# zhaoweicai/mscnn

Measured on AMD Instinct MI355X. Metric: images/sec mscnn-7s-576 KITTI-car inference, higher is better.
Workload: dtype f32

## Files before the change

include/mscnn_hip.h:

```cpp
#ifndef MSCNN_HIP_H_
#define MSCNN_HIP_H_

#include <stddef.h>
#include <stdint.h>

#if defined(__GNUC__)
#define MSCNN_API __attribute__((visibility("default")))
#else
#define MSCNN_API
#endif

#ifdef __cplusplus
extern "C" {
#endif

typedef enum {
  MSCNN_OK = 0,
  MSCNN_ERR_BAD_ARG = 1,
  MSCNN_ERR_HIP = 2,
  MSCNN_ERR_WORKSPACE = 3,
  MSCNN_ERR_UNSUPPORTED = 4
} mscnn_status;

MSCNN_API const char* mscnn_last_error(void);
MSCNN_API const char* mscnn_version(void);

typedef struct mscnn_conv_plan mscnn_conv_plan;

typedef enum {
  MSCNN_CONV_ALGO_AUTO = 0,
  MSCNN_CONV_ALGO_DIRECT = 1,
  MSCNN_CONV_ALGO_WINO_F2 = 2,
  MSCNN_CONV_ALGO_WINO_F3 = 3,
  MSCNN_CONV_ALGO_F16 = 4,
  MSCNN_CONV_ALGO_WINO_F3_X3 = 5,
  MSCNN_CONV_ALGO_WINO_F4 = 6
} mscnn_conv_algo;

typedef struct {
  int N, Cin, H, W;
  int Cout, Kh, Kw;
  int pad_h, pad_w, stride_h, stride_w, group;
  int relu;
  int algo;
  int tune_variant, tune_grid, tune_flags;
} mscnn_conv_desc;

MSCNN_API int mscnn_conv2d_plan_create(const mscnn_conv_desc* desc, mscnn_conv_plan** plan_out);
MSCNN_API void mscnn_conv2d_plan_destroy(mscnn_conv_plan* plan);
MSCNN_API size_t mscnn_conv2d_packed_weight_bytes(const mscnn_conv_plan* plan);
MSCNN_API size_t mscnn_conv2d_workspace_bytes(const mscnn_conv_plan* plan);
MSCNN_API const char* mscnn_conv2d_plan_kernel(const mscnn_conv_plan* plan);
MSCNN_API double mscnn_conv2d_plan_flops(const mscnn_conv_plan* plan);
MSCNN_API const char* mscnn_conv2d_plan_dtype(const mscnn_conv_plan* plan);
MSCNN_API double mscnn_conv2d_plan_executed_flops(const mscnn_conv_plan* plan);
MSCNN_API int mscnn_conv2d_plan_plane_columns(const mscnn_conv_plan* plan, int* cols, int n);
MSCNN_API int mscnn_conv2d_plan_set_profiling(mscnn_conv_plan* plan, int on);
MSCNN_API int mscnn_conv2d_plan_stage_ms(const mscnn_conv_plan* plan, float ms_out[3]);
#define MSCNN_AMAX_SLOTS 1024
MSCNN_API int mscnn_conv2d_plan_publishes_amax(const mscnn_conv_plan* plan);
MSCNN_API int mscnn_conv2d_plan_set_amax_io(mscnn_conv_plan* plan, const uint32_t* in_bound, uint32_t* out_amax);
MSCNN_API int mscnn_conv2d_plan_set_batch(mscnn_conv_plan* plan, int N);
MSCNN_API unsigned long long mscnn_conv2d_plan_weight_layout(const mscnn_conv_plan* plan);
MSCNN_API int mscnn_conv2d_pack_weights(const mscnn_conv_plan* plan, const float* w, float* packed, void* stream);
MSCNN_API int mscnn_conv2d_fwd_f32(const mscnn_conv_plan* plan, const float* x, const float* w, const float* packed,
                         const float* bias, float* y, void* workspace, size_t workspace_bytes, void* stream);
MSCNN_API int mscnn_conv2d_plan_can_pool(const mscnn_conv_plan* plan);
MSCNN_API int mscnn_conv2d_fwd_pool_f32(const mscnn_conv_plan* plan, const float* x, const float* w, const float* packed,
                              const float* bias, float* y, float* y_pool, void* workspace, size_t workspace_bytes,
                              void* stream);

MSCNN_API int mscnn_relu_fwd_f32(const float* x, float* y, size_t count, float negative_slope, void* stream);

MSCNN_API int mscnn_pool_out_dim(int in, int kernel, int pad, int stride);
MSCNN_API int mscnn_pool2d_fwd_f32(const float* x, float* y, int N, int C, int H, int W, int kernel_h, int kernel_w,
                         int pad_h, int pad_w, int stride_h, int stride_w, int method, void* stream);

MSCNN_API int mscnn_inner_product_fwd_f32(const float* x, const float* w, const float* bias, float* y,
                                int M, int N, int K, int relu, void* stream);
MSCNN_API void mscnn_debug_inner_product_rows(int rows);

MSCNN_API int mscnn_inner_product_wg_supported(int M, int N, int K);
MSCNN_API size_t mscnn_inner_product_wg_packed_bytes(int N, int K);
MSCNN_API size_t mscnn_inner_product_wg_workspace_bytes(int M, int N, int K);
MSCNN_API int mscnn_inner_product_wg_pack(const float* w, float* wt, int N, int K, void* stream);
MSCNN_API int mscnn_inner_product_wg_fwd(const float* x, const float* wt, const float* bias, float* y, int M, int N, int K, int relu,
                                         void* workspace, size_t workspace_bytes, void* stream);
MSCNN_API unsigned long long mscnn_wgemm_handoff_event(void);
MSCNN_API void mscnn_wgemm_force_whole_tiles(int on);
MSCNN_API int mscnn_wgemm_whole_tiles_forced(void);
MSCNN_API void mscnn_debug_wgemm_handoff_fault(int drop_publish, unsigned spin_limit);
MSCNN_API long mscnn_debug_wgemm_schedule(const mscnn_conv_plan* plan, int whole_tiles, int* rows, long max_rows, int info[8]);
MSCNN_API int mscnn_inner_product_x3_supported(int N, int K);
MSCNN_API size_t mscnn_inner_product_x3_packed_bytes(int N, int K);
MSCNN_API size_t mscnn_inner_product_x3_workspace_bytes(int M, int N, int K);
MSCNN_API int mscnn_inner_product_x3_pack(const float* w, void* packed, int N, int K, void* stream);
MSCNN_API int mscnn_inner_product_x3_fwd(const float* x, const void* packed, const float* bias, float* y, int M, int N, int K, int relu,
                               const uint32_t* in_bound, void* workspace, size_t workspace_bytes, void* stream);
MSCNN_API int mscnn_inner_product_f16_supported(int N, int K);
MSCNN_API int mscnn_inner_product_pack_f16(const float* w, void* w16, int N, int K, void* stream);
MSCNN_API int mscnn_inner_product_fwd_f16(const float* x, const void* w16, const float* bias, float* y, int M, int N, int K, int relu,
                                          void* stream);

MSCNN_API int mscnn_concat_channels_f32(const float* x, float* y, int N, int C, int inner, int C_total, int c_offset, void* stream);

MSCNN_API int mscnn_deconv_depthwise_fwd_f32(const float* x, const float* w, const float* bias, float* y,
                                   int N, int C, int H, int W, int Kh, int Kw, int pad_h, int pad_w,
                                   int stride_h, int stride_w, void* stream);

MSCNN_API int mscnn_deconv2d_fwd_f32(const float* x, const float* w, const float* bias, float* y, int N, int Cin, int H, int W,
                                     int Cout, int Kh, int Kw, int pad_h, int pad_w, int stride_h, int stride_w, int group,
                                     void* stream);

MSCNN_API int mscnn_max_rel_diff_f32(const float* a, const float* ref, size_t count, float floor, float* out_dev, void* stream);
MSCNN_API int mscnn_max_rel_diff_strided_f32(const float* a, size_t a_stride, const float* ref, size_t ref_stride, size_t planes, size_t run,
                                             const double* sumsq_dev, double sumsq_count, float* out_dev, void* stream);
MSCNN_API int mscnn_store_words_i32(int* dst_dev, const int* values_host, int n, void* stream);
MSCNN_API int mscnn_sum_squares_f32(const float* x, size_t count, double* out_dev, void* stream);

MSCNN_API int mscnn_softmax_fwd_f32(const float* x, float* y, int outer, int C, int inner, void* stream);

MSCNN_API int mscnn_roipool_fwd_f32(const float* feat, const float* rois, float* out, int R, int N, int C, int H, int W,
                          int pooled_h, int pooled_w, float spatial_scale, float pad_ratio,
                          int C_total, int c_offset, void* stream);
MSCNN_API int mscnn_roipool_pair_fwd_f32(const float* feat, const float* rois, float* out, int R, int N, int C, int H, int W,
                                         int pooled_h, int pooled_w, float spatial_scale, float pad_ratio_a, int c_offset_a,
                                         float pad_ratio_b, int c_offset_b, int C_total, void* stream);

MSCNN_API int mscnn_conv2d_plan_can_chain(const mscnn_conv_plan* plan, const mscnn_conv_plan* next);
MSCNN_API int mscnn_conv2d_plan_can_pool_only(const mscnn_conv_plan* plan);
MSCNN_API int mscnn_conv2d_fwd_chain_f32(const mscnn_conv_plan* plan, const mscnn_conv_plan* next, const float* x, const float* packed,
                               const float* bias, float* y, float* y_pool, void* workspace, size_t workspace_bytes,
                               void* next_workspace, size_t next_workspace_bytes, void* stream);

MSCNN_API int mscnn_conv2d_plan_can_fuse_roipool(const mscnn_conv_plan* plan, int C, int pooled_h, int pooled_w);
MSCNN_API size_t mscnn_conv2d_roipool_workspace_bytes(const mscnn_conv_plan* plan, int N, int C, int H, int W);
MSCNN_API size_t mscnn_roipool_maps_bytes(int N, int C, int H, int W);
MSCNN_API int mscnn_roipool_maps_build_f32(const float* feat, float* maps, int N, int C, int H, int W, void* stream);
MSCNN_API int mscnn_conv2d_fwd_roipool_pair_f32(const mscnn_conv_plan* plan, const float* feat, const float* prepared_maps, int N, int C,
                                                int H, int W, const float* rois, float spatial_scale, float pad_ratio_a,
                                                float pad_ratio_b, const float* packed_w, const float* bias, float* y, void* workspace,
                                                size_t workspace_bytes, void* stream);

MSCNN_API int mscnn_roialign_fwd_f32(const float* feat, const float* rois, float* out, int R, int N, int C, int H, int W,
                                     int pooled_h, int pooled_w, float spatial_scale, float pad_ratio, void* stream);
MSCNN_API int mscnn_roialign_ave_fwd_f32(const float* feat, const float* rois, float* out, int R, int N, int C, int H, int W,
                                         int pooled_h, int pooled_w, float spatial_scale, float pad_ratio,
                                         int C_total, int c_offset, void* stream);
MSCNN_API int mscnn_roialign_ave_pair_fwd_f32(const float* feat, const float* rois, float* out, int R, int N, int C, int H, int W,
                                              int pooled_h, int pooled_w, float spatial_scale, float pad_ratio_a, int c_offset_a,
                                              float pad_ratio_b, int c_offset_b, int C_total, void* stream);

MSCNN_API int mscnn_eltwise_fwd_f32(const float* const* bottoms_host, int num_bottoms, const float* coeffs_host, float* y,
                                    size_t count, int op, void* stream);

#define MSCNN_BOXOUT_MAX_HEADS 16
typedef struct {
  int num_heads;
  int num;
  int channels;
  int head_h[MSCNN_BOXOUT_MAX_HEADS], head_w[MSCNN_BOXOUT_MAX_HEADS];
  float field_w[MSCNN_BOXOUT_MAX_HEADS], field_h[MSCNN_BOXOUT_MAX_HEADS], downsample_rate[MSCNN_BOXOUT_MAX_HEADS];
  float fg_thr, iou_thr;
  int nms_mode;
  float field_whr, field_xyr;
  int max_nms_num, max_post_nms_num;
  float min_size;
  int do_bbox_norm;
  float bbox_mean[4], bbox_std[4];
} mscnn_boxoutput_desc;

MSCNN_API size_t mscnn_boxoutput_workspace_bytes(const mscnn_boxoutput_desc* desc);
MSCNN_API int mscnn_boxoutput_max_rows(const mscnn_boxoutput_desc* desc);
MSCNN_API int mscnn_boxoutput_fwd_f32(const mscnn_boxoutput_desc* desc, const float* const* heads_host,
                            float* rois_out, float* props_out, int* anchor_ids_out, int cap,
                            int* count_out_dev, void* workspace, size_t workspace_bytes, void* stream);
MSCNN_API size_t mscnn_boxoutput_batch_workspace_bytes(const mscnn_boxoutput_desc* desc);
MSCNN_API int mscnn_boxoutput_batch_fwd_f32(const mscnn_boxoutput_desc* desc, const float* const* heads_host,
                            float* rois_out, float* props_out, int* anchor_ids_out, int cap,
                            int* count_out_dev, void* workspace, size_t workspace_bytes, void* stream);

MSCNN_API size_t mscnn_nms_workspace_bytes(int n);
MSCNN_API int mscnn_nms_greedy_f32(const float* boxes_xywh, int n, float iou_thr, int nms_mode, unsigned char* keep_out,
                         void* workspace, size_t workspace_bytes, void* stream);

MSCNN_API int mscnn_decodebbox_fwd_f32(const float* bbox, const float* prior, float* out, int R, int bbox_dim,
                             const float* mean_host, const float* std_host, void* stream);

typedef struct {
  int ncls, cls_id;
  float bbox_mean[4], bbox_std[4];
  float proposal_thr;
  double ratio_h, ratio_w, org_h, org_w, nms_overlap;
} mscnn_detections_desc;
MSCNN_API size_t mscnn_detections_workspace_bytes(int R);

enum { MSCNN_NMS_TYPE_MAXG = 0, MSCNN_NMS_TYPE_MAX = 1, MSCNN_NMS_TYPE_MS = 2, MSCNN_NMS_TYPE_COVER = 3, MSCNN_NMS_TYPE_NONE = 4 };
enum { MSCNN_NMS_OVR_UNION = 0, MSCNN_NMS_OVR_MIN = 1 };
#ifndef MSCNN_NMS_PARAMS_DEFINED
#define MSCNN_NMS_PARAMS_DEFINED
typedef struct {
  int type;
  int ovr_dnm;
  double thr;
  float det_thr;
} mscnn_nms_params;
#endif
MSCNN_API int mscnn_nms_params_resolve(const mscnn_nms_params* nms, mscnn_nms_params* out);
MSCNN_API int mscnn_nms_params_from_names(const char* type, const char* ovr_dnm, double thr, double maxn, float det_thr,
                                          mscnn_nms_params* out);
MSCNN_API int mscnn_detections_fwd(const mscnn_detections_desc* desc, const float* bbox_pred, const float* cls_pred,
                         const float* props, int R, double* dets_out, int* ids_out, int* count_out_dev,
                         void* workspace, size_t workspace_bytes, void* stream);

MSCNN_API int mscnn_detections_nms_fwd(const mscnn_detections_desc* desc, const mscnn_nms_params* nms, const float* bbox_pred,
                                       const float* cls_pred, const float* props, int R, double* dets_out, int* ids_out,
                                       int* count_out_dev, void* workspace, size_t workspace_bytes, void* stream);

MSCNN_API int mscnn_detections_cascade_fwd(const mscnn_detections_desc* desc, float det_thr, const float* boxes,
                                 const float* cls_prob, const float* props, int R, double* dets_out, int* ids_out,
                                 int* count_out_dev, void* workspace, size_t workspace_bytes, void* stream);
MSCNN_API int mscnn_detections_cascade_nms_fwd(const mscnn_detections_desc* desc, float det_thr, const mscnn_nms_params* nms,
                                               const float* boxes, const float* cls_prob, const float* props, int R, double* dets_out,
                                               int* ids_out, int* count_out_dev, void* workspace, size_t workspace_bytes, void* stream);

enum { MSCNN_MULTI_PACK_WORDS = 4 };
typedef struct { size_t dets, ids, total; } mscnn_multi_pack_layout;
static inline mscnn_multi_pack_layout mscnn_multi_pack_layout_of(int num_segments, int cap) {
  const size_t S = (size_t)(num_segments > 0 ? num_segments : 0), rows = (size_t)(cap > 0 ? cap : 1);
  mscnn_multi_pack_layout L;
  L.dets = sizeof(int32_t) * MSCNN_MULTI_PACK_WORDS * (1 + S);
  L.ids = L.dets + rows * 5 * sizeof(double);
  L.total = (L.ids + rows * sizeof(int32_t) + 15) / 16 * 16;
  return L;
}
#ifdef __HIPCC__
__host__ __device__
#endif
static inline size_t mscnn_multi_pack_slot(int K, int row0, int k, int rows) {
  return (size_t)K * row0 + (size_t)k * rows;
// ... 88 lines not shown
```

mscnn_amd/csrc/gemm.hip:

```cpp
#include "common.h"
#include "wgemm.h"

namespace {

typedef float f32x16 __attribute__((ext_vector_type(16)));

constexpr int BK = 32, LDK = BK + 4;

struct GemmArgs {
  const float* x; const float* w; const float* bias; float* y; float* ws;
  int M, N, K, MT, NT, KI, G, relu;
  long total_iters;
};

__device__ __forceinline__ void wg_range(long total, int G, int g, long& b, long& e) {
  b = total * g / G;
  e = total * (g + 1) / G;
}

template <int BM, int BN>
__global__ __launch_bounds__(256) void gemm_tn_kernel(GemmArgs a) {
  static_assert(BM * BN == 128 * 128 && BM % 64 == 0 && BN % 64 == 0, "4 waves of 64 x 64");
  __shared__ __attribute__((aligned(16))) float ldsX[BM * LDK];
  __shared__ __attribute__((aligned(16))) float ldsW[BN * LDK];
// ... 378 lines not shown

static int inner_product_gemm(const float* x, const void* w, bool w_is_f16, const float* bias, float* y, int M, int N, int K, int relu,
                              hipStream_t st);

extern "C" int mscnn_inner_product_fwd_f16(const float* x, const void* w16, const float* bias, float* y, int M, int N, int K, int relu,
                                           void* stream) {
  MSCNN_REQUIRE(M >= 0 && N > 0 && K > 0, "inner_product: bad shape M=%d N=%d K=%d", M, N, K);
  if (M == 0) return MSCNN_OK;
  MSCNN_REQUIRE(x && w16 && y, "inner_product: null pointer");
  MSCNN_REQUIRE(mscnn_inner_product_f16_supported(N, K) && reinterpret_cast<uintptr_t>(x) % 16 == 0 && reinterpret_cast<uintptr_t>(w16) % 16 == 0,
                "inner_product f16: needs N >= 64, K %% 8 == 0 and 16-byte aligned operands (N=%d K=%d)", N, K);
  return inner_product_gemm(x, w16, true, bias, y, M, N, K, relu, as_stream(stream));
}

static int g_ip_rows = 0;
extern "C" void mscnn_debug_inner_product_rows(int rows) { g_ip_rows = rows == 2 || rows == 4 || rows == 8 ? rows : 0; }

extern "C" int mscnn_inner_product_fwd_f32(const float* x, const float* w, const float* bias, float* y, int M, int N, int K,
                                           int relu, void* stream) {
  MSCNN_REQUIRE(M >= 0 && N > 0 && K > 0, "inner_product: bad shape M=%d N=%d K=%d", M, N, K);
  if (M == 0) return MSCNN_OK;
  MSCNN_REQUIRE(x && w && y, "inner_product: null pointer");
  hipStream_t st = as_stream(stream);
  const bool aligned = (K % 4 == 0) && (reinterpret_cast<uintptr_t>(x) % 16 == 0) && (reinterpret_cast<uintptr_t>(w) % 16 == 0);
  if (N < 64 || !aligned) {
    if (N <= kRowMaxN && K <= 256 * kRowMaxKPerThread) {
      const int rows = g_ip_rows ? g_ip_rows : (N <= 5 ? 4 : 2);
#define MSCNN_IP_ROWWISE(NB_, R_) ip_rowwise_kernel<NB_, R_><<<cdiv(M, R_), 256, 0, st>>>(x, w, bias, y, M, N, K, relu)
      if (N <= 5) { if (rows == 8) MSCNN_IP_ROWWISE(5, 8); else if (rows == 2) MSCNN_IP_ROWWISE(5, 2); else MSCNN_IP_ROWWISE(5, 4); }
      else { if (rows == 8) MSCNN_IP_ROWWISE(4, 8); else if (rows == 2) MSCNN_IP_ROWWISE(8, 2); else MSCNN_IP_ROWWISE(4, 4); }
#undef MSCNN_IP_ROWWISE
    } else {
      ip_generic_kernel<<<dim3(M, N < 64 ? N : 64), 256, 0, st>>>(x, w, bias, y, M, N, K, relu);
    }
    MSCNN_POST_LAUNCH();
    return MSCNN_OK;
  }
  return inner_product_gemm(x, w, false, bias, y, M, N, K, relu, st);
}

static int inner_product_gemm(const float* x, const void* w, bool w_is_f16, const float* bias, float* y, int M, int N, int K, int relu,
                              hipStream_t st) {
  GemmArgs a;
  a.x = x; a.w = static_cast<const float*>(w); a.bias = bias; a.y = y;
  a.M = M; a.N = N; a.K = K; a.relu = relu;
  const bool m64 = cdiv(M, 64) * 64 < cdiv(M, 128) * 128 && N >= 256;
  const int BM = m64 ? 64 : 128, BN = m64 ? 256 : 128;
  a.MT = cdiv(M, BM); a.NT = cdiv(N, BN); a.KI = cdiv(K, BK);
  a.total_iters = (long)a.MT * a.NT * a.KI;
  long G = 512;
  if (a.total_iters / 8 < G) G = a.total_iters / 8;
  if (G < 1) G = 1;
  a.G = (int)G;
  const size_t need = (size_t)a.G * 2 * BM * BN * sizeof(float);
  {
    const int rc = reserve_slabs(need, &a.ws);
    if (rc != MSCNN_OK) return rc;
  }
  if (w_is_f16) {
    if (m64) gemm16_tn_kernel<64, 256><<<a.G, 256, 0, st>>>(a);
    else gemm16_tn_kernel<128, 128><<<a.G, 256, 0, st>>>(a);
  } else {
    if (m64) gemm_tn_kernel<64, 256><<<a.G, 256, 0, st>>>(a);
    else gemm_tn_kernel<128, 128><<<a.G, 256, 0, st>>>(a);
  }
  MSCNN_POST_LAUNCH();
  if (m64) gemm_fixup_kernel<64, 256><<<a.MT * a.NT * 4, 256, 0, st>>>(a);
  else gemm_fixup_kernel<128, 128><<<a.MT * a.NT * 4, 256, 0, st>>>(a);
  MSCNN_POST_LAUNCH();
  return MSCNN_OK;
}


namespace {

__global__ __launch_bounds__(256) void ip_pack_rows_kernel(const float* __restrict__ x, float* __restrict__ up, int M, int K, int KI) {
  __shared__ float t[32][257];
  const int kc = blockIdx.x, mt = blockIdx.y, tid = threadIdx.x;
  const int r0 = mt * 256, k0 = kc * 32;
#pragma unroll
  for (int i = 0; i < 8; ++i) {
    const int v = tid + i * 256, row = v >> 3, k4 = (v & 7) * 4;
    float4 q = make_float4(0.f, 0.f, 0.f, 0.f);
    if (r0 + row < M) q = *reinterpret_cast<const float4*>(x + (size_t)(r0 + row) * K + k0 + k4);
    t[k4][row] = q.x; t[k4 + 1][row] = q.y; t[k4 + 2][row] = q.z; t[k4 + 3][row] = q.w;
  }
  __syncthreads();
  float* dst = up + ((size_t)mt * KI + kc) * (32 * 256);
#pragma unroll
  for (int i = 0; i < 32; ++i) dst[i * 256 + tid] = t[i][tid];
}

__global__ __launch_bounds__(256) void ip_transpose_w_kernel(const float* __restrict__ w, float* __restrict__ wt, int N, int K) {
  __shared__ float t[32][33];
  const int k0 = blockIdx.x * 32, n0 = blockIdx.y * 32, tx = threadIdx.x & 31, ty = threadIdx.x >> 5;
#pragma unroll
  for (int i = 0; i < 4; ++i) {
    const int n = n0 + ty + 8 * i, k = k0 + tx;
    t[ty + 8 * i][tx] = (n < N && k < K) ? w[(size_t)n * K + k] : 0.f;
  }
  __syncthreads();
#pragma unroll
  for (int i = 0; i < 4; ++i) {
    const int k = k0 + ty + 8 * i, n = n0 + tx;
    if (k < K && n < N) wt[(size_t)k * N + n] = t[tx][ty + 8 * i];
  }
}

bool ip_wg_plan(int M, int N, int K, mscnn::WgemmPlan* pl) {
  if (M < 192 || N % 128 != 0 || K % 32 != 0 || N < 256) return false;
  const int Mp = (M + 31) / 32 * 32;
  return mscnn::wgemm_plan(1, Mp, K, N, 1 + 64, pl) && pl->T_pad == N;
}

}

extern "C" int mscnn_inner_product_wg_supported(int M, int N, int K) {
  mscnn::WgemmPlan pl;
  return ip_wg_plan(M, N, K, &pl) ? 1 : 0;
}
extern "C" size_t mscnn_inner_product_wg_packed_bytes(int N, int K) { return (size_t)N * K * sizeof(float); }
extern "C" size_t mscnn_inner_product_wg_workspace_bytes(int M, int N, int K) {
  mscnn::WgemmPlan pl;
  if (!ip_wg_plan(M, N, K, &pl)) return 0;
  return (pl.packed_bytes + 255) / 256 * 256 + pl.ws_bytes;
}
extern "C" int mscnn_inner_product_wg_pack(const float* w, float* wt, int N, int K, void* stream) {
  MSCNN_REQUIRE(w && wt && N > 0 && K > 0, "inner_product wg pack: bad argument");
  ip_transpose_w_kernel<<<dim3(cdiv(K, 32), cdiv(N, 32)), 256, 0, as_stream(stream)>>>(w, wt, N, K);
  MSCNN_POST_LAUNCH();
  return MSCNN_OK;
}
extern "C" int mscnn_inner_product_wg_fwd(const float* x, const float* wt, const float* bias, float* y, int M, int N, int K, int relu,
                                          void* workspace, size_t workspace_bytes, void* stream) {
  MSCNN_REQUIRE(M >= 0 && N > 0 && K > 0, "inner_product: bad shape M=%d N=%d K=%d", M, N, K);
  if (M == 0) return MSCNN_OK;
  mscnn::WgemmPlan pl;
  MSCNN_REQUIRE(ip_wg_plan(M, N, K, &pl), "inner_product wg: shape M=%d N=%d K=%d is not one the plane-GEMM kernel takes", M, N, K);
  MSCNN_REQUIRE(x && wt && y && reinterpret_cast<uintptr_t>(x) % 16 == 0, "inner_product wg: null or unaligned pointer");
  MSCNN_REQUIRE_ALIGNED(wt, 16, "inner_product wg: wt");
  MSCNN_REQUIRE_ALIGNED(workspace, 16, "inner_product wg: workspace");
  const size_t need = mscnn_inner_product_wg_workspace_bytes(M, N, K);
  if (!workspace || workspace_bytes < need) {
    set_error("inner_product wg: workspace %zu < %zu", workspace_bytes, need);
    return MSCNN_ERR_WORKSPACE;
  }
  hipStream_t st = as_stream(stream);
  float* up = static_cast<float*>(workspace);
  float* slabs = reinterpret_cast<float*>(static_cast<unsigned char*>(workspace) + (pl.packed_bytes + 255) / 256 * 256);
  ip_pack_rows_kernel<<<dim3(pl.KI, pl.MT), 256, 0, st>>>(x, up, M, K, pl.KI);
  MSCNN_POST_LAUNCH();
  return mscnn::wgemm_launch(pl, up, wt, y, pl.ws_bytes ? slabs : nullptr, st, 0, nullptr, bias, relu, (size_t)M * N * sizeof(float));
}
```

mscnn_amd/csrc/wgemm.h:

```cpp
#pragma once
#include <hip/hip_runtime.h>
#include <cstddef>

namespace mscnn {

constexpr int kWgemmMaxPlanes = 36;

__host__ __device__ __forceinline__ void wgemm_tile_decode(int t, int MT, int NT, int P, const int* nt_off, int& p, int& nt, int& mt) {
  mt = t % MT;
  if (!nt_off) {
    nt = (t / MT) % NT;
    p = t / (MT * NT);
    return;
  }
#if defined(__HIP_DEVICE_COMPILE__)
  const int q = __builtin_amdgcn_readfirstlane(t / MT);
#else
  const int q = t / MT;
#endif
  int pp = 0;
  while (pp + 1 < P && nt_off[pp + 1] <= q) ++pp;
  p = pp;
  nt = q - nt_off[pp];
}

struct WgemmPlan {
  int P, Cout, Cin, T, T_pad;
  int BM, BN, CK, MT, NT, KI;
  int G;
  int tiles;
  int ragged;
  int cols[kWgemmMaxPlanes];
  int nt_off[kWgemmMaxPlanes + 1];
  int device;
  int full_q;
  int variant;
  double model_us;
  const char* name;
  size_t packed_bytes;
  size_t ws_bytes;
};

bool wgemm_plan(int P, int Cout, int Cin, int T, int variant, WgemmPlan* out, const int* plane_cols = nullptr);

int wgemm_launch(const WgemmPlan& p, const float* Up, const float* V, float* M, float* ws, hipStream_t st, int abl = 0,
                 unsigned long long* dbg = nullptr, const float* bias = nullptr, int relu = 0, size_t m_valid_bytes = 0);

unsigned long long wgemm_handoff_event();
void wgemm_force_whole_tiles(int on);
int wgemm_whole_tiles_forced();
void wgemm_debug_handoff_fault(int drop_publish, unsigned spin_limit);
long wgemm_debug_schedule(const WgemmPlan& p, int whole_tiles, int* out, long max_rows);

}
```

mscnn_amd/csrc/wgemm.hip:

```cpp
#include "wgemm.h"
#include "common.h"
#include <atomic>
#include <chrono>

namespace {

typedef float f32x16 __attribute__((ext_vector_type(16)));

struct WgemmArgs {
  const float* Up; const float* V; float* M; float* ws;
  int P, MT, NT, KI, Cin, Cout, T_pad;
  int tiles, G, abl;
  int full_q;
  unsigned ws_bytes;
  unsigned epoch;
  unsigned long long* dbg;
  unsigned up_bytes, v_bytes, m_bytes;
  const float* bias; int relu;
  unsigned long long* status;
  unsigned spin_limit;
  int drop_publish;
  int nt_off[mscnn::kWgemmMaxPlanes + 1];
};

template <int BM_, int BN_, int WGM_, int WGN_, int CK_, int ST_, int DPG_ = 1, int SK_ = 0>
struct WCfg {
  static constexpr int BM = BM_, BN = BN_, WGM = WGM_, WGN = WGN_, CK = CK_, ST = ST_;
  static constexpr int DPG = DPG_, SK = SK_;
  static constexpr int NW = WGM * WGN, THREADS = NW * 64;
  static constexpr int WM = BM / WGM, WN = BN / WGN, MI = WM / 32, NI = WN / 32;
  static constexpr int A_BYTES = CK * BM * 4, B_BYTES = CK * BN * 4, STAGE_BYTES = A_BYTES + B_BYTES;
  static constexpr int STAGE_FLOATS = STAGE_BYTES / 4;
  static constexpr int PA = A_BYTES / 1024, PB = B_BYTES / 1024;
  static constexpr int PA_W = PA / NW, PB_W = (PB + NW - 1) / NW;
  static constexpr int NP = PA_W + PB_W;
  static constexpr int F4_PER_ROW = BN / 4;
  static constexpr bool B_EVEN = (64 % F4_PER_ROW == 0) && (PB % NW == 0);
  static constexpr int ROWS_PER_PIECE = B_EVEN ? 64 / F4_PER_ROW : 0;
  static constexpr int LDS_FLOATS = ST * STAGE_FLOATS + (B_EVEN ? 0 : 256);
  static constexpr int STEPS = CK / 2;
  static_assert(PA % NW == 0 && B_BYTES % 1024 == 0, "pieces per wave");
  static_assert(LDS_FLOATS * 4 <= 160 * 1024, "LDS ring");
  static_assert(WM % 32 == 0 && WN % 32 == 0, "wave tile");
};

template <int I, int N, class F>
__device__ __forceinline__ void static_for(F&& f) {
  if constexpr (I < N) {
    f(std::integral_constant<int, I>{});
    static_for<I + 1, N>(f);
  }
}

__device__ __forceinline__ __amdgpu_buffer_rsrc_t make_rsrc(const void* p, unsigned bytes) {
  return __builtin_amdgcn_make_buffer_rsrc(const_cast<void*>(p), 0, (int)bytes, 0x00020000);
}

__device__ __forceinline__ void dma16(__amdgpu_buffer_rsrc_t rsrc, unsigned voff, unsigned soff, unsigned lds_addr) {
  soff = __builtin_amdgcn_readfirstlane(soff);
  lds_addr = __builtin_amdgcn_readfirstlane(lds_addr);
  asm volatile("s_nop 4\n\ts_mov_b32 m0, %3\n\ts_nop 0\n\tbuffer_load_dwordx4 %0, %1, %2 offen lds" ::"v"(voff), "s"(rsrc), "s"(soff), "s"(lds_addr) : "memory");
}

template <int N>
__device__ __forceinline__ void wait_vm_barrier() {
  if constexpr (N == 0) asm volatile("s_waitcnt vmcnt(0)\n\ts_barrier" ::: "memory");
  else asm volatile("s_waitcnt vmcnt(%0)\n\ts_barrier" ::"n"(N) : "memory");
}

template <int OFF>
__device__ __forceinline__ float lds_rd(unsigned addr) {
  float r;
  asm volatile("ds_read_b32 %0, %1 offset:%2" : "=v"(r) : "v"(addr), "n"(OFF) : "memory");
  return r;
}
template <int N>
__device__ __forceinline__ void lds_wait() { asm volatile("s_waitcnt lgkmcnt(%0)" ::"n"(N) : "memory"); }
__device__ __forceinline__ void lds_pin(float& v) { asm volatile("" : "+v"(v)); }

__device__ __host__ __forceinline__ void wg_range(int total, int G, int g, int& b, int& e) {
  b = (int)((unsigned)total * (unsigned)g / (unsigned)G);
  e = (int)((unsigned)total * (unsigned)(g + 1) / (unsigned)G);
}

struct SegCursor {
  int slot, G, KI, full_q, rem_tile0, r;
  int it, re;
  int nparts;
  __device__ __forceinline__ void init(const WgemmArgs& a, int slot_) { init(a.tiles, a.G, a.KI, a.full_q, slot_); }
  __device__ __host__ __forceinline__ void init(int tiles, int G_, int KI_, int a_full_q, int slot_) {
    slot = slot_; G = G_; KI = KI_; rem_tile0 = a_full_q * G_; r = 0; nparts = 0;
    const int rounds = slot_ < tiles ? (tiles - slot_ + G_ - 1) / G_ : 0;
    full_q = a_full_q < rounds ? a_full_q : rounds;
    if (tiles > rem_tile0) wg_range((tiles - rem_tile0) * KI_, G_, slot_, it, re);
    else it = re = 0;
  }
  __device__ __forceinline__ int units() const { return full_q * KI + (re - it); }
  __device__ __host__ __forceinline__ bool next(int& t, int& k0, int& k1, int& part) {
    if (r < full_q) { t = slot + r * G; k0 = 0; k1 = KI; part = -1; ++r; return true; }
    if (it >= re) return false;
    t = rem_tile0 + it / KI;
    k0 = it % KI;
    const int left = re - it;
    k1 = left < KI - k0 ? k0 + left : KI;
    it += k1 - k0;
    part = (k0 == 0 && k1 == KI) ? -1 : nparts++;
    return true;
  }
};

template <class C, int ABL, int EPI = 0, bool RAG = false>
__global__ __launch_bounds__(C::THREADS, C::NW / 4) void wgemm_kernel(WgemmArgs a) {
  __shared__ __attribute__((aligned(1024))) float lds[C::LDS_FLOATS];
  __shared__ unsigned s_handoff_timeout;
  static_assert(C::ST == 3, "the ring protocol below is written for three stages");
  const int tid = threadIdx.x;
  const int lane = tid & 63;
  const int wave = __builtin_amdgcn_readfirstlane(tid >> 6);
  const int l31 = lane & 31, khalf = lane >> 5;
  const int wm = wave / C::WGN, wn = wave % C::WGN;

  const int xcd = (int)(blockIdx.x % 8), gq = a.G / 8, gr = a.G % 8;
  const int slot = xcd * gq + min(xcd, gr) + (int)(blockIdx.x / 8);
  SegCursor pcur, ccur;
  pcur.init(a, slot); ccur.init(a, slot);
  const int nunits = pcur.units();
  if (nunits == 0) return;
  unsigned long long dbg_c = 0, dbg_r = 0;
  if (a.dbg && tid == 0) { dbg_c = __builtin_amdgcn_s_memtime(); dbg_r = __builtin_amdgcn_s_memrealtime(); }

  const __amdgpu_buffer_rsrc_t rA = make_rsrc(a.Up, a.up_bytes), rB = make_rsrc(a.V, a.v_bytes), rM = make_rsrc(a.M, a.m_bytes),
                               rW = make_rsrc(a.ws, a.ws_bytes);
  const unsigned row_bytes = (unsigned)a.T_pad * 4u;
  const unsigned vA = (unsigned)lane * 16u;
  const unsigned vB = (unsigned)(lane / C::F4_PER_ROW) * row_bytes + (unsigned)(lane % C::F4_PER_ROW) * 16u;
  unsigned vBj[C::PB_W];
#pragma unroll
  for (int i = 0; i < C::PB_W; ++i) {
    const int u = (wave * C::PB_W + i) * 64 + lane;
    vBj[i] = wave * C::PB_W + i < C::PB ? (unsigned)(u / C::F4_PER_ROW) * row_bytes + (unsigned)(u % C::F4_PER_ROW) * 16u : 0x80000000u;
  }
  const unsigned lds0 = (unsigned)(size_t)lds;
  const unsigned a_lane = (unsigned)(khalf * C::BM + wm * C::WM + l31) * 4u;
  const unsigned b_lane = (unsigned)C::A_BYTES + (unsigned)(khalf * C::BN + wn * C::WN + l31) * 4u;

  int pu = 0, p_kc = 0, p_k1 = 0, p_stage = 0;
  unsigned p_a = 0, p_b = 0;
  unsigned vA_eff = vA, vB_eff = vB;
  auto p_begin = [&]() {
    if (pu >= nunits) {
      vA_eff = 0x80000000u; vB_eff = 0x80000000u;
#pragma unroll
      for (int i = 0; i < C::PB_W; ++i) vBj[i] = 0x80000000u;
    }
    if (p_kc == p_k1 && pu < nunits) {
      int t, part;
      pcur.next(t, p_kc, p_k1, part);
      int mt, nt, p;
      mscnn::wgemm_tile_decode(t, a.MT, a.NT, a.P, RAG ? a.nt_off : nullptr, p, nt, mt);
      p_kc = __builtin_amdgcn_readfirstlane(p_kc); p_k1 = __builtin_amdgcn_readfirstlane(p_k1);
      p_a = __builtin_amdgcn_readfirstlane((unsigned)((p * a.MT + mt) * a.KI) * (unsigned)C::A_BYTES);
      p_b = __builtin_amdgcn_readfirstlane(((unsigned)(p * a.Cin) * (unsigned)a.T_pad + (unsigned)(nt * C::BN)) * 4u);
    }
  };
  auto p_piece = [&](auto ic) {
    constexpr int i = decltype(ic)::value;
    const unsigned ls = lds0 + (unsigned)p_stage * C::STAGE_BYTES;
    if constexpr (i < C::PA_W) {
      const unsigned sa = p_a + (unsigned)p_kc * C::A_BYTES + (unsigned)(wave * C::PA_W + i) * 1024u;
      dma16(rA, vA_eff, sa, ls + (unsigned)(wave * C::PA_W + i) * 1024u);
    } else if constexpr (C::B_EVEN) {
      const int j = wave * C::PB_W + (i - C::PA_W);
      const unsigned sb = p_b + (unsigned)(p_kc * C::CK + j * C::ROWS_PER_PIECE) * row_bytes;
      dma16(rB, vB_eff, sb, ls + C::A_BYTES + (unsigned)j * 1024u);
    } else {
      const int j = wave * C::PB_W + (i - C::PA_W);
      const unsigned sb = p_b + (unsigned)(p_kc * C::CK) * row_bytes;
      dma16(rB, vBj[i - C::PA_W], sb, j < C::PB ? ls + C::A_BYTES + (unsigned)j * 1024u : lds0 + (unsigned)(C::ST * C::STAGE_BYTES));
    }
  };
  auto p_end = [&]() {
    ++pu;
    ++p_kc;
    if (++p_stage == C::ST) p_stage = 0;
  };

#pragma unroll
  for (int i = 0; i < 2; ++i)
    if (pu < nunits) {
      p_begin();
      static_for<0, C::NP>([&](auto ic) { p_piece(ic); });
      p_end();
    }
  wait_vm_barrier<0>();

  f32x16 acc[2][C::MI][C::NI];
#pragma unroll
  for (int q = 0; q < 2; ++q)
#pragma unroll
    for (int mi = 0; mi < C::MI; ++mi)
#pragma unroll
      for (int ni = 0; ni < C::NI; ++ni)
#pragma unroll
        for (int r = 0; r < 16; ++r) acc[q][mi][ni][r] = 0.f;
  float old_bias[C::NI];
#pragma unroll
  for (int ni = 0; ni < C::NI; ++ni) old_bias[ni] = 0.f;
  unsigned old_voff[C::MI][C::NI];
#pragma unroll
  for (int mi = 0; mi < C::MI; ++mi)
#pragma unroll
    for (int ni = 0; ni < C::NI; ++ni) old_voff[mi][ni] = 0x80000000u;

  float av[2][C::MI], bv[2][C::NI];
#define WG_READ(buf, stage_addr, s)                                                                                         \
  {                                                                                                                         \
    _Pragma("unroll") for (int mi = 0; mi < C::MI; ++mi) av[buf][mi] = 0.f;                                                  \
    static_for<0, C::MI>([&](auto m_) { av[buf][decltype(m_)::value] = lds_rd<(s) * 2 * C::BM * 4 + decltype(m_)::value * 128>((stage_addr) + a_lane); }); \
    static_for<0, C::NI>([&](auto n_) { bv[buf][decltype(n_)::value] = lds_rd<(s) * 2 * C::BN * 4 + decltype(n_)::value * 128>((stage_addr) + b_lane); }); \
  }
  constexpr int NR = C::MI + C::NI;
  constexpr int NMF = C::MI * C::NI;
  constexpr int TOTAL = NMF * 16;
  constexpr int SPG = (TOTAL + (C::STEPS - C::SK) - 1) / (C::STEPS - C::SK);
  constexpr int SPM = (SPG + NMF - 1) / NMF;
  constexpr int DMA_GROUPS = (C::NP + C::DPG - 1) / C::DPG;
  static_assert(C::DPG <= NMF && DMA_GROUPS <= C::STEPS && C::SK < C::STEPS, "schedule");
  constexpr int AFTER_DMA = [] {
    int n = 0;
    for (int g = 0; g < C::STEPS; ++g)
      for (int j = 0; j < NMF; ++j) {
        if (g < C::SK) continue;
        const int lo = (g - C::SK) * SPG + j * SPM, hi_g = (g - C::SK + 1) * SPG;
        int cnt = 0;
        for (int k = lo; k < lo + SPM && k < hi_g && k < TOTAL; ++k) ++cnt;
        const bool after = g > DMA_GROUPS - 1 || (g == DMA_GROUPS - 1 && j > (C::NP - 1) % C::DPG);
        if (after) n += cnt;
      }
    return n;
  }();

  __amdgpu_buffer_rsrc_t old_rsrc = rM;
  unsigned old_rowb = row_bytes;
  bool old_pub = false;
  unsigned c_addr = lds0;
  WG_READ(0, c_addr, 0);

  auto store_one = [&](auto qc, auto ec) {
    constexpr int Q = decltype(qc)::value, e = decltype(ec)::value;
    constexpr int blk = e / 16, r = e % 16, mi = blk / C::NI, ni = blk % C::NI, dr = (r & 3) + 8 * (r >> 2);
    float v = acc[Q][mi][ni][r];
    if (old_pub) __builtin_amdgcn_raw_buffer_store_b32(__builtin_bit_cast(unsigned, v), old_rsrc, old_voff[mi][ni], (unsigned)dr * old_rowb, 16);
    else {
      if constexpr (EPI) {
        v += old_bias[ni];
        if (a.relu) v = v < 0.f ? 0.f : v;
      }
      __builtin_amdgcn_raw_buffer_store_b32(__builtin_bit_cast(unsigned, v), old_rsrc, old_voff[mi][ni], (unsigned)dr * old_rowb, 0);
    }
  };

  auto chunk = [&](auto par_c, auto flush_c, unsigned next_addr) {
    constexpr int PAR = decltype(par_c)::value;
    constexpr bool FLUSH = decltype(flush_c)::value;
    p_begin();
    static_for<0, C::STEPS>([&](auto sc) {
      constexpr int s = decltype(sc)::value, cur = s & 1, nxt = cur ^ 1;
      if constexpr (!(ABL & 8)) {
        if constexpr (s + 1 < C::STEPS) WG_READ(nxt, c_addr, s + 1)
        else WG_READ(nxt, next_addr, 0)
        lds_wait<NR>();
      }
#pragma unroll
      for (int mi = 0; mi < C::MI; ++mi) lds_pin(av[cur][mi]);
#pragma unroll
      for (int ni = 0; ni < C::NI; ++ni) lds_pin(bv[cur][ni]);
      __builtin_amdgcn_sched_barrier(0);
      static_for<0, NMF>([&](auto jc) {
        constexpr int j = decltype(jc)::value, mi = j / C::NI, ni = j % C::NI;
        if constexpr (!(ABL & 4)) acc[PAR][mi][ni] = __builtin_amdgcn_mfma_f32_32x32x2f32(av[cur][mi], bv[cur][ni], acc[PAR][mi][ni], 0, 0, 0);
        __builtin_amdgcn_sched_barrier(0);
        if constexpr (FLUSH && s >= C::SK) {
          if constexpr (!(ABL & 2))
            static_for<0, SPM>([&](auto kc_) {
              constexpr int e = (s - C::SK) * SPG + j * SPM + decltype(kc_)::value;
              if constexpr (e < (s - C::SK + 1) * SPG && e < TOTAL) store_one(std::integral_constant<int, PAR ^ 1>{}, std::integral_constant<int, e>{});
            });
          __builtin_amdgcn_sched_barrier(0);
        }
        if constexpr (j < C::DPG && s * C::DPG + j < C::NP) {
          if constexpr (!(ABL & 1)) p_piece(std::integral_constant<int, s * C::DPG + j>{});
          __builtin_amdgcn_sched_barrier(0);
        }
      });
    });
    p_end();
    if constexpr (ABL & 16) asm volatile("s_waitcnt vmcnt(0)" ::: "memory");
    else if constexpr (FLUSH) wait_vm_barrier<(AFTER_DMA < 63 ? AFTER_DMA : 63)>();
    else wait_vm_barrier<0>();
    c_addr = next_addr;
  };

  int c_stage = 0;
  auto next_stage_addr = [&]() {
    if (++c_stage == C::ST) c_stage = 0;
    return lds0 + (unsigned)c_stage * C::STAGE_BYTES;
  };
  int t, k0, k1, part;
  int fin_tile = -1;
  typedef __attribute__((address_space(1))) unsigned long long gu64;
  gu64* flags = (gu64*)(a.ws + (size_t)a.G * (C::BM * C::BN));
  const unsigned long long want_flag = ((unsigned long long)a.epoch << 32) | (unsigned)~a.epoch;
  auto publish_flag = [&]() {
    asm volatile("s_waitcnt vmcnt(0)\n\ts_barrier" ::: "memory");
    if (tid == 0 && !a.drop_publish) __hip_atomic_store(flags + slot, want_flag, __ATOMIC_RELAXED, __HIP_MEMORY_SCOPE_AGENT);
  };
  auto segment = [&](auto par_c) {
    constexpr int PAR = decltype(par_c)::value;
    chunk(par_c, std::true_type{}, next_stage_addr());
    if (old_pub) { publish_flag(); old_pub = false; }
    for (int kc = k0 + 1; kc < k1; ++kc) chunk(par_c, std::false_type{}, next_stage_addr());
    int mt, nt, p;
    mscnn::wgemm_tile_decode(t, a.MT, a.NT, a.P, RAG ? a.nt_off : nullptr, p, nt, mt);
    const bool pub = part >= 0 && k0 > 0;
    if (part >= 0 && k0 == 0) fin_tile = t;
    old_pub = pub;
    if (pub) { old_rsrc = rW; old_rowb = (unsigned)C::BN * 4u; }
    else { old_rsrc = rM; old_rowb = row_bytes; }
    const unsigned slab = (unsigned)slot * (unsigned)(C::BM * C::BN * 4);
    if constexpr (EPI) {
#pragma unroll
      for (int ni = 0; ni < C::NI; ++ni) {
        const int col = nt * C::BN + wn * C::WN + ni * 32 + l31;
        old_bias[ni] = (a.bias && col < a.T_pad) ? a.bias[col] : 0.f;
      }
    }
#pragma unroll
    for (int mi = 0; mi < C::MI; ++mi)
#pragma unroll
      for (int ni = 0; ni < C::NI; ++ni) {
        const int row = wm * C::WM + mi * 32, col = wn * C::WN + ni * 32 + l31;
        const int co0 = mt * C::BM + row;
        const unsigned to_m = co0 + 32 <= a.Cout ? ((unsigned)(p * a.Cout + co0 + 4 * khalf) * (unsigned)a.T_pad + (unsigned)(nt * C::BN + col)) * 4u : 0x80000000u;
        const unsigned to_ws = slab + (unsigned)((row + 4 * khalf) * C::BN + col) * 4u;
        old_voff[mi][ni] = pub ? to_ws : to_m;
#pragma unroll
        for (int r = 0; r < 16; ++r) acc[PAR ^ 1][mi][ni][r] = 0.f;
      }
  };
  int par = 0;
  while (true) {
    if (!ccur.next(t, k0, k1, part)) break;
    segment(std::integral_constant<int, 0>{});
    par = 1;
    if (!ccur.next(t, k0, k1, part)) break;
    segment(std::integral_constant<int, 1>{});
    par = 0;
  }
  auto finish = [&](auto qc) {
    constexpr int Q = decltype(qc)::value;
    if (fin_tile >= 0) {
      const int rem_tile0 = a.full_q * a.G, RU = (a.tiles - rem_tile0) * a.KI;
      const int tile_end = (fin_tile - rem_tile0 + 1) * a.KI;
      for (int s2 = slot + 1; s2 < a.G; ++s2) {
        int b, e;
        wg_range(RU, a.G, s2, b, e);
        if (b >= tile_end) break;
        if (e <= b) continue;
        if (tid == 0) {
          unsigned spins = 0;
          while (__hip_atomic_load(flags + s2, __ATOMIC_RELAXED, __HIP_MEMORY_SCOPE_AGENT) != want_flag && ++spins < a.spin_limit) __builtin_amdgcn_s_sleep(4);
          const bool timed_out = spins >= a.spin_limit;
          s_handoff_timeout = timed_out ? 1u : 0u;
          if (timed_out) {
            __hip_atomic_store(flags + a.G, 1ull, __ATOMIC_RELAXED, __HIP_MEMORY_SCOPE_AGENT);
            if (a.status) __hip_atomic_store(a.status, (unsigned long long)a.epoch, __ATOMIC_RELAXED, __HIP_MEMORY_SCOPE_SYSTEM);
          }
          __builtin_amdgcn_fence(__ATOMIC_ACQUIRE, "agent");
        }
        __syncthreads();
        const bool poisoned = s_handoff_timeout != 0;
        const unsigned sl2 = (unsigned)s2 * (unsigned)(C::BM * C::BN * 4);
#pragma unroll
        for (int mi = 0; mi < C::MI; ++mi)
#pragma unroll
          for (int ni = 0; ni < C::NI; ++ni) {
            const unsigned vo = sl2 + (unsigned)((wm * C::WM + mi * 32 + 4 * khalf) * C::BN + wn * C::WN + ni * 32 + l31) * 4u;
#pragma unroll
            for (int r = 0; r < 16; ++r)
              acc[Q][mi][ni][r] += __builtin_bit_cast(float, __builtin_amdgcn_raw_buffer_load_b32(rW, vo, (unsigned)((r & 3) + 8 * (r >> 2)) * (unsigned)(C::BN * 4), 0));
            if (poisoned)
#pragma unroll
              for (int r = 0; r < 16; ++r) acc[Q][mi][ni][r] = __builtin_nanf("");
          }
        __syncthreads();
      }
    }
    if (!(ABL & 2) || a.tiles < 0) static_for<0, NMF * 16>([&](auto ec) { store_one(qc, ec); });
  };
  if (par == 1) finish(std::integral_constant<int, 0>{});
  else finish(std::integral_constant<int, 1>{});
  if (old_pub) publish_flag();
  if (a.dbg && tid == 0) {
    const unsigned long long end_r = __builtin_amdgcn_s_memrealtime();
    a.dbg[blockIdx.x * 2] = __builtin_amdgcn_s_memtime() - dbg_c;
    a.dbg[blockIdx.x * 2 + 1] = end_r - dbg_r;
    a.dbg[2 * a.G + blockIdx.x * 2] = dbg_r;
    a.dbg[2 * a.G + blockIdx.x * 2 + 1] = end_r;
  }
}

typedef void (*WgemmFn)(WgemmArgs);
struct WEntry { const char* name; int variant, abl, BM, BN, CK, threads; WgemmFn fn; WgemmFn fn_ragged = nullptr; };
#define WG_ENTRY(name, v, abl, BM, BN, WGM, WGN, CK) {name, v, abl, BM, BN, CK, WGM * WGN * 64, wgemm_kernel<WCfg<BM, BN, WGM, WGN, CK, 3>, abl>}
#define WG_ENTRY_R(name, v, BM, BN, WGM, WGN, CK) {name, v, 0, BM, BN, CK, WGM * WGN * 64, wgemm_kernel<WCfg<BM, BN, WGM, WGN, CK, 3>, 0>, wgemm_kernel<WCfg<BM, BN, WGM, WGN, CK, 3>, 0, 0, true>}
#define WG_ENTRY_EPI(name, v, BM, BN, WGM, WGN, CK) {name, v + 64, 0, BM, BN, CK, WGM * WGN * 64, wgemm_kernel<WCfg<BM, BN, WGM, WGN, CK, 3>, 0, 1>}
#define WG_ENTRY_S(name, v, BM, BN, WGM, WGN, CK, DPG, SK) {name, v, 0, BM, BN, CK, WGM * WGN * 64, wgemm_kernel<WCfg<BM, BN, WGM, WGN, CK, 3, DPG, SK>, 0>}
const WEntry kW[] = {
    WG_ENTRY_R("wgemm_256x128_ck32", 1, 256, 128, 4, 2, 32),
    WG_ENTRY_R("wgemm_128x256_ck32", 2, 128, 256, 2, 4, 32),
    WG_ENTRY_R("wgemm_128x128_ck32", 3, 128, 128, 2, 4, 32),
    WG_ENTRY_R("wgemm_256x96_ck32", 4, 256, 96, 8, 1, 32),
    WG_ENTRY_R("wgemm_256x160_ck32", 5, 256, 160, 8, 1, 32),
    WG_ENTRY_EPI("wgemm_256x128_ck32_epi", 1, 256, 128, 4, 2, 32),
#ifdef MSCNN_WGEMM_DEV
    WG_ENTRY_S("wgemm_256x128_ck32_d2", 25, 256, 128, 4, 2, 32, 2, 0),
    WG_ENTRY_S("wgemm_256x128_ck32_d2_s3", 26, 256, 128, 4, 2, 32, 2, 3),
    WG_ENTRY_S("wgemm_256x128_ck32_d3_s2", 27, 256, 128, 4, 2, 32, 3, 2),
    WG_ENTRY_S("wgemm_256x128_ck32_d1_s6", 28, 256, 128, 4, 2, 32, 1, 6),
#endif
#ifdef MSCNN_WGEMM_DEV
    WG_ENTRY("wgemm_256x128_ck32", 1, 1, 256, 128, 4, 2, 32),
    WG_ENTRY("wgemm_256x128_ck32", 1, 2, 256, 128, 4, 2, 32),
    WG_ENTRY("wgemm_256x128_ck32", 1, 3, 256, 128, 4, 2, 32),
    WG_ENTRY("wgemm_256x128_ck32", 1, 4, 256, 128, 4, 2, 32),
    WG_ENTRY("wgemm_256x128_ck32", 1, 11, 256, 128, 4, 2, 32),
    WG_ENTRY("wgemm_256x128_ck32", 1, 19, 256, 128, 4, 2, 32),
    WG_ENTRY("wgemm_256x128_ck32", 1, 27, 256, 128, 4, 2, 32),
    WG_ENTRY("wgemm_128x256_ck32", 2, 1, 128, 256, 2, 4, 32),
    WG_ENTRY("wgemm_128x256_ck32", 2, 2, 128, 256, 2, 4, 32),
    WG_ENTRY("wgemm_128x256_ck32", 2, 3, 128, 256, 2, 4, 32),
#endif
};

}

namespace mscnn {

static int device_cus(int* dev_out) {
  int dev = 0, n = 0;
  *dev_out = -1;
  if (hipGetDevice(&dev) != hipSuccess || hipDeviceGetAttribute(&n, hipDeviceAttributeMultiprocessorCount, dev) != hipSuccess || n <= 0) {
    (void)hipGetLastError();
    return 256;
  }
  *dev_out = dev;
  return n;
}

namespace {
std::atomic<int> g_whole_tiles{0};
std::atomic<unsigned> g_spin_limit{1u << 22};
std::atomic<int> g_drop_publish{0};
std::atomic<unsigned long long*> g_status[64];
}

static unsigned long long* status_word(int dev) {
  if (dev < 0 || dev >= 64) return nullptr;
  unsigned long long* w = g_status[dev].load(std::memory_order_acquire);
  if (w) return w;
  void* p = nullptr;
  if (hipHostMalloc(&p, 64, hipHostMallocPortable | hipHostMallocMapped | hipHostMallocCoherent) != hipSuccess || !p) {
    (void)hipGetLastError();
    return nullptr;
  }
  *static_cast<volatile unsigned long long*>(p) = 0ull;
  unsigned long long* expected = nullptr;
  if (!g_status[dev].compare_exchange_strong(expected, static_cast<unsigned long long*>(p))) {
    (void)hipHostFree(p);
    return expected;
  }
  return static_cast<unsigned long long*>(p);
}

unsigned long long wgemm_handoff_event() {
  int dev = 0;
  if (hipGetDevice(&dev) != hipSuccess) { (void)hipGetLastError(); return 0; }
  if (dev < 0 || dev >= 64) return 0;
  const unsigned long long* w = g_status[dev].load(std::memory_order_acquire);
  return w ? *static_cast<const volatile unsigned long long*>(w) : 0ull;
}
void wgemm_force_whole_tiles(int on) { g_whole_tiles.store(on ? 1 : 0); }
int wgemm_whole_tiles_forced() { return g_whole_tiles.load(); }
void wgemm_debug_handoff_fault(int drop_publish, unsigned spin_limit) {
  g_drop_publish.store(drop_publish ? 1 : 0);
  g_spin_limit.store(spin_limit ? spin_limit : (1u << 22));
}

bool wgemm_plan(int P, int Cout, int Cin, int T, int variant, WgemmPlan* o, const int* plane_cols) {
  if (P < 1 || P > kWgemmMaxPlanes) return false;
  if (plane_cols)
    for (int p = 0; p < P; ++p)
      if (plane_cols[p] < 0 || plane_cols[p] > T) return false;
  const int variant_flags = variant >> 8;
  variant &= 255;
  if (variant == 0) {
    variant = Cout >= 256 ? 1 : 2;
    if (variant == 1 && !variant_flags) {
      WgemmPlan p1, pc;
      if (wgemm_plan(P, Cout, Cin, T, 1, &p1, plane_cols)) {
        double best = 0.95 * p1.model_us;
        for (int cand : {4, 5})
          if (wgemm_plan(P, Cout, Cin, T, cand, &pc, plane_cols) && pc.model_us < best) { best = pc.model_us; variant = cand; }
        if ((long)p1.tiles * 2 < p1.G && wgemm_plan(P, Cout, Cin, T, 3, &pc, plane_cols) && pc.model_us < best) { best = pc.model_us; variant = 3; }
      }
    }
  }
  const WEntry* e = nullptr;
  for (const WEntry& w : kW) if (w.variant == variant && w.abl == 0) e = &w;
  if (!e || Cin % e->CK != 0 || Cout % 32 != 0) return false;
  o->P = P; o->Cout = Cout; o->Cin = Cin; o->T = T;
  o->BM = e->BM; o->BN = e->BN; o->CK = e->CK;
  o->T_pad = (T + e->BN - 1) / e->BN * e->BN;
  o->MT = (Cout + e->BM - 1) / e->BM; o->NT = o->T_pad / e->BN; o->KI = Cin / e->CK;
  o->G = device_cus(&o->device);
  o->ragged = plane_cols ? 1 : 0;
  o->nt_off[0] = 0;
  for (int p = 0; p < kWgemmMaxPlanes; ++p) {
    o->cols[p] = p < P ? (plane_cols ? plane_cols[p] : T) : 0;
    o->nt_off[p + 1] = o->nt_off[p] + (p < P ? (plane_cols ? (plane_cols[p] + e->BN - 1) / e->BN : o->NT) : 0);
  }
  const long tiles = (long)o->MT * o->nt_off[P];
  o->tiles = (int)tiles;
  const long rem = tiles % o->G;
  const double chunk_us = (double)e->BM * e->BN * e->CK / 128.0 / 2214.0;
  const double whole = (double)((tiles + o->G - 1) / o->G) * (o->KI * chunk_us + 6.0);
  const double handoff_us = 18.0 * (double)(e->BM * e->BN) / (256.0 * 128.0);
  const double split = (double)tiles * o->KI / o->G * chunk_us + (double)tiles / o->G * 6.0 + handoff_us;
  o->full_q = (int)(tiles / o->G);
  if (rem > 0 && !(split < 0.97 * whole)) o->full_q += 1;
  o->model_us = rem > 0 ? (split < 0.97 * whole ? split : whole) : whole;
  if (variant_flags & 1) o->full_q = (int)(tiles / o->G);
  if (variant_flags & 2) o->full_q = (int)((tiles + o->G - 1) / o->G);
  o->variant = variant; o->name = e->name;
  o->packed_bytes = (size_t)P * o->MT * o->KI * e->CK * e->BM * 4;
  o->ws_bytes = tiles > (long)o->full_q * o->G ? (size_t)o->G * e->BM * e->BN * 4 + ((size_t)o->G + 1) * 8 : 0;
  const double lim = 2147483648.0 - 65536.0;
  if ((double)tiles * o->KI * o->G >= 2.0e9 || o->KI < 1) return false;
  if ((double)P * Cin * o->T_pad * 4 >= lim || (double)P * Cout * o->T_pad * 4 >= lim || (double)o->packed_bytes >= lim ||
      (double)o->ws_bytes >= lim) return false;
  return true;
}

int wgemm_launch(const WgemmPlan& p, const float* Up, const float* V, float* M, float* ws, hipStream_t st, int abl, unsigned long long* dbg,
                 const float* bias, int relu, size_t m_valid_bytes) {
  const WEntry* e = nullptr;
  for (const WEntry& w : kW) if (w.variant == p.variant && w.abl == abl) e = &w;
  if (!e || (p.ragged && !e->fn_ragged)) return MSCNN_ERR_BAD_ARG;
  int dev = -1;
  if (hipGetDevice(&dev) != hipSuccess) { (void)hipGetLastError(); dev = -1; }
  if (p.device >= 0 && dev != p.device) {
    set_error("wgemm: plan made on device %d launched on device %d (re-plan on the device that runs it)", p.device, dev);
    return MSCNN_ERR_BAD_ARG;
  }
  WgemmArgs a;
  a.Up = Up; a.V = V; a.M = M; a.ws = ws;
  a.P = p.P; a.MT = p.MT; a.NT = p.NT; a.KI = p.KI; a.Cin = p.Cin; a.Cout = p.Cout; a.T_pad = p.T_pad;
  a.tiles = p.tiles; a.G = p.G;
  a.abl = abl; a.dbg = dbg;
  for (int i = 0; i <= kWgemmMaxPlanes; ++i) a.nt_off[i] = p.nt_off[i];
  a.full_q = p.full_q; a.ws_bytes = (unsigned)p.ws_bytes;
  if (g_whole_tiles.load(std::memory_order_relaxed)) a.full_q = (a.tiles + p.G - 1) / p.G;
  const int rem = a.tiles - a.full_q * p.G;
  if (rem > 0 && !ws) { set_error("wgemm: workspace missing"); return MSCNN_ERR_WORKSPACE; }
  a.status = rem > 0 ? status_word(dev) : nullptr;
  a.spin_limit = g_spin_limit.load(std::memory_order_relaxed);
  a.drop_publish = g_drop_publish.load(std::memory_order_relaxed);
  a.up_bytes = (unsigned)p.packed_bytes; a.v_bytes = (unsigned)((size_t)p.P * p.Cin * p.T_pad * 4); a.m_bytes = (unsigned)((size_t)p.P * p.Cout * p.T_pad * 4);
  if (m_valid_bytes) a.m_bytes = (unsigned)m_valid_bytes;
  a.bias = bias; a.relu = relu;
  static std::atomic<unsigned> g_epoch{(unsigned)std::chrono::steady_clock::now().time_since_epoch().count() * 2654435761u};
  unsigned ep = ++g_epoch;
  if (ep == 0) ep = ++g_epoch;
  a.epoch = ep;
  (p.ragged ? e->fn_ragged : e->fn)<<<p.G, e->threads, 0, st>>>(a);
  MSCNN_POST_LAUNCH();
  return MSCNN_OK;
}

long wgemm_debug_schedule(const WgemmPlan& p, int whole_tiles, int* out, long max_rows) {
  const int full_q = whole_tiles ? (p.tiles + p.G - 1) / p.G : p.full_q;
  long n = 0;
  for (int slot = 0; slot < p.G; ++slot) {
    SegCursor c;
    c.init(p.tiles, p.G, p.KI, full_q, slot);
    int t, k0, k1, part;
    while (c.next(t, k0, k1, part)) {
      if (out) {
        if (n >= max_rows) return -1;
        int pl, nt, mt;
        wgemm_tile_decode(t, p.MT, p.NT, p.P, p.ragged ? p.nt_off : nullptr, pl, nt, mt);
        const int row[7] = {slot, pl, nt, mt, k0, k1, part};
        for (int i = 0; i < 7; ++i) out[n * 7 + i] = row[i];
      }
      ++n;
    }
  }
  return n;
}

}

extern "C" unsigned long long mscnn_wgemm_handoff_event(void) { return mscnn::wgemm_handoff_event(); }
extern "C" void mscnn_wgemm_force_whole_tiles(int on) { mscnn::wgemm_force_whole_tiles(on); }
extern "C" int mscnn_wgemm_whole_tiles_forced(void) { return mscnn::wgemm_whole_tiles_forced(); }
extern "C" void mscnn_debug_wgemm_handoff_fault(int drop_publish, unsigned spin_limit) { mscnn::wgemm_debug_handoff_fault(drop_publish, spin_limit); }
```

mscnn_amd/hipapi.py:

```python
import ctypes as C
import os

import numpy as np
import torch

_HERE = os.path.dirname(os.path.abspath(__file__))
LIB_PATH = os.path.join(_HERE, "libmscnn_hip.so")
_lib = None


class MscnnError(RuntimeError):
    pass


class ConvDesc(C.Structure):
    _fields_ = [(n, C.c_int) for n in ("N", "Cin", "H", "W", "Cout", "Kh", "Kw", "pad_h", "pad_w",
                                       "stride_h", "stride_w", "group", "relu", "algo", "tune_variant", "tune_grid", "tune_flags")]


AMAX_SLOTS = 1024
ALGO_AUTO, ALGO_DIRECT, ALGO_WINO_F2, ALGO_WINO_F3, ALGO_F16, ALGO_WINO_F3_X3, ALGO_WINO_F4 = 0, 1, 2, 3, 4, 5, 6


MAX_HEADS = 16


class BoxOutputDesc(C.Structure):
    _fields_ = [("num_heads", C.c_int), ("num", C.c_int), ("channels", C.c_int),
                ("head_h", C.c_int * MAX_HEADS), ("head_w", C.c_int * MAX_HEADS),
                ("field_w", C.c_float * MAX_HEADS), ("field_h", C.c_float * MAX_HEADS),
                ("downsample_rate", C.c_float * MAX_HEADS),
                ("fg_thr", C.c_float), ("iou_thr", C.c_float), ("nms_mode", C.c_int),
                ("field_whr", C.c_float), ("field_xyr", C.c_float),
                ("max_nms_num", C.c_int), ("max_post_nms_num", C.c_int), ("min_size", C.c_float),
                ("do_bbox_norm", C.c_int), ("bbox_mean", C.c_float * 4), ("bbox_std", C.c_float * 4)]


class DetectionsDesc(C.Structure):
    _fields_ = [("ncls", C.c_int), ("cls_id", C.c_int), ("bbox_mean", C.c_float * 4), ("bbox_std", C.c_float * 4),
                ("proposal_thr", C.c_float), ("ratio_h", C.c_double), ("ratio_w", C.c_double),
                ("org_h", C.c_double), ("org_w", C.c_double), ("nms_overlap", C.c_double)]


class ProposalsDesc(C.Structure):
    _fields_ = [("proposal_thr", C.c_float), ("ratio_h", C.c_double), ("ratio_w", C.c_double)]


PROPOSALS_IMAGES_PER_LAUNCH = 64


class NmsParams(C.Structure):
    _fields_ = [("type", C.c_int), ("ovr_dnm", C.c_int), ("thr", C.c_double), ("det_thr", C.c_float)]


NMS_MODES = {"IOU": 0, "IOMU": 1, "IOFU": 2}


def nms_params(type="maxg", ovr_dnm="union", thr=None, det_thr=0.0, maxn=None):
    out = NmsParams()
    _check(lib().mscnn_nms_params_from_names(None if type is None else str(type).encode(), None if ovr_dnm is None else str(ovr_dnm).encode(),
                                             float("-inf") if thr is None else float(thr), float("inf") if maxn is None else float(maxn),
                                             float(det_thr), C.byref(out)))
    return out


NMS_NULL = object()


def _nms_ref(nms):
    if nms is NMS_NULL:
        return None
    return C.byref(nms if isinstance(nms, NmsParams) else nms_params(**nms))


def lib():
    global _lib
    if _lib is None:
        if not os.path.exists(LIB_PATH):
            raise MscnnError(f"{LIB_PATH} not built: run `python -c 'import __graft_entry__ as g; g.build()'`")
        L = C.CDLL(LIB_PATH)
        L.mscnn_last_error.restype = C.c_char_p
        L.mscnn_version.restype = C.c_char_p
        L.mscnn_conv2d_plan_kernel.restype = C.c_char_p
        L.mscnn_conv2d_plan_kernel.argtypes = [C.c_void_p]
        L.mscnn_conv2d_plan_publishes_amax.argtypes = [C.c_void_p]
        L.mscnn_conv2d_plan_set_amax_io.argtypes = [C.c_void_p, C.c_void_p, C.c_void_p]
        L.mscnn_conv2d_plan_dtype.restype = C.c_char_p
        L.mscnn_conv2d_plan_dtype.argtypes = [C.c_void_p]
        L.mscnn_inner_product_f16_supported.argtypes = [C.c_int, C.c_int]
        L.mscnn_inner_product_x3_supported.argtypes = [C.c_int, C.c_int]
        L.mscnn_inner_product_x3_packed_bytes.restype = C.c_size_t
        L.mscnn_inner_product_x3_packed_bytes.argtypes = [C.c_int, C.c_int]
        L.mscnn_inner_product_x3_workspace_bytes.restype = C.c_size_t
        L.mscnn_inner_product_x3_workspace_bytes.argtypes = [C.c_int] * 3
        L.mscnn_inner_product_x3_pack.argtypes = [C.c_void_p, C.c_void_p, C.c_int, C.c_int, C.c_void_p]
        L.mscnn_inner_product_x3_fwd.argtypes = [C.c_void_p] * 4 + [C.c_int] * 4 + [C.c_void_p, C.c_void_p, C.c_size_t, C.c_void_p]
        L.mscnn_inner_product_wg_supported.argtypes = [C.c_int] * 3
        L.mscnn_inner_product_wg_packed_bytes.restype = C.c_size_t
        L.mscnn_inner_product_wg_packed_bytes.argtypes = [C.c_int, C.c_int]
        L.mscnn_inner_product_wg_workspace_bytes.restype = C.c_size_t
        L.mscnn_inner_product_wg_workspace_bytes.argtypes = [C.c_int] * 3
        L.mscnn_inner_product_wg_pack.argtypes = [C.c_void_p, C.c_void_p, C.c_int, C.c_int, C.c_void_p]
        L.mscnn_inner_product_wg_fwd.argtypes = [C.c_void_p] * 4 + [C.c_int] * 4 + [C.c_void_p, C.c_size_t, C.c_void_p]
        L.mscnn_max_rel_diff_f32.argtypes = [C.c_void_p, C.c_void_p, C.c_size_t, C.c_float, C.c_void_p, C.c_void_p]
        L.mscnn_sum_squares_f32.argtypes = [C.c_void_p, C.c_size_t, C.c_void_p, C.c_void_p]
        L.mscnn_max_rel_diff_strided_f32.argtypes = [C.c_void_p, C.c_size_t, C.c_void_p, C.c_size_t, C.c_size_t, C.c_size_t, C.c_void_p, C.c_double,
                                                     C.c_void_p, C.c_void_p]
        L.mscnn_store_words_i32.argtypes = [C.c_void_p, C.c_void_p, C.c_int, C.c_void_p]
        L.mscnn_wgemm_handoff_event.restype = C.c_ulonglong
        L.mscnn_wgemm_handoff_event.argtypes = []
        L.mscnn_wgemm_force_whole_tiles.restype = None
        L.mscnn_wgemm_force_whole_tiles.argtypes = [C.c_int]
        L.mscnn_wgemm_whole_tiles_forced.argtypes = []
        L.mscnn_debug_inner_product_rows.restype = None
        L.mscnn_debug_inner_product_rows.argtypes = [C.c_int]
        L.mscnn_debug_wgemm_handoff_fault.restype = None
        L.mscnn_debug_wgemm_handoff_fault.argtypes = [C.c_int, C.c_uint]
        L.mscnn_inner_product_pack_f16.argtypes = [C.c_void_p, C.c_void_p, C.c_int, C.c_int, C.c_void_p]
        L.mscnn_inner_product_fwd_f16.argtypes = [C.c_void_p] * 4 + [C.c_int] * 4 + [C.c_void_p]
        for f in ("mscnn_conv2d_plan_flops", "mscnn_conv2d_plan_executed_flops"):
            getattr(L, f).restype = C.c_double
            getattr(L, f).argtypes = [C.c_void_p]
        L.mscnn_conv2d_plan_set_profiling.argtypes = [C.c_void_p, C.c_int]
        L.mscnn_conv2d_plan_plane_columns.argtypes = [C.c_void_p, C.c_void_p, C.c_int]
        L.mscnn_debug_wgemm_schedule.restype = C.c_long
        L.mscnn_debug_wgemm_schedule.argtypes = [C.c_void_p, C.c_int, C.c_void_p, C.c_long, C.c_void_p]
        L.mscnn_conv2d_plan_stage_ms.argtypes = [C.c_void_p, C.c_void_p]
        for f in ("mscnn_conv2d_packed_weight_bytes", "mscnn_conv2d_workspace_bytes"):
            getattr(L, f).restype = C.c_size_t
            getattr(L, f).argtypes = [C.c_void_p]
        L.mscnn_conv2d_plan_destroy.argtypes = [C.c_void_p]
        L.mscnn_conv2d_plan_destroy.restype = None
        L.mscnn_conv2d_plan_set_batch.argtypes = [C.c_void_p, C.c_int]
        L.mscnn_conv2d_pack_weights.argtypes = [C.c_void_p] * 4
        L.mscnn_conv2d_fwd_f32.argtypes = [C.c_void_p] * 7 + [C.c_size_t, C.c_void_p]
        L.mscnn_conv2d_fwd_pool_f32.argtypes = [C.c_void_p] * 8 + [C.c_size_t, C.c_void_p]
        L.mscnn_conv2d_plan_can_pool.argtypes = [C.c_void_p]
        L.mscnn_conv2d_plan_can_fuse_roipool.argtypes = [C.c_void_p, C.c_int, C.c_int, C.c_int]
        L.mscnn_conv2d_plan_can_chain.argtypes = [C.c_void_p, C.c_void_p]
        L.mscnn_conv2d_plan_can_pool_only.argtypes = [C.c_void_p]
        L.mscnn_conv2d_fwd_chain_f32.argtypes = [C.c_void_p] * 8 + [C.c_size_t, C.c_void_p, C.c_size_t, C.c_void_p]
        L.mscnn_conv2d_roipool_workspace_bytes.restype = C.c_size_t
        L.mscnn_conv2d_roipool_workspace_bytes.argtypes = [C.c_void_p] + [C.c_int] * 4
        L.mscnn_conv2d_fwd_roipool_pair_f32.argtypes = ([C.c_void_p, C.c_void_p, C.c_void_p] + [C.c_int] * 4 + [C.c_void_p, C.c_float, C.c_float, C.c_float]
                                                        + [C.c_void_p] * 4 + [C.c_size_t, C.c_void_p])
        L.mscnn_roipool_maps_bytes.restype = C.c_size_t
        L.mscnn_roipool_maps_bytes.argtypes = [C.c_int] * 4
        L.mscnn_roipool_maps_build_f32.argtypes = [C.c_void_p, C.c_void_p] + [C.c_int] * 4 + [C.c_void_p]
        L.mscnn_conv2d_plan_weight_layout.argtypes = [C.c_void_p]
        L.mscnn_conv2d_plan_weight_layout.restype = C.c_ulonglong
        L.mscnn_relu_fwd_f32.argtypes = [C.c_void_p, C.c_void_p, C.c_size_t, C.c_float, C.c_void_p]
        L.mscnn_pool2d_fwd_f32.argtypes = [C.c_void_p, C.c_void_p] + [C.c_int] * 11 + [C.c_void_p]
        L.mscnn_inner_product_fwd_f32.argtypes = [C.c_void_p] * 4 + [C.c_int] * 4 + [C.c_void_p]
        L.mscnn_concat_channels_f32.argtypes = [C.c_void_p, C.c_void_p] + [C.c_int] * 5 + [C.c_void_p]
        L.mscnn_deconv_depthwise_fwd_f32.argtypes = [C.c_void_p] * 4 + [C.c_int] * 10 + [C.c_void_p]
        L.mscnn_softmax_fwd_f32.argtypes = [C.c_void_p, C.c_void_p, C.c_int, C.c_int, C.c_int, C.c_void_p]
        L.mscnn_roipool_fwd_f32.argtypes = ([C.c_void_p] * 3 + [C.c_int] * 7 + [C.c_float, C.c_float] + [C.c_int] * 2
                                            + [C.c_void_p])
        L.mscnn_roipool_pair_fwd_f32.argtypes = ([C.c_void_p] * 3 + [C.c_int] * 7 + [C.c_float, C.c_float, C.c_int, C.c_float, C.c_int, C.c_int]
                                                 + [C.c_void_p])
        L.mscnn_roialign_fwd_f32.argtypes = [C.c_void_p] * 3 + [C.c_int] * 7 + [C.c_float, C.c_float, C.c_void_p]
        L.mscnn_roialign_ave_fwd_f32.argtypes = ([C.c_void_p] * 3 + [C.c_int] * 7 + [C.c_float, C.c_float] + [C.c_int] * 2
                                                 + [C.c_void_p])
        L.mscnn_roialign_ave_pair_fwd_f32.argtypes = ([C.c_void_p] * 3 + [C.c_int] * 7
                                                      + [C.c_float, C.c_float, C.c_int, C.c_float, C.c_int, C.c_int] + [C.c_void_p])
        L.mscnn_eltwise_fwd_f32.argtypes = [C.c_void_p, C.c_int, C.c_void_p, C.c_void_p, C.c_size_t, C.c_int, C.c_void_p]
        L.mscnn_boxoutput_workspace_bytes.restype = C.c_size_t
        L.mscnn_boxoutput_workspace_bytes.argtypes = [C.c_void_p]
        L.mscnn_boxoutput_max_rows.argtypes = [C.c_void_p]
        L.mscnn_boxoutput_fwd_f32.argtypes = [C.c_void_p, C.c_void_p, C.c_void_p, C.c_void_p, C.c_void_p, C.c_int,
                                              C.c_void_p, C.c_void_p, C.c_size_t, C.c_void_p]
        L.mscnn_boxoutput_batch_workspace_bytes.restype = C.c_size_t
        L.mscnn_boxoutput_batch_workspace_bytes.argtypes = [C.c_void_p]
        L.mscnn_boxoutput_batch_fwd_f32.argtypes = L.mscnn_boxoutput_fwd_f32.argtypes
        L.mscnn_nms_workspace_bytes.restype = C.c_size_t
        L.mscnn_nms_workspace_bytes.argtypes = [C.c_int]
        L.mscnn_nms_greedy_f32.argtypes = [C.c_void_p, C.c_int, C.c_float, C.c_int, C.c_void_p, C.c_void_p, C.c_size_t,
                                           C.c_void_p]
        L.mscnn_decodebbox_fwd_f32.argtypes = [C.c_void_p] * 3 + [C.c_int, C.c_int, C.c_void_p, C.c_void_p, C.c_void_p]
        L.mscnn_detections_workspace_bytes.restype = C.c_size_t
        L.mscnn_detections_workspace_bytes.argtypes = [C.c_int]
        L.mscnn_detections_fwd.argtypes = [C.c_void_p] * 4 + [C.c_int] + [C.c_void_p] * 4 + [C.c_size_t, C.c_void_p]
        L.mscnn_detections_multi_pack_bytes.restype = C.c_size_t
        L.mscnn_detections_multi_pack_bytes.argtypes = [C.c_int, C.c_int]
        L.mscnn_detections_multi_workspace_bytes.restype = C.c_size_t
        L.mscnn_detections_multi_workspace_bytes.argtypes = [C.c_int, C.c_int]
        L.mscnn_detections_multi_fwd.argtypes = ([C.c_void_p, C.c_int, C.c_int] + [C.c_void_p] * 3 + [C.c_int, C.c_int, C.c_void_p, C.c_int,
                                                 C.c_void_p, C.c_size_t, C.c_void_p])
        L.mscnn_detections_cascade_multi_workspace_bytes.restype = C.c_size_t
        L.mscnn_detections_cascade_multi_workspace_bytes.argtypes = [C.c_int, C.c_int]
        L.mscnn_detections_cascade_multi_fwd.argtypes = ([C.c_void_p, C.c_float, C.c_int, C.c_int, C.c_int, C.c_void_p, C.c_int, C.c_int,
                                                         C.c_void_p, C.c_int, C.c_void_p, C.c_size_t, C.c_void_p])
        L.mscnn_nms_params_resolve.argtypes = [C.c_void_p, C.c_void_p]
        L.mscnn_nms_params_from_names.argtypes = [C.c_char_p, C.c_char_p, C.c_double, C.c_double, C.c_float, C.c_void_p]
        L.mscnn_detections_nms_fwd.argtypes = [C.c_void_p] * 5 + [C.c_int] + [C.c_void_p] * 4 + [C.c_size_t, C.c_void_p]
        L.mscnn_detections_cascade_nms_fwd.argtypes = ([C.c_void_p, C.c_float] + [C.c_void_p] * 4 + [C.c_int] + [C.c_void_p] * 4 +
                                                       [C.c_size_t, C.c_void_p])
        L.mscnn_detections_multi_nms_fwd.argtypes = ([C.c_void_p, C.c_void_p, C.c_int, C.c_int] + [C.c_void_p] * 3 +
                                                     [C.c_int, C.c_int, C.c_void_p, C.c_int, C.c_void_p, C.c_size_t, C.c_void_p])
        L.mscnn_detections_cascade_multi_nms_fwd.argtypes = ([C.c_void_p, C.c_float, C.c_void_p, C.c_int, C.c_int, C.c_int, C.c_void_p,
                                                              C.c_int, C.c_int, C.c_void_p, C.c_int, C.c_void_p, C.c_size_t, C.c_void_p])
        L.mscnn_detections_candidates_bytes.restype = C.c_size_t
        L.mscnn_detections_candidates_bytes.argtypes = [C.c_int, C.c_int]
        L.mscnn_detections_candidates_reset.argtypes = [C.c_void_p, C.c_int, C.c_int, C.c_void_p]
        L.mscnn_detections_candidates_add.argtypes = ([C.c_void_p] * 3 + [C.c_int] * 3 + [C.c_void_p] * 3 +
                                                      [C.c_int, C.c_void_p, C.c_int, C.c_void_p])
        L.mscnn_detections_candidates_cascade_add.argtypes = ([C.c_void_p, C.c_void_p, C.c_float, C.c_void_p] + [C.c_int] * 4 +
                                                              [C.c_void_p, C.c_int, C.c_void_p, C.c_int, C.c_void_p])
        L.mscnn_detections_candidates_add_views.argtypes = ([C.c_void_p] * 4 + [C.c_int] * 4 + [C.c_void_p] * 3 +
                                                            [C.c_int, C.c_void_p, C.c_int, C.c_void_p])
        L.mscnn_detections_candidates_cascade_add_views.argtypes = ([C.c_void_p, C.c_void_p, C.c_void_p, C.c_float, C.c_void_p] + [C.c_int] * 5 +
                                                                    [C.c_void_p, C.c_int, C.c_void_p, C.c_int, C.c_void_p])
        L.mscnn_preprocess_views_workspace_bytes.restype = C.c_size_t
        L.mscnn_preprocess_views_workspace_bytes.argtypes = [C.c_void_p, C.c_int, C.c_int, C.c_int]
        L.mscnn_preprocess_views_u8_f32.argtypes = ([C.c_void_p, C.c_void_p, C.c_void_p, C.c_int, C.c_void_p, C.c_int, C.c_void_p, C.c_int, C.c_int,
                                                     C.c_void_p, C.c_void_p, C.c_size_t, C.c_void_p])
        L.mscnn_detections_merge_workspace_bytes.restype = C.c_size_t
        L.mscnn_detections_merge_workspace_bytes.argtypes = [C.c_int, C.c_int]
        L.mscnn_detections_merge_fwd.argtypes = [C.c_void_p, C.c_void_p, C.c_int, C.c_void_p, C.c_int, C.c_void_p, C.c_void_p, C.c_size_t,
                                                 C.c_void_p]
        L.mscnn_proposals_multi_pack_bytes.restype = C.c_size_t
        L.mscnn_proposals_multi_pack_bytes.argtypes = [C.c_int, C.c_int]
        L.mscnn_proposals_multi_fwd.argtypes = [C.c_void_p, C.c_int, C.c_void_p, C.c_int, C.c_void_p, C.c_int, C.c_void_p]
        L.mscnn_rois_reason_text.restype = C.c_char_p
        L.mscnn_rois_reason_text.argtypes = [C.c_int]
        L.mscnn_rois_ingest_f32.argtypes = [C.c_void_p, C.c_int, C.c_int, C.c_int] + [C.c_void_p] * 7
        _lib = L
    return _lib


def _check(rc):
    if rc != 0:
        raise MscnnError(f"mscnn status {rc}: {lib().mscnn_last_error().decode()}")


def _dev(t):
    if t is None:
        return None
    if not t.is_cuda:
        raise MscnnError("libmscnn_hip has no CPU path: tensor must live on the GPU")
    if not t.is_contiguous():
        raise MscnnError("tensor must be contiguous")
    return C.c_void_p(t.data_ptr())


def _stream():
    return C.c_void_p(torch.cuda.current_stream().cuda_stream)


class ConvPlan:

    def __init__(self, N, Cin, H, W, Cout, Kh, Kw, pad=(0, 0), stride=(1, 1), group=1, relu=False, device="cuda",
                 algo=ALGO_AUTO, tune_variant=0, tune_grid=0, tune_flags=0):
        self.desc = ConvDesc(N, Cin, H, W, Cout, Kh, Kw, pad[0], pad[1], stride[0], stride[1], group, int(relu),
                             algo, tune_variant, tune_grid, tune_flags)
        self._p = C.c_void_p()
# ... 54 lines not shown
        return tuple(out)

    def out_shape(self):
        d = self.desc
        return (d.N, d.Cout, (d.H + 2 * d.pad_h - d.Kh) // d.stride_h + 1, (d.W + 2 * d.pad_w - d.Kw) // d.stride_w + 1)

    def set_batch(self, N):
        before, had = lib().mscnn_conv2d_plan_weight_layout(self._p), self.packed
        _check(lib().mscnn_conv2d_plan_set_batch(self._p, N))
        self.desc.N = N
        self._alloc()
        if getattr(self, "w", None) is not None and self.packed is not None and \
                (lib().mscnn_conv2d_plan_weight_layout(self._p) != before or self.packed is not had):
            self.pack(self.w)

    def pack(self, w):
        self.w = w
        if self.packed is not None:
            _check(lib().mscnn_conv2d_pack_weights(self._p, _dev(w), _dev(self.packed), _stream()))

    @property
    def publishes_amax(self):
        return bool(lib().mscnn_conv2d_plan_publishes_amax(self._p))

    def set_amax_io(self, in_bound=None, out_amax=None):
        self._amax = (in_bound, out_amax)
        _check(lib().mscnn_conv2d_plan_set_amax_io(self._p, _dev(in_bound), _dev(out_amax)))

    @property
    def can_pool(self):
        return bool(lib().mscnn_conv2d_plan_can_pool(self._p))

    def forward(self, x, bias=None, out=None, pool_out=None):
        if out is None:
            out = torch.empty(self.out_shape(), dtype=torch.float32, device=x.device)
        wsb = self.ws.numel() * 4 if self.ws is not None else 0
        _check(lib().mscnn_conv2d_fwd_pool_f32(self._p, _dev(x), _dev(self.w), _dev(self.packed), _dev(bias), _dev(out),
                                               _dev(pool_out), _dev(self.ws), wsb, _stream()))
        return out

    @property
    def can_pool_only(self):
        return bool(lib().mscnn_conv2d_plan_can_pool_only(self._p))

    def can_chain(self, nxt):
        return bool(lib().mscnn_conv2d_plan_can_chain(self._p, nxt._p))

    def forward_chain(self, x, nxt, bias=None, out=None, pool_out=None, write_y=True):
        if out is None and write_y:
            out = torch.empty(self.out_shape(), dtype=torch.float32, device=self.ws.device)
        wsb = self.ws.numel() * 4
        _check(lib().mscnn_conv2d_fwd_chain_f32(self._p, nxt._p if nxt is not None else None, _dev(x), _dev(self.packed), _dev(bias),
                                                _dev(out) if write_y else None, _dev(pool_out), _dev(self.ws), wsb,
                                                _dev(nxt.ws) if nxt is not None else None, nxt.ws.numel() * 4 if nxt is not None else 0,
                                                _stream()))
        return out

    def can_fuse_roipool(self, Cc, pooled_h, pooled_w):
        return bool(lib().mscnn_conv2d_plan_can_fuse_roipool(self._p, Cc, pooled_h, pooled_w))

    def forward_roipool_pair(self, feat, rois, spatial_scale, pad_a, pad_b, bias=None, out=None, maps=None):
        N, Cc, H, W = feat.shape
        need = lib().mscnn_conv2d_roipool_workspace_bytes(self._p, N, Cc, H, W)
        if self.ws is None or self.ws.numel() * 4 < need:
            self.ws = torch.empty((need + 3) // 4, dtype=torch.float32, device=feat.device)
        if out is None:
            out = torch.empty(self.out_shape(), dtype=torch.float32, device=feat.device)
        _check(lib().mscnn_conv2d_fwd_roipool_pair_f32(self._p, _dev(feat), _dev(maps), N, Cc, H, W, _dev(rois), spatial_scale, pad_a, pad_b,
                                                       _dev(self.packed), _dev(bias), _dev(out), _dev(self.ws), self.ws.numel() * 4,
                                                       _stream()))
        return out

    def __del__(self):
        try:
            if self._p:
                lib().mscnn_conv2d_plan_destroy(self._p)
                self._p = None
        except Exception:
            pass


def conv2d(x, w, bias=None, pad=(0, 0), stride=(1, 1), group=1, relu=False, algo=ALGO_AUTO):
    N, Cin, H, W = x.shape
    Cout, _, Kh, Kw = w.shape
    plan = ConvPlan(N, Cin, H, W, Cout, Kh, Kw, pad, stride, group, relu, device=x.device, algo=algo)
    plan.pack(w)
    y = plan.forward(x, bias)
    torch.cuda.current_stream().synchronize()
    return y


def relu(x, slope=0.0, inplace=False):
    y = x if inplace else torch.empty_like(x)
    _check(lib().mscnn_relu_fwd_f32(_dev(x), _dev(y), x.numel(), slope, _stream()))
    return y


def sum_squares(x):
    out = torch.zeros(1, dtype=torch.float64, device=x.device)
    _check(lib().mscnn_sum_squares_f32(_dev(x), x.numel(), _dev(out), _stream()))
    return out


def max_rel_diff(a, ref, floor=1.0):
    out = torch.zeros(1, dtype=torch.float32, device=a.device)
    _check(lib().mscnn_max_rel_diff_f32(_dev(a), _dev(ref), a.numel(), floor, _dev(out), _stream()))
    return out


def max_rel_diff_strided(a, a_stride, ref, ref_stride, planes, run, sumsq, sumsq_count):
    out = torch.zeros(1, dtype=torch.float32, device=a.device)
    _check(lib().mscnn_max_rel_diff_strided_f32(_dev(a), a_stride, _dev(ref), ref_stride, planes, run, _dev(sumsq), float(sumsq_count), _dev(out),
                                                _stream()))
    return out


def store_words(dst, values):
    arr = (C.c_int * len(values))(*[int(v) for v in values])
    _check(lib().mscnn_store_words_i32(_dev(dst), arr, len(values), _stream()))


def pool_out_dim(i, k, p, s):
    return lib().mscnn_pool_out_dim(i, k, p, s)


def pool2d(x, kernel=(2, 2), pad=(0, 0), stride=(2, 2), method="MAX"):
    N, Cc, H, W = x.shape
    Ho, Wo = pool_out_dim(H, kernel[0], pad[0], stride[0]), pool_out_dim(W, kernel[1], pad[1], stride[1])
    y = torch.empty((N, Cc, Ho, Wo), dtype=torch.float32, device=x.device)
    _check(lib().mscnn_pool2d_fwd_f32(_dev(x), _dev(y), N, Cc, H, W, kernel[0], kernel[1], pad[0], pad[1],
                                      stride[0], stride[1], 0 if method == "MAX" else 1, _stream()))
    return y


def inner_product_wg_supported(M, N, K):
    return bool(lib().mscnn_inner_product_wg_supported(M, N, K))


def inner_product_wg(x, w, bias=None, relu=False, wt=None, out=None):
    M = x.shape[0]
    K = x.numel() // M
    Nn = w.shape[0]
    if wt is None:
        wt = torch.empty((K, Nn), dtype=torch.float32, device=x.device)
        _check(lib().mscnn_inner_product_wg_pack(_dev(w), _dev(wt), Nn, K, _stream()))
    wb = lib().mscnn_inner_product_wg_workspace_bytes(M, Nn, K)
    ws = torch.empty((wb + 3) // 4, dtype=torch.float32, device=x.device)
    y = out if out is not None else torch.empty((M, Nn), dtype=torch.float32, device=x.device)
    _check(lib().mscnn_inner_product_wg_fwd(_dev(x), _dev(wt), _dev(bias), _dev(y), M, Nn, K, int(relu), _dev(ws), wb, _stream()))
    torch.cuda.current_stream().synchronize()
    return y, wt


def inner_product(x, w, bias=None, relu=False):
    M = x.shape[0]
    K = x.numel() // max(M, 1) if M else w.shape[1]
    Nn = w.shape[0]
    y = torch.empty((M, Nn), dtype=torch.float32, device=x.device)
    _check(lib().mscnn_inner_product_fwd_f32(_dev(x), _dev(w), _dev(bias), _dev(y), M, Nn, K, int(relu), _stream()))
    return y


def inner_product_x3(x, w, bias=None, relu=False, packed=None):
    M, K = x.shape[0], int(x.numel() // max(x.shape[0], 1))
    Nn = w.shape[0]
    if not lib().mscnn_inner_product_x3_supported(Nn, K):
        raise MscnnError(f"inner_product x3 needs N >= 128 and K % 32 == 0 (N={Nn}, K={K})")
    if packed is None:
        packed = torch.empty(lib().mscnn_inner_product_x3_packed_bytes(Nn, K), dtype=torch.uint8, device=x.device)
        _check(lib().mscnn_inner_product_x3_pack(_dev(w), _dev(packed), Nn, K, _stream()))
    wb = lib().mscnn_inner_product_x3_workspace_bytes(M, Nn, K)
    ws = torch.empty(wb, dtype=torch.uint8, device=x.device)
    y = torch.empty((M, Nn), dtype=torch.float32, device=x.device)
    _check(lib().mscnn_inner_product_x3_fwd(_dev(x), _dev(packed), _dev(bias), _dev(y), M, Nn, K, int(relu), None, _dev(ws), wb, _stream()))
    return y


def inner_product_f16(x, w, bias=None, relu=False):
    M = x.shape[0]
    Nn, K = w.shape[0], w[0].numel()
    if not lib().mscnn_inner_product_f16_supported(Nn, K):
        raise MscnnError(f"inner_product f16 needs N >= 64 and K % 8 == 0 (N={Nn}, K={K})")
    w16 = torch.empty(Nn * K, dtype=torch.float16, device=x.device)
    _check(lib().mscnn_inner_product_pack_f16(_dev(w), _dev(w16), Nn, K, _stream()))
    y = torch.empty((M, Nn), dtype=torch.float32, device=x.device)
    _check(lib().mscnn_inner_product_fwd_f16(_dev(x), _dev(w16), _dev(bias), _dev(y), M, Nn, K, int(relu), _stream()))
    return y


def concat_channels(xs):
    N = xs[0].shape[0]
    inner = xs[0][0, 0].numel()
    ctot = sum(t.shape[1] for t in xs)
    y = torch.empty((N, ctot) + tuple(xs[0].shape[2:]), dtype=torch.float32, device=xs[0].device)
    off = 0
    for t in xs:
        _check(lib().mscnn_concat_channels_f32(_dev(t), _dev(y), N, t.shape[1], inner, ctot, off, _stream()))
        off += t.shape[1]
    return y


def deconv_depthwise(x, w, bias=None, pad=(0, 0), stride=(1, 1)):
    N, Cc, H, W = x.shape
    Kh, Kw = w.shape[2], w.shape[3]
    Ho, Wo = stride[0] * (H - 1) + Kh - 2 * pad[0], stride[1] * (W - 1) + Kw - 2 * pad[1]
    y = torch.empty((N, Cc, Ho, Wo), dtype=torch.float32, device=x.device)
    _check(lib().mscnn_deconv_depthwise_fwd_f32(_dev(x), _dev(w), _dev(bias), _dev(y), N, Cc, H, W, Kh, Kw,
                                                pad[0], pad[1], stride[0], stride[1], _stream()))
    return y


def softmax(x, axis=1):
    outer = 1
    for d in x.shape[:axis]:
        outer *= d
    inner = 1
    for d in x.shape[axis + 1:]:
        inner *= d
    y = torch.empty_like(x)
    _check(lib().mscnn_softmax_fwd_f32(_dev(x), _dev(y), outer, x.shape[axis], inner, _stream()))
    return y


def roipool(feat, rois, pooled_h, pooled_w, spatial_scale, pad_ratio=0.0, out=None, c_total=None, c_offset=0):
    N, Cc, H, W = feat.shape
    R = rois.shape[0]
    c_total = c_total or Cc
    if out is None:
        out = torch.empty((R, c_total, pooled_h, pooled_w), dtype=torch.float32, device=feat.device)
    _check(lib().mscnn_roipool_fwd_f32(_dev(feat), _dev(rois), _dev(out), R, N, Cc, H, W, pooled_h, pooled_w,
                                       spatial_scale, pad_ratio, c_total, c_offset, _stream()))
    return out


def roipool_maps(feat, stream=None):
    N, Cc, H, W = feat.shape
    maps = torch.empty(lib().mscnn_roipool_maps_bytes(N, Cc, H, W) // 4, dtype=torch.float32, device=feat.device)
    _check(lib().mscnn_roipool_maps_build_f32(_dev(feat), _dev(maps), N, Cc, H, W, C.c_void_p(stream.cuda_stream) if stream is not None else _stream()))
    return maps


def roipool_pair(feat, rois, pooled_h, pooled_w, spatial_scale, pad_a, pad_b):
    N, Cc, H, W = feat.shape
    R = rois.shape[0]
    out = torch.empty((R, 2 * Cc, pooled_h, pooled_w), dtype=torch.float32, device=feat.device)
    _check(lib().mscnn_roipool_pair_fwd_f32(_dev(feat), _dev(rois), _dev(out), R, N, Cc, H, W, pooled_h, pooled_w, spatial_scale,
                                            pad_a, 0, pad_b, Cc, 2 * Cc, _stream()))
    return out


def roialign(feat, rois, pooled_h, pooled_w, spatial_scale, pad_ratio=0.0):
    N, Cc, H, W = feat.shape
    R = rois.shape[0]
    out = torch.empty((R, Cc, pooled_h + 1, pooled_w + 1), dtype=torch.float32, device=feat.device)
    _check(lib().mscnn_roialign_fwd_f32(_dev(feat), _dev(rois), _dev(out), R, N, Cc, H, W, pooled_h, pooled_w, spatial_scale,
                                        pad_ratio, _stream()))
    return out


def roialign_ave(feat, rois, ph, pw, scale, pad, out=None, c_total=None, c_offset=0):
    N, Cc, H, W = feat.shape
    R = rois.shape[0]
    c_total = c_total or Cc
    if out is None:
        out = torch.empty((R, c_total, ph, pw), dtype=torch.float32, device=feat.device)
    _check(lib().mscnn_roialign_ave_fwd_f32(_dev(feat), _dev(rois), _dev(out), R, N, Cc, H, W, ph, pw, scale, pad, c_total, c_offset,
                                            _stream()))
    return out


def roialign_ave_pair(feat, rois, ph, pw, scale, pad_a, pad_b, out=None, c_total=None, c_offset_a=0, c_offset_b=None):
    N, Cc, H, W = feat.shape
    R = rois.shape[0]
    if c_offset_b is None:
        c_offset_b = c_offset_a + Cc
    c_total = c_total or max(c_offset_a, c_offset_b) + Cc
    if out is None:
        out = torch.empty((R, c_total, ph, pw), dtype=torch.float32, device=feat.device)
    _check(lib().mscnn_roialign_ave_pair_fwd_f32(_dev(feat), _dev(rois), _dev(out), R, N, Cc, H, W, ph, pw, scale, pad_a, c_offset_a,
                                                 pad_b, c_offset_b, c_total, _stream()))
    return out


def eltwise(xs, op="SUM", coeffs=None):
    n = len(xs)
    for t in xs:
        _dev(t)
    ptrs = (C.c_void_p * n)(*[t.data_ptr() for t in xs])
    cf = (C.c_float * n)(*coeffs) if coeffs is not None and len(coeffs) else None
    y = torch.empty_like(xs[0])
    _check(lib().mscnn_eltwise_fwd_f32(ptrs, n, cf, _dev(y), y.numel(), {"PROD": 0, "SUM": 1, "MAX": 2}[op], _stream()))
    return y


def make_boxoutput_desc(head_shapes, num, channels, field_w, field_h, downsample, fg_thr=-5.0, iou_thr=0.65,
                        nms_type="IOU", field_whr=2.0, field_xyr=2.0, max_nms_num=2000, max_post_nms_num=0,
                        min_size=15.0, bbox_mean=None, bbox_std=None):
    d = BoxOutputDesc()
    d.num_heads = len(head_shapes); d.num = num; d.channels = channels
    for j, (h, w) in enumerate(head_shapes):
        d.head_h[j] = h; d.head_w[j] = w
        d.field_w[j] = field_w[j]; d.field_h[j] = field_h[j]; d.downsample_rate[j] = downsample[j]
    d.fg_thr = fg_thr; d.iou_thr = iou_thr; d.nms_mode = NMS_MODES[nms_type]
    d.field_whr = field_whr; d.field_xyr = field_xyr
    d.max_nms_num = max_nms_num; d.max_post_nms_num = max_post_nms_num; d.min_size = min_size
    if bbox_mean is not None and bbox_std is not None and len(bbox_mean) and len(bbox_std):
# ... 449 lines not shown
```

mscnn_amd/host/include/caffe/layers/mscnn_layers.hpp:

```cpp
#ifndef MSCNN_CAFFE_LAYERS_HPP_
#define MSCNN_CAFFE_LAYERS_HPP_

#include <functional>
#include <string>
#include <vector>

#include "caffe/blob.hpp"
#include "caffe/layer.hpp"

struct mscnn_conv_plan;

namespace caffe {

class DeviceBuffer {
 public:
  DeviceBuffer() : ptr_(nullptr), bytes_(0) {}
  ~DeviceBuffer();
  void* Reserve(size_t bytes);
  void Release();
  void* get() const { return ptr_; }
  size_t bytes() const { return bytes_; }
 private:
  void* ptr_;
  size_t bytes_;
// ... 49 lines not shown
  void PrebuildRoiMaps(const Blob<Dtype>* feat);
  void InvalidateRoiMaps() { roi_maps_feat_ = nullptr; }
  void ChainTo(ConvolutionLayer* next) { chain_next_ = next; }
  ConvolutionLayer* chain_next() const { return chain_next_; }
  void set_chain_live(bool on) { chain_live_ = on; if (!on) prepared_ = false; }
  void set_pool_only_live(bool on) { pool_only_live_ = on; }
  void set_keep_top(bool on) { keep_top_ = on; }
  bool top_stale() const { return top_stale_; }
  void ForwardUnchained(const vector<Blob<Dtype>*>& bottom, const vector<Blob<Dtype>*>& top) {
    const bool live = chain_live_, po = pool_only_live_;
    chain_live_ = false; prepared_ = false; pool_only_live_ = false;
    this->Forward(bottom, top);
    chain_live_ = live; pool_only_live_ = po;
  }
  virtual double ForwardFlops() const;
  const char* kernel_name() const;
  const char* dtype() const;
  void set_algo(int algo);
  int algo() const { return algo_; }
  void set_calibrated_direct(bool on) { calibrated_direct_ = on; }
  bool calibrated_direct() const { return calibrated_direct_; }
  static constexpr double kDefaultSelfcheckTol = 5e-5;
  bool WinogradCheckApplies() const;
  void set_selfcheck(double tol) { selfcheck_tol_ = tol; selfcheck_pending_ = true; wino_checked_ = false; }
  double selfcheck_tol() const { return selfcheck_tol_; }
  bool take_selfcheck(double* err, bool* fell_back) {
    if (!selfcheck_ran_) return false;
    selfcheck_ran_ = false; *err = selfcheck_err_; *fell_back = selfcheck_fell_back_;
    selfcheck_fell_back_ = false;
    return true;
  }
  void set_tuning(int variant, int grid, int flags);
  double ExecutedFlops() const;
  void set_profiling(bool on);
  bool StageMs(float ms[3]) const;
  enum CheckUse { kWhole = 0, kBand = 1 };
  bool BeginCheck(const vector<Blob<Dtype>*>& bottom, const vector<Blob<Dtype>*>& top, CheckUse use);
  int PollCheck(CheckUse use, double* err, bool wait, bool* vacuous = nullptr);
  double ErrorAgainstDirect(const vector<Blob<Dtype>*>& bottom, const vector<Blob<Dtype>*>& top, bool* vacuous = nullptr);
  static void ReleaseCheckScratch();
  void set_amax_io(const ConvolutionLayer* src, const unsigned* in, unsigned* out) { amax_src_ = src; amax_in_ = in; amax_out_ = out; }
  const ConvolutionLayer* amax_src() const { return amax_src_; }
  void set_amax_wanted(bool on) { amax_wanted_ = on; }
  void set_amax_trusted(bool on) { amax_trusted_ = on; }
  bool publishes_amax() const;
 protected:
  MSCNN_NO_CPU_PATH("Convolution")
  virtual void Forward_gpu(const vector<Blob<Dtype>*>& bottom, const vector<Blob<Dtype>*>& top);
  void Plan(int n, int h, int w);
  int num_output_, channels_, group_, kernel_h_, kernel_w_, pad_h_, pad_w_, stride_h_, stride_w_;
  bool bias_term_;
  mscnn_conv_plan* plan_;
  bool relu_, weights_dirty_;
  int planned_n_, planned_h_, planned_w_;
  Blob<Dtype>* pooled_top_ = nullptr;
  DeviceBuffer packed_, workspace_;
  int algo_, tune_[3];
  ROIPoolingLayer<Dtype>* roi_src_ = nullptr;
  bool last_fused_roipool_ = false;
  DeviceBuffer roi_maps_;
  const Dtype* roi_maps_feat_ = nullptr;
  int roi_maps_shape_[4] = {0, 0, 0, 0};
  ConvolutionLayer* chain_next_ = nullptr;
  bool chain_live_ = false, pool_only_live_ = false, top_stale_ = false, last_chained_ = false, keep_top_ = false;
  bool prepared_ = false;
  size_t ws_off_ = 0, next_off_ = 0;
  bool fuse_next_now_ = false;
  bool ChainableNow(int n, int h, int w);
  bool calibrated_direct_ = false;
  double selfcheck_tol_ = kDefaultSelfcheckTol, selfcheck_err_ = 0.0;
  bool selfcheck_pending_ = true, selfcheck_ran_ = false, selfcheck_fell_back_ = false;
  bool wino_checked_ = false;
  struct CheckBand { bool by_rows; int n0, bn, r0, rows, in0, bh; };
  CheckBand BandOf(int N, int H, int Ho, bool roi_pending, int band) const;
  struct Check {
    mscnn_conv_plan* plan = nullptr;
    void* done = nullptr;
    bool inflight = false;
  } check_[2];
  struct Verdict { double ssx; float err; };
  Verdict* verdict_ = nullptr;
  int next_band_ = 0;
  bool profiling_;
  const ConvolutionLayer* amax_src_ = nullptr;
  const unsigned* amax_in_ = nullptr;
  unsigned* amax_out_ = nullptr;
  bool amax_wanted_ = false, amax_trusted_ = false;
};

template <typename Dtype>
class DeconvolutionLayer : public Layer<Dtype> {
 public:
  explicit DeconvolutionLayer(const LayerParameter& param) : Layer<Dtype>(param) {}
  virtual void LayerSetUp(const vector<Blob<Dtype>*>& bottom, const vector<Blob<Dtype>*>& top);
  virtual void Reshape(const vector<Blob<Dtype>*>& bottom, const vector<Blob<Dtype>*>& top);
  virtual inline const char* type() const { return "Deconvolution"; }
  virtual inline int ExactNumBottomBlobs() const { return 1; }
  virtual inline int ExactNumTopBlobs() const { return 1; }
 protected:
  MSCNN_NO_CPU_PATH("Deconvolution")
  virtual void Forward_gpu(const vector<Blob<Dtype>*>& bottom, const vector<Blob<Dtype>*>& top);
  int num_output_, channels_, group_, kernel_h_, kernel_w_, pad_h_, pad_w_, stride_h_, stride_w_;
  bool bias_term_;
};

template <typename Dtype>
class PoolingLayer : public Layer<Dtype> {
 public:
  explicit PoolingLayer(const LayerParameter& param) : Layer<Dtype>(param) {}
  virtual void LayerSetUp(const vector<Blob<Dtype>*>& bottom, const vector<Blob<Dtype>*>& top);
  virtual void Reshape(const vector<Blob<Dtype>*>& bottom, const vector<Blob<Dtype>*>& top);
  virtual inline const char* type() const { return "Pooling"; }
  virtual inline int ExactNumBottomBlobs() const { return 1; }
  virtual inline int ExactNumTopBlobs() const { return 1; }
  virtual bool IsMaxPool2x2() const {
    return method_ == 0 && !global_pooling_ && kernel_h_ == 2 && kernel_w_ == 2 && stride_h_ == 2 && stride_w_ == 2 && pad_h_ == 0 && pad_w_ == 0;
  }
  bool IsAvePool2x2Stride1() const {
    return method_ == 1 && !global_pooling_ && kernel_h_ == 2 && kernel_w_ == 2 && stride_h_ == 1 && stride_w_ == 1 && pad_h_ == 0 && pad_w_ == 0;
  }
 protected:
  MSCNN_NO_CPU_PATH("Pooling")
  virtual void Forward_gpu(const vector<Blob<Dtype>*>& bottom, const vector<Blob<Dtype>*>& top);
  int kernel_h_, kernel_w_, stride_h_, stride_w_, pad_h_, pad_w_;
  int channels_, height_, width_, pooled_height_, pooled_width_;
  bool global_pooling_;
  int method_;
};

template <typename Dtype>
class ReLULayer : public Layer<Dtype> {
 public:
  explicit ReLULayer(const LayerParameter& param) : Layer<Dtype>(param) {}
  virtual void Reshape(const vector<Blob<Dtype>*>& bottom, const vector<Blob<Dtype>*>& top) { top[0]->ReshapeLike(*bottom[0]); }
  virtual inline const char* type() const { return "ReLU"; }
  virtual inline int ExactNumBottomBlobs() const { return 1; }
  virtual inline int ExactNumTopBlobs() const { return 1; }
 protected:
  MSCNN_NO_CPU_PATH("ReLU")
  virtual void Forward_gpu(const vector<Blob<Dtype>*>& bottom, const vector<Blob<Dtype>*>& top);
};

template <typename Dtype>
class InnerProductLayer : public Layer<Dtype> {
 public:
  explicit InnerProductLayer(const LayerParameter& param) : Layer<Dtype>(param), relu_(false), f16_(false), w16_dirty_(true) {}
  void set_f16(bool on) { f16_ = on; w16_dirty_ = true; }
  void set_x3(bool on) { x3_ = on; w16_dirty_ = true; }
  bool x3() const { return x3_; }
  void set_amax_in(const ConvolutionLayer<Dtype>* src, const unsigned* in) { amax_src_ = src; amax_in_ = in; }
  void set_amax_trusted(bool on) { amax_trusted_ = on; }
  const char* dtype() const { return used_x3_ ? "f16x3" : used_f16_ ? "f16" : "f32"; }
  void set_algo(int algo) { algo_ = algo; }
  const char* kernel_name() const { return used_x3_ ? "x3_gemm" : used_f16_ ? "gemm16_tn" : used_wg_ ? "wgemm_256x128_ck32_epi" : "gemm_tn"; }
  virtual void OnWeightsChanged() { w16_dirty_ = true; wt_dirty_ = true; }
  virtual void LayerSetUp(const vector<Blob<Dtype>*>& bottom, const vector<Blob<Dtype>*>& top);
  virtual void Reshape(const vector<Blob<Dtype>*>& bottom, const vector<Blob<Dtype>*>& top);
  virtual inline const char* type() const { return "InnerProduct"; }
  virtual inline int ExactNumBottomBlobs() const { return 1; }
  virtual inline int ExactNumTopBlobs() const { return 1; }
  virtual bool FuseReLU(Dtype negative_slope) { if (negative_slope != 0) return false; relu_ = true; return true; }
  virtual double ForwardFlops() const { return 2.0 * M_ * N_ * K_; }
 protected:
  MSCNN_NO_CPU_PATH("InnerProduct")
  virtual void Forward_gpu(const vector<Blob<Dtype>*>& bottom, const vector<Blob<Dtype>*>& top);
  int M_, K_, N_;
  bool bias_term_, relu_;
  bool f16_, w16_dirty_, used_f16_ = false;
  bool x3_ = false, used_x3_ = false, amax_trusted_ = false;
  const ConvolutionLayer<Dtype>* amax_src_ = nullptr;
  const unsigned* amax_in_ = nullptr;
  DeviceBuffer w16_, x3_ws_;
  int algo_ = 0;
  bool wt_dirty_ = true, used_wg_ = false;
  DeviceBuffer wt_, wg_ws_;
};

template <typename Dtype>
class ConcatLayer : public Layer<Dtype> {
 public:
  explicit ConcatLayer(const LayerParameter& param) : Layer<Dtype>(param) {}
  virtual void LayerSetUp(const vector<Blob<Dtype>*>& bottom, const vector<Blob<Dtype>*>& top);
  virtual void Reshape(const vector<Blob<Dtype>*>& bottom, const vector<Blob<Dtype>*>& top);
  virtual inline const char* type() const { return "Concat"; }
  virtual inline int MinBottomBlobs() const { return 1; }
  virtual inline int ExactNumTopBlobs() const { return 1; }
 protected:
  MSCNN_NO_CPU_PATH("Concat")
  virtual void Forward_gpu(const vector<Blob<Dtype>*>& bottom, const vector<Blob<Dtype>*>& top);
  int concat_axis_, num_concats_, concat_input_size_;
};

template <typename Dtype>
class DropoutLayer : public Layer<Dtype> {
 public:
  explicit DropoutLayer(const LayerParameter& param) : Layer<Dtype>(param) {}
  virtual void Reshape(const vector<Blob<Dtype>*>& bottom, const vector<Blob<Dtype>*>& top) { top[0]->ReshapeLike(*bottom[0]); }
  virtual inline const char* type() const { return "Dropout"; }
  virtual inline int ExactNumBottomBlobs() const { return 1; }
  virtual inline int ExactNumTopBlobs() const { return 1; }
 protected:
  MSCNN_NO_CPU_PATH("Dropout")
  virtual void Forward_gpu(const vector<Blob<Dtype>*>& bottom, const vector<Blob<Dtype>*>& top);
};

template <typename Dtype>
class SoftmaxLayer : public Layer<Dtype> {
 public:
  explicit SoftmaxLayer(const LayerParameter& param) : Layer<Dtype>(param) {}
  virtual void Reshape(const vector<Blob<Dtype>*>& bottom, const vector<Blob<Dtype>*>& top);
  virtual inline const char* type() const { return "Softmax"; }
  virtual inline int ExactNumBottomBlobs() const { return 1; }
  virtual inline int ExactNumTopBlobs() const { return 1; }
 protected:
  MSCNN_NO_CPU_PATH("Softmax")
  virtual void Forward_gpu(const vector<Blob<Dtype>*>& bottom, const vector<Blob<Dtype>*>& top);
  int outer_num_, inner_num_, softmax_axis_;
};

template <typename Dtype>
class ROIPoolingLayer : public Layer<Dtype> {
 public:
  explicit ROIPoolingLayer(const LayerParameter& param)
      : Layer<Dtype>(param), window_(nullptr), window_c_total_(0), window_c_offset_(0), partner_(nullptr), skip_(false) {}
  bool PairWith(ROIPoolingLayer* second);
  void set_skip(bool s) { skip_ = s; }
  void set_deferred(bool on) { deferred_ = on; if (!on) pending_ = false; }
  bool deferred() const { return deferred_; }
  bool pending() const { return pending_; }
  void Materialize();
  const vector<Blob<Dtype>*>& pending_bottoms() const { return pending_bottom_; }
  ROIPoolingLayer* partner() const { return partner_; }
  int channels() const { return channels_; }
  int pooled_height() const { return pooled_height_; }
  int pooled_width() const { return pooled_width_; }
  Dtype spatial_scale() const { return spatial_scale_; }
  Dtype pad_ratio() const { return pad_ratio_; }
  int window_c_offset() const { return window_c_offset_; }
  const Blob<Dtype>* window() const { return window_; }
  virtual bool SetOutputWindow(Blob<Dtype>* target, int c_total, int c_offset) {
    window_ = target; window_c_total_ = c_total; window_c_offset_ = c_offset;
    return true;
  }
  virtual void LayerSetUp(const vector<Blob<Dtype>*>& bottom, const vector<Blob<Dtype>*>& top);
  virtual void Reshape(const vector<Blob<Dtype>*>& bottom, const vector<Blob<Dtype>*>& top);
  virtual inline const char* type() const { return "ROIPooling"; }
  virtual inline int MinBottomBlobs() const { return 2; }
  virtual inline int MaxBottomBlobs() const { return 2; }
  virtual inline int MinTopBlobs() const { return 1; }
  virtual inline int MaxTopBlobs() const { return 1; }
 protected:
  MSCNN_NO_CPU_PATH("ROIPooling")
  virtual void Forward_gpu(const vector<Blob<Dtype>*>& bottom, const vector<Blob<Dtype>*>& top);
  int channels_, height_, width_, pooled_height_, pooled_width_;
  Dtype spatial_scale_, pad_ratio_;
  Blob<Dtype>* window_;
  int window_c_total_, window_c_offset_;
  ROIPoolingLayer* partner_;
  bool skip_;
  bool deferred_ = false, pending_ = false;
  vector<Blob<Dtype>*> pending_bottom_;
  void LaunchPair(const vector<Blob<Dtype>*>& bottom);
};

template <typename Dtype>
class ROIAlignLayer : public Layer<Dtype> {
 public:
  explicit ROIAlignLayer(const LayerParameter& param) : Layer<Dtype>(param) {}
  void PairWith(ROIAlignLayer* partner, Blob<Dtype>* head_top, int c_total, int c_offset, int partner_c_offset) {
    partner_ = partner; head_top_ = head_top; head_c_total_ = c_total; head_c_offset_ = c_offset; partner_c_offset_ = partner_c_offset;
  }
  void set_pair_live(bool on) { pair_live_ = on; }
  const char* kernel_name() const { return last_fused_ ? "roialign_ave_pair" : ""; }
  void ForwardStandalone(const vector<Blob<Dtype>*>& bottom, const vector<Blob<Dtype>*>& top);
  int pooled_height() const { return pooled_height_; }
  int pooled_width() const { return pooled_width_; }
  Dtype spatial_scale() const { return spatial_scale_; }
  Dtype pad_ratio() const { return pad_ratio_; }
  virtual void LayerSetUp(const vector<Blob<Dtype>*>& bottom, const vector<Blob<Dtype>*>& top);
  virtual void Reshape(const vector<Blob<Dtype>*>& bottom, const vector<Blob<Dtype>*>& top);
  virtual inline const char* type() const { return "ROIAlign"; }
  virtual inline int MinBottomBlobs() const { return 2; }
  virtual inline int MaxBottomBlobs() const { return 2; }
  virtual inline int ExactNumTopBlobs() const { return 1; }
 protected:
  MSCNN_NO_CPU_PATH("ROIAlign")
  virtual void Forward_gpu(const vector<Blob<Dtype>*>& bottom, const vector<Blob<Dtype>*>& top);
  int channels_, height_, width_, pooled_height_, pooled_width_;
  Dtype spatial_scale_, pad_ratio_;
  ROIAlignLayer* partner_ = nullptr;
  Blob<Dtype>* head_top_ = nullptr;
  int head_c_total_ = 0, head_c_offset_ = 0, partner_c_offset_ = 0;
  bool pair_live_ = false, last_fused_ = false;
};

template <typename Dtype>
class EltwiseLayer : public Layer<Dtype> {
 public:
  explicit EltwiseLayer(const LayerParameter& param) : Layer<Dtype>(param) {}
  virtual void LayerSetUp(const vector<Blob<Dtype>*>& bottom, const vector<Blob<Dtype>*>& top);
  virtual void Reshape(const vector<Blob<Dtype>*>& bottom, const vector<Blob<Dtype>*>& top);
  virtual inline const char* type() const { return "Eltwise"; }
  virtual inline int MinBottomBlobs() const { return 2; }
  virtual inline int ExactNumTopBlobs() const { return 1; }
 protected:
  MSCNN_NO_CPU_PATH("Eltwise")
  virtual void Forward_gpu(const vector<Blob<Dtype>*>& bottom, const vector<Blob<Dtype>*>& top);
  int op_;
  vector<float> coeffs_;
};

template <typename Dtype>
class BoxOutputLayer : public Layer<Dtype> {
 public:
  explicit BoxOutputLayer(const LayerParameter& param) : Layer<Dtype>(param), forwarded_(false) {}
  virtual ~BoxOutputLayer();
  virtual void LayerSetUp(const vector<Blob<Dtype>*>& bottom, const vector<Blob<Dtype>*>& top);
  virtual void Reshape(const vector<Blob<Dtype>*>& bottom, const vector<Blob<Dtype>*>& top);
  virtual inline const char* type() const { return "BoxOutput"; }
  virtual inline int MinBottomBlobs() const { return 1; }
  virtual inline int MinTopBlobs() const { return 1; }
  virtual inline int MaxTopBlobs() const { return 2; }
  int last_num_rois() const { return last_rows_; }
  int max_rows() const { return cap_; }
  void set_before_sync(std::function<void()> f) { before_sync_ = std::move(f); }
  void set_one_pass(bool on) { one_pass_ = on; }
  int RowBound(const vector<Blob<Dtype>*>& bottom) const;
  void IngestBegin(const vector<Blob<Dtype>*>& bottom, const vector<Blob<Dtype>*>& top, const void* rows, bool on_device, int coords,
// ... 43 lines not shown
```

mscnn_amd/host/src/capi.cpp:

```cpp
#include <hip/hip_runtime_api.h>

#include <algorithm>
#include <cstring>
#include <functional>
#include <string>
#include <vector>

#include "../../../include/mscnn_hip.h"
#include "../../../include/mscnn_net.h"
#include "caffe/caffe.hpp"

using caffe::Blob;
using caffe::Caffe;
using caffe::Net;

struct mscnn_net {
  std::unique_ptr<Net<float> > net;
  int device;
  caffe::DeviceBuffer det_ws;
  caffe::DeviceBuffer img_in, img_ws;
  caffe::DeviceBuffer det_pack;
  void* det_host = nullptr;
  void* det_host_dev = nullptr;
  size_t det_host_bytes = 0;
  std::vector<int> row_end;
  long rows_forward = -1;
  struct Slot { caffe::DeviceBuffer pack; void* host = nullptr; size_t bytes = 0; hipEvent_t done = nullptr; int cap = 0, handoff_errors = 0; } slot[2];
  int slot_head = 0, slot_tail = 0, slots_inflight = 0;
  mscnn_nms_params nms;
  bool nms_set = false;
  struct Merge {
    bool open = false;
    int images = 0, slots = 0, cand_cap = 0, passes = 0, handoff_errors = 0;
    long rows = 0;
    std::vector<double> overlap;
    std::vector<char> overlap_known;
    caffe::DeviceBuffer cand;
  } merge;
  ~mscnn_net() {
    if (det_host) (void)hipHostFree(det_host);
    for (Slot& sl : slot) {
      if (sl.done) { (void)hipEventSynchronize(sl.done); (void)hipEventDestroy(sl.done); }
      if (sl.host) (void)hipHostFree(sl.host);
    }
  }
};

namespace {
thread_local std::string g_err;

template <class F>
int guarded(F&& f) {
  try {
    f();
    return 0;
  } catch (const std::exception& e) {
    g_err = e.what();
    return 1;
  }
}

void fill_shape(const Blob<float>& b, int* dims8, int* ndim) {
  *ndim = b.num_axes();
  for (int i = 0; i < 8; ++i) dims8[i] = i < b.num_axes() ? b.shape(i) : 1;
}

int create(caffe::NetParameter param, int device, mscnn_net** out, unsigned flags = 0, bool use_default_fusion = true) {
  return guarded([&] {
    CHECK(out != nullptr);
    if (device >= 0) Caffe::SetDevice(device);
    Caffe::set_mode(Caffe::GPU);
    std::unique_ptr<mscnn_net> h(new mscnn_net());
    h->device = device;
    if (use_default_fusion) h->net.reset(new Net<float>(param, caffe::TEST));
    else h->net.reset(new Net<float>(param, caffe::TEST, !(flags & MSCNN_NET_NO_FUSION)));
    *out = h.release();
  });
}
}

extern "C" {

const char* mscnn_net_last_error(void) { return g_err.c_str(); }

int mscnn_net_create_from_file(const char* path, int device, mscnn_net** out) {
  caffe::NetParameter p;
  int rc = guarded([&] { caffe::ReadNetParamsFromTextFileOrDie(path, &p); });
  return rc ? rc : create(p, device, out);
}

int mscnn_net_create_from_string(const char* text, int device, mscnn_net** out) {
  caffe::NetParameter p;
  int rc = guarded([&] { p = caffe::NetParameterFromString(text); });
  return rc ? rc : create(p, device, out);
}

int mscnn_net_create_from_string_ex(const char* text, int device, unsigned flags, mscnn_net** out) {
  caffe::NetParameter p;
  int rc = guarded([&] { p = caffe::NetParameterFromString(text); });
  return rc ? rc : create(p, device, out, flags, false);
}

void mscnn_net_destroy(mscnn_net* net) { delete net; }

int mscnn_net_load_caffemodel(mscnn_net* net, const char* path) { return guarded([&] { net->net->CopyTrainedLayersFrom(path); }); }

int mscnn_net_set_stream(void* stream) { Caffe::set_stream(stream); return 0; }

int mscnn_net_num_layers(const mscnn_net* n) { return (int)n->net->layers().size(); }
const char* mscnn_net_layer_name(const mscnn_net* n, int i) { return n->net->layer_names()[i].c_str(); }
const char* mscnn_net_layer_type(const mscnn_net* n, int i) { return n->net->layers()[i]->type(); }
int mscnn_net_layer_index(const mscnn_net* n, const char* name) {
  const auto& v = n->net->layer_names();
  for (size_t i = 0; i < v.size(); ++i)
    if (v[i] == name) return (int)i;
  return -1;
}
int mscnn_net_layer_num_bottoms(const mscnn_net* n, int l) { return (int)n->net->bottom_vecs()[l].size(); }
int mscnn_net_layer_num_tops(const mscnn_net* n, int l) { return (int)n->net->top_vecs()[l].size(); }
static const char* blob_name_of(const mscnn_net* n, const Blob<float>* b) {
  const auto& blobs = n->net->blobs();
  for (size_t i = 0; i < blobs.size(); ++i)
    if (blobs[i].get() == b) return n->net->blob_names()[i].c_str();
  return "";
}
const char* mscnn_net_layer_bottom(const mscnn_net* n, int l, int i) { return blob_name_of(n, n->net->bottom_vecs()[l][i]); }
const char* mscnn_net_layer_top(const mscnn_net* n, int l, int i) { return blob_name_of(n, n->net->top_vecs()[l][i]); }
int mscnn_net_layer_num_params(const mscnn_net* n, int l) { return (int)n->net->layers()[l]->blobs().size(); }
int mscnn_net_layer_param_shape(const mscnn_net* n, int l, int p, int* dims8, int* ndim) {
  return guarded([&] {
    CHECK_LT(p, (int)n->net->layers()[l]->blobs().size());
    fill_shape(*n->net->layers()[l]->blobs()[p], dims8, ndim);
  });
}
const char* mscnn_net_layer_param_text(const mscnn_net* n, int l) {
  static thread_local std::string text;
  text = n->net->layers()[l]->layer_param().raw().DebugString();
  return text.c_str();
}
int mscnn_net_layer_fused_away(const mscnn_net* n, int l) { return n->net->layer_fused_away()[l] ? 1 : 0; }
const char* mscnn_net_layer_kernel(const mscnn_net* n, int l) {
  auto* c = dynamic_cast<caffe::ConvolutionLayer<float>*>(n->net->layers()[l].get());
  if (c) return c->kernel_name();
  auto* ip = dynamic_cast<caffe::InnerProductLayer<float>*>(n->net->layers()[l].get());
  if (ip) return ip->kernel_name();
  auto* ra = dynamic_cast<caffe::ROIAlignLayer<float>*>(n->net->layers()[l].get());
  return ra ? ra->kernel_name() : "";
}
int mscnn_net_set_inner_product_algo(mscnn_net* n, int layer, int algo) {
  return guarded([&] {
    CHECK_LT(layer, (int)n->net->layers().size());
    CHECK(algo == 0 || algo == 1) << "inner product algo: 0 auto, 1 gemm.hip's stream-K kernel";
    for (int l = (layer < 0 ? 0 : layer); l < (layer < 0 ? (int)n->net->layers().size() : layer + 1); ++l)
      if (auto* ip = dynamic_cast<caffe::InnerProductLayer<float>*>(n->net->layers()[l].get())) ip->set_algo(algo);
      else CHECK_LT(layer, 0) << "layer " << n->net->layer_names()[l] << " is not an InnerProduct";
  });
}
double mscnn_net_layer_flops(const mscnn_net* n, int l) { return n->net->layers()[l]->ForwardFlops(); }
static caffe::ConvolutionLayer<float>* conv_of(const mscnn_net* n, int l) {
  return dynamic_cast<caffe::ConvolutionLayer<float>*>(n->net->layers()[l].get());
}
double mscnn_net_layer_executed_flops(const mscnn_net* n, int l) {
  auto* c = conv_of(n, l);
  return c ? c->ExecutedFlops() : n->net->layers()[l]->ForwardFlops();
}
int mscnn_net_set_conv_profiling(mscnn_net* n, int on) {
  return guarded([&] {
    for (size_t l = 0; l < n->net->layers().size(); ++l)
      if (auto* c = conv_of(n, (int)l)) c->set_profiling(on != 0);
  });
}
int mscnn_net_layer_stage_ms(const mscnn_net* n, int l, float ms_out[3]) {
  ms_out[0] = ms_out[1] = ms_out[2] = 0.f;
  auto* c = conv_of(n, l);
  return (c && c->StageMs(ms_out)) ? 0 : 1;
}
int mscnn_net_set_conv_algo(mscnn_net* n, int layer, int algo) {
  return guarded([&] {
    CHECK_LT(layer, (int)n->net->layers().size());
    for (int l = (layer < 0 ? 0 : layer); l < (layer < 0 ? (int)n->net->layers().size() : layer + 1); ++l)
      if (auto* c = conv_of(n, l)) { c->set_algo(algo); c->set_calibrated_direct(false); }
      else CHECK_LT(layer, 0) << "layer " << n->net->layer_names()[l] << " is not a Convolution";
  });
}
int mscnn_net_set_conv_tuning(mscnn_net* n, int layer, int variant, int grid, int flags) {
  return guarded([&] {
    CHECK_LT(layer, (int)n->net->layers().size());
    for (int l = (layer < 0 ? 0 : layer); l < (layer < 0 ? (int)n->net->layers().size() : layer + 1); ++l)
      if (auto* c = conv_of(n, l)) c->set_tuning(variant, grid, flags);
  });
}
int mscnn_net_set_precision(mscnn_net* n, const char* dtype) {
  return guarded([&] {
    const std::string d = dtype ? dtype : "";
    CHECK(d == "f32" || d == "f16" || d == "f16x3") << "precision must be f32, f16 or f16x3, not '" << d << "'";
    for (size_t l = 0; l < n->net->layers().size(); ++l) {
      if (auto* c = conv_of(n, (int)l)) c->set_algo(d == "f16" ? 4 : c->calibrated_direct() ? 1 : d == "f16x3" ? 5 : 0);
      if (auto* ip = dynamic_cast<caffe::InnerProductLayer<float>*>(n->net->layers()[l].get())) { ip->set_f16(d == "f16"); ip->set_x3(d == "f16x3"); }
    }
  });
}
const char* mscnn_net_layer_dtype(const mscnn_net* n, int l) {
  if (auto* c = conv_of(n, l)) return c->dtype();
  if (auto* ip = dynamic_cast<caffe::InnerProductLayer<float>*>(n->net->layers()[l].get())) return ip->dtype();
  return "f32";
}
int mscnn_net_calibrate_numerics(mscnn_net* n, double tol, int* num_switched) {
  return guarded([&] {
    const std::vector<int> sw = n->net->CalibrateNumerics(tol);
    if (num_switched) *num_switched = (int)sw.size();
  });
}
double mscnn_net_layer_calibration_err(const mscnn_net* n, int l) { return n->net->calibration_err()[l]; }
int mscnn_net_set_numerics_watch(mscnn_net* n, int period, double tol) {
  return guarded([&] {
    CHECK_GE(period, 0);
    n->net->SetNumericsWatch(period, tol);
  });
}
int mscnn_net_numerics_watch_state(const mscnn_net* n, int* checks, int* switched_layers, int cap) {
  const std::vector<int>& sw = n->net->numerics_watch_switched();
  if (checks) *checks = n->net->numerics_watch_checks();
  for (int i = 0; switched_layers && i < cap && i < (int)sw.size(); ++i) switched_layers[i] = sw[i];
  return (int)sw.size();
}
int mscnn_net_set_auto_calibrate(mscnn_net* n, double tol) {
  return guarded([&] { n->net->SetAutoCalibrate(tol); });
}
int mscnn_net_set_chain_fusion(mscnn_net* n, int on) {
  return guarded([&] { n->net->SetChainFusion(on != 0); });
}
int mscnn_net_set_boxoutput_one_pass(mscnn_net* n, int on) {
  return guarded([&] {
    for (const auto& layer : n->net->layers())
      if (auto* bo = dynamic_cast<caffe::BoxOutputLayer<float>*>(layer.get())) bo->set_one_pass(on != 0);
  });
}
int mscnn_net_set_roialign_one_pass(mscnn_net* n, int on) {
  return guarded([&] { n->net->SetRoiAlignOnePass(on != 0); });
}
int mscnn_net_roialign_pairs(const mscnn_net* n, int* first_layers, int cap) {
  const std::vector<int> heads = n->net->roialign_pairs();
  for (int i = 0; first_layers && i < cap && i < (int)heads.size(); ++i) first_layers[i] = heads[i];
  return (int)heads.size();
}
int mscnn_net_chain_pairs(const mscnn_net* n, int* producers, int* consumers, int cap) {
  const auto pairs = n->net->chain_pairs();
  for (int i = 0; i < cap && i < (int)pairs.size(); ++i) {
    if (producers) producers[i] = pairs[i].first;
    if (consumers) consumers[i] = pairs[i].second;
  }
  return (int)pairs.size();
}
int mscnn_net_auto_calibrate_state(const mscnn_net* n, int* checks, int* switched_layers, int cap) {
  const std::vector<int>& sw = n->net->auto_calibrate_switched();
  if (checks) *checks = n->net->auto_calibrate_checks();
  for (int i = 0; switched_layers && i < cap && i < (int)sw.size(); ++i) switched_layers[i] = sw[i];
  return (int)sw.size();
}
int mscnn_net_num_blobs(const mscnn_net* n) { return (int)n->net->blobs().size(); }
const char* mscnn_net_blob_name(const mscnn_net* n, int b) { return n->net->blob_names()[b].c_str(); }
int mscnn_net_blob_shape(const mscnn_net* n, const char* name, int* dims8, int* ndim) {
  return guarded([&] {
    CHECK(n->net->has_blob(name)) << "Unknown blob name " << name;
    fill_shape(*n->net->blob_by_name(name), dims8, ndim);
  });
}
int mscnn_net_num_inputs(const mscnn_net* n) { return n->net->num_inputs(); }
int mscnn_net_num_outputs(const mscnn_net* n) { return n->net->num_outputs(); }
const char* mscnn_net_output_name(const mscnn_net* n, int i) { return n->net->blob_names()[n->net->output_blob_indices()[i]].c_str(); }

int mscnn_net_set_param(mscnn_net* n, int l, int p, const float* host, size_t count) {
  return guarded([&] {
    auto& blobs = n->net->layers()[l]->blobs();
    CHECK_LT(p, (int)blobs.size());
    CHECK_EQ((size_t)blobs[p]->count(), count) << "param size mismatch for layer " << n->net->layer_names()[l];
    n->net->MaterializeStale();
    std::memcpy(blobs[p]->mutable_cpu_data(), host, sizeof(float) * count);
    n->net->layers()[l]->OnWeightsChanged();
  });
}
int mscnn_net_get_param(mscnn_net* n, int l, int p, float* host, size_t count) {
  return guarded([&] {
    auto& blobs = n->net->layers()[l]->blobs();
    CHECK_LT(p, (int)blobs.size());
    CHECK_EQ((size_t)blobs[p]->count(), count);
    std::memcpy(host, blobs[p]->cpu_data(), sizeof(float) * count);
  });
}

int mscnn_net_set_blob(mscnn_net* n, const char* name, const float* host, size_t count) {
  return guarded([&] {
    CHECK(n->net->has_blob(name)) << "Unknown blob name " << name;
    n->net->MaterializePendingReadersOf(name);
    auto b = n->net->blob_by_name(name);
    CHECK_EQ((size_t)b->count(), count) << "blob " << name << " has shape " << b->shape_string();
    std::memcpy(b->mutable_cpu_data(), host, sizeof(float) * count);
  });
}
int mscnn_net_set_blob_device(mscnn_net* n, const char* name, const float* dev, size_t count) {
  return guarded([&] {
    CHECK(n->net->has_blob(name)) << "Unknown blob name " << name;
    n->net->MaterializePendingReadersOf(name);
    auto b = n->net->blob_by_name(name);
    CHECK_EQ((size_t)b->count(), count) << "blob " << name << " has shape " << b->shape_string();
// ... 1051 lines not shown
```

mscnn_amd/host/src/layers.cpp:

```cpp
#include <hip/hip_runtime_api.h>

#include <cmath>
#include <cstring>
#include <random>

#include "../../../include/mscnn_hip.h"
#include "caffe/layer_factory.hpp"
#include "caffe/layers/mscnn_layers.hpp"

namespace caffe {

namespace {
void Fill(const FillerParameter& fp, Blob<float>* blob, unsigned seed) {
  float* d = blob->mutable_cpu_data();
  const string t = fp.type();
  if (t == "constant") {
    if (fp.value() != 0.f)
      for (int i = 0; i < blob->count(); ++i) d[i] = fp.value();
  } else if (t == "gaussian") {
    std::mt19937 gen(seed);
    std::normal_distribution<float> dist(fp.mean(), fp.std());
    for (int i = 0; i < blob->count(); ++i) d[i] = dist(gen);
  } else if (t == "bilinear") {
    CHECK_EQ(blob->num_axes(), 4) << "Blob must be 4 dim.";
// ... 435 lines not shown
    top_stale_ = pool_only;
  }
  if (pooled_top_ && !pooled) {
    MSCNN_CHECK(mscnn_pool2d_fwd_f32(top[0]->gpu_data(), pooled_top_->mutable_gpu_data(), top[0]->num(), top[0]->channels(),
                                     top[0]->height(), top[0]->width(), 2, 2, 0, 0, 2, 2, 0, S()));
  }
  if (selfcheck_pending_ && bottom[0]->count() > 0) {
    selfcheck_pending_ = false;
    if (selfcheck_tol_ > 0 && WinogradCheckApplies()) {
      bool vacuous = false;
      selfcheck_err_ = ErrorAgainstDirect(bottom, top, &vacuous);
      if (vacuous) selfcheck_pending_ = true;
      else selfcheck_ran_ = wino_checked_ = true;
      if (!vacuous && !(selfcheck_err_ <= selfcheck_tol_)) {
        LOG(WARNING) << "layer " << this->layer_param_.name() << ": Winograd result off the direct sum by " << selfcheck_err_ << " > "
                     << selfcheck_tol_ << " on the first input after a weight change: using the direct kernel";
        set_algo(MSCNN_CONV_ALGO_DIRECT);
        calibrated_direct_ = true;
        selfcheck_fell_back_ = true;
        Forward_gpu(bottom, top);
      }
    }
  }
}

template <typename Dtype>
void ConvolutionLayer<Dtype>::PrebuildRoiMaps(const Blob<Dtype>* feat) {
  roi_maps_feat_ = nullptr;
  ROIPoolingLayer<Dtype>* a = roi_src_;
  if (!a || !last_fused_roipool_ || selfcheck_pending_ || pooled_top_ || feat->count() == 0 || feat->channels() != a->channels()) return;
  const int N = feat->num(), C = feat->channels(), H = feat->height(), W = feat->width();
  float* maps = static_cast<float*>(roi_maps_.Reserve(mscnn_roipool_maps_bytes(N, C, H, W)));
  MSCNN_CHECK(mscnn_roipool_maps_build_f32(feat->gpu_data(), maps, N, C, H, W, S()));
  roi_maps_feat_ = feat->gpu_data();
  roi_maps_shape_[0] = N; roi_maps_shape_[1] = C; roi_maps_shape_[2] = H; roi_maps_shape_[3] = W;
}

template <typename Dtype>
bool ConvolutionLayer<Dtype>::FusePool2x2(Blob<Dtype>* pooled_top) {
  pooled_top_ = pooled_top;
  return true;
}

template <typename Dtype>
void DeconvolutionLayer<Dtype>::LayerSetUp(const vector<Blob<Dtype>*>& bottom, const vector<Blob<Dtype>*>& top) {
  const ConvolutionParameter p = this->layer_param_.convolution_param();
  ParseConvParam(p, &kernel_h_, &kernel_w_, &pad_h_, &pad_w_, &stride_h_, &stride_w_);
  channels_ = bottom[0]->channels();
  num_output_ = p.num_output();
  group_ = p.group();
  CHECK_GT(num_output_, 0);
  CHECK_EQ(channels_ % group_, 0);
  CHECK_EQ(num_output_ % group_, 0) << "Number of output should be multiples of group.";
  bias_term_ = p.bias_term();
  if (this->blobs_.size() == 0) {
    this->blobs_.resize(bias_term_ ? 2 : 1);
    this->blobs_[0].reset(new Blob<Dtype>(channels_, num_output_ / group_, kernel_h_, kernel_w_));
    Fill(p.weight_filler(), this->blobs_[0].get(), 1703);
    if (bias_term_) {
      this->blobs_[1].reset(new Blob<Dtype>(vector<int>(1, num_output_)));
      Fill(p.bias_filler(), this->blobs_[1].get(), 1704);
    }
  }
}
template <typename Dtype>
void DeconvolutionLayer<Dtype>::Reshape(const vector<Blob<Dtype>*>& bottom, const vector<Blob<Dtype>*>& top) {
  const int oh = stride_h_ * (bottom[0]->height() - 1) + kernel_h_ - 2 * pad_h_;
  const int ow = stride_w_ * (bottom[0]->width() - 1) + kernel_w_ - 2 * pad_w_;
  top[0]->Reshape(bottom[0]->num(), num_output_, oh, ow);
}
template <typename Dtype>
void DeconvolutionLayer<Dtype>::Forward_gpu(const vector<Blob<Dtype>*>& bottom, const vector<Blob<Dtype>*>& top) {
  MSCNN_CHECK(mscnn_deconv2d_fwd_f32(bottom[0]->gpu_data(), this->blobs_[0]->gpu_data(),
                                     bias_term_ ? this->blobs_[1]->gpu_data() : nullptr, top[0]->mutable_gpu_data(),
                                     bottom[0]->num(), channels_, bottom[0]->height(), bottom[0]->width(), num_output_, kernel_h_,
                                     kernel_w_, pad_h_, pad_w_, stride_h_, stride_w_, group_, S()));
}

template <typename Dtype>
void PoolingLayer<Dtype>::LayerSetUp(const vector<Blob<Dtype>*>& bottom, const vector<Blob<Dtype>*>& top) {
  const PoolingParameter p = this->layer_param_.pooling_param();
  global_pooling_ = p.global_pooling();
  if (global_pooling_) {
    CHECK(!(p.has_kernel_size() || p.has_kernel_h() || p.has_kernel_w())) << "With Global_pooling: true Filter size cannot specified";
    kernel_h_ = bottom[0]->height(); kernel_w_ = bottom[0]->width();
  } else {
    CHECK(!p.has_kernel_size() != !(p.has_kernel_h() && p.has_kernel_w())) << "Filter size is kernel_size OR kernel_h and kernel_w; not both";
    if (p.has_kernel_size()) kernel_h_ = kernel_w_ = p.kernel_size();
    else { kernel_h_ = p.kernel_h(); kernel_w_ = p.kernel_w(); }
  }
  CHECK_GT(kernel_h_, 0); CHECK_GT(kernel_w_, 0);
  if (!p.has_pad_h()) pad_h_ = pad_w_ = p.pad(); else { pad_h_ = p.pad_h(); pad_w_ = p.pad_w(); }
  if (!p.has_stride_h()) stride_h_ = stride_w_ = p.stride(); else { stride_h_ = p.stride_h(); stride_w_ = p.stride_w(); }
  if (pad_h_ != 0 || pad_w_ != 0) {
    CHECK(p.pool() == PoolingParameter_PoolMethod_AVE || p.pool() == PoolingParameter_PoolMethod_MAX) << "Padding implemented only for average and max pooling.";
    CHECK_LT(pad_h_, kernel_h_); CHECK_LT(pad_w_, kernel_w_);
  }
  CHECK(p.pool() != PoolingParameter_PoolMethod_STOCHASTIC) << "stochastic pooling is training-only";
  method_ = p.pool() == PoolingParameter_PoolMethod_MAX ? 0 : 1;
}
template <typename Dtype>
void PoolingLayer<Dtype>::Reshape(const vector<Blob<Dtype>*>& bottom, const vector<Blob<Dtype>*>& top) {
  CHECK_EQ(4, bottom[0]->num_axes()) << "Input must have 4 axes, corresponding to (num, channels, height, width)";
  channels_ = bottom[0]->channels(); height_ = bottom[0]->height(); width_ = bottom[0]->width();
  if (global_pooling_) { kernel_h_ = height_; kernel_w_ = width_; }
  pooled_height_ = mscnn_pool_out_dim(height_, kernel_h_, pad_h_, stride_h_);
  pooled_width_ = mscnn_pool_out_dim(width_, kernel_w_, pad_w_, stride_w_);
  top[0]->Reshape(bottom[0]->num(), channels_, pooled_height_, pooled_width_);
}
template <typename Dtype>
void PoolingLayer<Dtype>::Forward_gpu(const vector<Blob<Dtype>*>& bottom, const vector<Blob<Dtype>*>& top) {
  MSCNN_CHECK(mscnn_pool2d_fwd_f32(bottom[0]->gpu_data(), top[0]->mutable_gpu_data(), bottom[0]->num(), channels_, height_, width_,
                                   kernel_h_, kernel_w_, pad_h_, pad_w_, stride_h_, stride_w_, method_, S()));
}

template <typename Dtype>
void ReLULayer<Dtype>::Forward_gpu(const vector<Blob<Dtype>*>& bottom, const vector<Blob<Dtype>*>& top) {
  MSCNN_CHECK(mscnn_relu_fwd_f32(bottom[0]->gpu_data(), top[0]->mutable_gpu_data(), (size_t)bottom[0]->count(),
                                 this->layer_param_.relu_param().negative_slope(), S()));
}

template <typename Dtype>
void InnerProductLayer<Dtype>::LayerSetUp(const vector<Blob<Dtype>*>& bottom, const vector<Blob<Dtype>*>& top) {
  const InnerProductParameter p = this->layer_param_.inner_product_param();
  N_ = p.num_output();
  bias_term_ = p.bias_term();
  CHECK(!p.transpose()) << "transpose: true is not used by the MS-CNN nets";
  const int axis = bottom[0]->CanonicalAxisIndex(p.axis());
  K_ = bottom[0]->count(axis);
  if (this->blobs_.size() == 0) {
    this->blobs_.resize(bias_term_ ? 2 : 1);
    vector<int> ws(2); ws[0] = N_; ws[1] = K_;
    this->blobs_[0].reset(new Blob<Dtype>(ws));
    Fill(p.weight_filler(), this->blobs_[0].get(), 1705);
    if (bias_term_) {
      this->blobs_[1].reset(new Blob<Dtype>(vector<int>(1, N_)));
      Fill(p.bias_filler(), this->blobs_[1].get(), 1706);
    }
  }
}
template <typename Dtype>
void InnerProductLayer<Dtype>::Reshape(const vector<Blob<Dtype>*>& bottom, const vector<Blob<Dtype>*>& top) {
  const int axis = bottom[0]->CanonicalAxisIndex(this->layer_param_.inner_product_param().axis());
  const int new_K = bottom[0]->count(axis);
  CHECK_EQ(K_, new_K) << "Input size incompatible with inner product parameters.";
  M_ = bottom[0]->count(0, axis);
  vector<int> top_shape = bottom[0]->shape();
  top_shape.resize(axis + 1);
  top_shape[axis] = N_;
  top[0]->Reshape(top_shape);
}
template <typename Dtype>
void InnerProductLayer<Dtype>::Forward_gpu(const vector<Blob<Dtype>*>& bottom, const vector<Blob<Dtype>*>& top) {
  used_wg_ = false;
  used_x3_ = x3_ && mscnn_inner_product_x3_supported(N_, K_);
  if (used_x3_) {
    void* pk = w16_.Reserve(mscnn_inner_product_x3_packed_bytes(N_, K_));
    if (w16_dirty_) {
      MSCNN_CHECK(mscnn_inner_product_x3_pack(this->blobs_[0]->gpu_data(), pk, N_, K_, S()));
      w16_dirty_ = false;
    }
    const size_t wb = mscnn_inner_product_x3_workspace_bytes(M_, N_, K_);
    const bool handed = amax_trusted_ && amax_src_ && amax_in_ && amax_src_->publishes_amax();
    MSCNN_CHECK(mscnn_inner_product_x3_fwd(bottom[0]->gpu_data(), pk, bias_term_ ? this->blobs_[1]->gpu_data() : nullptr,
                                           top[0]->mutable_gpu_data(), M_, N_, K_, relu_ ? 1 : 0, handed ? amax_in_ : nullptr,
                                           x3_ws_.Reserve(wb), wb, S()));
    used_f16_ = false;
    return;
  }
  used_f16_ = f16_ && mscnn_inner_product_f16_supported(N_, K_);
  if (used_f16_) {
    void* w16 = w16_.Reserve((size_t)N_ * K_ * 2);
    if (w16_dirty_) {
      MSCNN_CHECK(mscnn_inner_product_pack_f16(this->blobs_[0]->gpu_data(), w16, N_, K_, S()));
      w16_dirty_ = false;
    }
    MSCNN_CHECK(mscnn_inner_product_fwd_f16(bottom[0]->gpu_data(), w16, bias_term_ ? this->blobs_[1]->gpu_data() : nullptr,
                                            top[0]->mutable_gpu_data(), M_, N_, K_, relu_ ? 1 : 0, S()));
    return;
  }
  used_wg_ = algo_ == 0 && !mscnn_wgemm_whole_tiles_forced() && mscnn_inner_product_wg_supported(M_, N_, K_);
  if (used_wg_) {
    float* wt = static_cast<float*>(wt_.Reserve(mscnn_inner_product_wg_packed_bytes(N_, K_)));
    if (wt_dirty_) {
      MSCNN_CHECK(mscnn_inner_product_wg_pack(this->blobs_[0]->gpu_data(), wt, N_, K_, S()));
      wt_dirty_ = false;
    }
    const size_t wb = mscnn_inner_product_wg_workspace_bytes(M_, N_, K_);
    MSCNN_CHECK(mscnn_inner_product_wg_fwd(bottom[0]->gpu_data(), wt, bias_term_ ? this->blobs_[1]->gpu_data() : nullptr,
                                           top[0]->mutable_gpu_data(), M_, N_, K_, relu_ ? 1 : 0, wg_ws_.Reserve(wb), wb, S()));
    return;
  }
  MSCNN_CHECK(mscnn_inner_product_fwd_f32(bottom[0]->gpu_data(), this->blobs_[0]->gpu_data(),
                                          bias_term_ ? this->blobs_[1]->gpu_data() : nullptr, top[0]->mutable_gpu_data(), M_, N_, K_,
                                          relu_ ? 1 : 0, S()));
}

template <typename Dtype>
void ConcatLayer<Dtype>::LayerSetUp(const vector<Blob<Dtype>*>& bottom, const vector<Blob<Dtype>*>& top) {
  const ConcatParameter p = this->layer_param_.concat_param();
  CHECK(!(p.raw().has("axis") && p.has_concat_dim())) << "Either axis or concat_dim should be specified; not both.";
}
template <typename Dtype>
void ConcatLayer<Dtype>::Reshape(const vector<Blob<Dtype>*>& bottom, const vector<Blob<Dtype>*>& top) {
  const ConcatParameter p = this->layer_param_.concat_param();
  const int num_axes = bottom[0]->num_axes();
  concat_axis_ = p.has_concat_dim() ? (int)p.concat_dim() : bottom[0]->CanonicalAxisIndex(p.axis());
  CHECK_LT(concat_axis_, num_axes) << "concat axis out of range.";
  vector<int> top_shape = bottom[0]->shape();
  num_concats_ = bottom[0]->count(0, concat_axis_);
  concat_input_size_ = bottom[0]->count(concat_axis_ + 1);
  for (size_t i = 1; i < bottom.size(); ++i) {
    CHECK_EQ(num_axes, bottom[i]->num_axes()) << "All inputs must have the same #axes.";
    for (int j = 0; j < num_axes; ++j) {
      if (j == concat_axis_) continue;
      CHECK_EQ(top_shape[j], bottom[i]->shape(j)) << "All inputs must have the same shape, except at concat_axis.";
    }
    top_shape[concat_axis_] += bottom[i]->shape(concat_axis_);
  }
  top[0]->Reshape(top_shape);
  if (bottom.size() == 1) top[0]->ShareData(*bottom[0]);
}
template <typename Dtype>
void ConcatLayer<Dtype>::Forward_gpu(const vector<Blob<Dtype>*>& bottom, const vector<Blob<Dtype>*>& top) {
  if (bottom.size() == 1) return;
  Dtype* top_data = top[0]->mutable_gpu_data();
  const int top_concat_axis = top[0]->shape(concat_axis_);
  int offset = 0;
  for (size_t i = 0; i < bottom.size(); ++i) {
    const int c = bottom[i]->shape(concat_axis_);
    MSCNN_CHECK(mscnn_concat_channels_f32(bottom[i]->gpu_data(), top_data, num_concats_, c, concat_input_size_, top_concat_axis, offset, S()));
    offset += c;
  }
}

template <typename Dtype>
void DropoutLayer<Dtype>::Forward_gpu(const vector<Blob<Dtype>*>& bottom, const vector<Blob<Dtype>*>& top) {
  CHECK(this->phase_ == TEST) << "Dropout: TRAIN phase is outside the inference path";
  if (top[0] == bottom[0]) return;
  const Dtype* src = bottom[0]->gpu_data();
  Dtype* dst = top[0]->mutable_gpu_data();
  if (src != dst)
    HIP_CHECK(hipMemcpyAsync(dst, src, sizeof(Dtype) * bottom[0]->count(), hipMemcpyDeviceToDevice, (hipStream_t)S()));
}

template <typename Dtype>
void SoftmaxLayer<Dtype>::Reshape(const vector<Blob<Dtype>*>& bottom, const vector<Blob<Dtype>*>& top) {
  softmax_axis_ = bottom[0]->CanonicalAxisIndex(this->layer_param_.softmax_param().axis());
  top[0]->ReshapeLike(*bottom[0]);
  outer_num_ = bottom[0]->count(0, softmax_axis_);
  inner_num_ = bottom[0]->count(softmax_axis_ + 1);
}
template <typename Dtype>
void SoftmaxLayer<Dtype>::Forward_gpu(const vector<Blob<Dtype>*>& bottom, const vector<Blob<Dtype>*>& top) {
  MSCNN_CHECK(mscnn_softmax_fwd_f32(bottom[0]->gpu_data(), top[0]->mutable_gpu_data(), outer_num_, bottom[0]->shape(softmax_axis_), inner_num_, S()));
}

template <typename Dtype>
void ROIPoolingLayer<Dtype>::LayerSetUp(const vector<Blob<Dtype>*>& bottom, const vector<Blob<Dtype>*>& top) {
  const ROIPoolingParameter p = this->layer_param_.roi_pooling_param();
  CHECK_GT(p.pooled_h(), 0u) << "pooled_h must be > 0";
  CHECK_GT(p.pooled_w(), 0u) << "pooled_w must be > 0";
  pooled_height_ = p.pooled_h();
  pooled_width_ = p.pooled_w();
  spatial_scale_ = p.spatial_scale();
  pad_ratio_ = p.pad_ratio();
  LOG(INFO) << "Spatial scale: " << spatial_scale_;
}
template <typename Dtype>
void ROIPoolingLayer<Dtype>::Reshape(const vector<Blob<Dtype>*>& bottom, const vector<Blob<Dtype>*>& top) {
  channels_ = bottom[0]->channels(); height_ = bottom[0]->height(); width_ = bottom[0]->width();
  top[0]->Reshape(bottom[1]->num(), channels_, pooled_height_, pooled_width_);
}
template <typename Dtype>
bool ROIPoolingLayer<Dtype>::PairWith(ROIPoolingLayer* b) {
  if (!b || b == this || !window_ || b->window_ != window_ || b->window_c_total_ != window_c_total_) return false;
  const ROIPoolingParameter pa = this->layer_param_.roi_pooling_param(), pb = b->layer_param_.roi_pooling_param();
  if (pa.pooled_h() != pb.pooled_h() || pa.pooled_w() != pb.pooled_w() || pa.spatial_scale() != pb.spatial_scale()) return false;
  partner_ = b;
  return true;
}

template <typename Dtype>
void ROIPoolingLayer<Dtype>::LaunchPair(const vector<Blob<Dtype>*>& bottom) {
  MSCNN_CHECK(mscnn_roipool_pair_fwd_f32(bottom[0]->gpu_data(), bottom[1]->gpu_data(), window_->mutable_gpu_data(), bottom[1]->num(),
                                         bottom[0]->num(), channels_, height_, width_, pooled_height_, pooled_width_, spatial_scale_,
                                         pad_ratio_, window_c_offset_, partner_->pad_ratio_, partner_->window_c_offset_, window_c_total_, S()));
}

template <typename Dtype>
void ROIPoolingLayer<Dtype>::Materialize() {
  if (!pending_) return;
  pending_ = false;
  if (pending_bottom_.size() == 2 && pending_bottom_[1]->num() > 0) LaunchPair(pending_bottom_);
}

template <typename Dtype>
void ROIPoolingLayer<Dtype>::Forward_gpu(const vector<Blob<Dtype>*>& bottom, const vector<Blob<Dtype>*>& top) {
  if (skip_) { skip_ = false; return; }
  Dtype* out = window_ ? nullptr : top[0]->mutable_gpu_data();
  int c_total = channels_, c_offset = 0;
  if (window_) {
    window_->Reshape(bottom[1]->num(), window_c_total_, pooled_height_, pooled_width_);
    c_total = window_c_total_; c_offset = window_c_offset_;
  }
  if (partner_ && window_ && partner_->channels_ == channels_) {
    if (deferred_) {
      pending_bottom_ = bottom;
      pending_ = true;
    } else {
      LaunchPair(bottom);
    }
    partner_->set_skip(true);
    return;
  }
  if (window_) out = window_->mutable_gpu_data();
  MSCNN_CHECK(mscnn_roipool_fwd_f32(bottom[0]->gpu_data(), bottom[1]->gpu_data(), out, bottom[1]->num(), bottom[0]->num(), channels_,
                                    height_, width_, pooled_height_, pooled_width_, spatial_scale_, pad_ratio_, c_total, c_offset, S()));
}

template <typename Dtype>
void ROIAlignLayer<Dtype>::LayerSetUp(const vector<Blob<Dtype>*>& bottom, const vector<Blob<Dtype>*>& top) {
  const ROIPoolingParameter p = this->layer_param_.roi_pooling_param();
  CHECK_GT(p.pooled_h(), 0u) << "pooled_h must be > 0";
  CHECK_GT(p.pooled_w(), 0u) << "pooled_w must be > 0";
  pooled_height_ = p.pooled_h(); pooled_width_ = p.pooled_w();
  spatial_scale_ = p.spatial_scale(); pad_ratio_ = p.pad_ratio();
}
template <typename Dtype>
void ROIAlignLayer<Dtype>::Reshape(const vector<Blob<Dtype>*>& bottom, const vector<Blob<Dtype>*>& top) {
  channels_ = bottom[0]->channels(); height_ = bottom[0]->height(); width_ = bottom[0]->width();
  top[0]->Reshape(bottom[1]->num(), channels_, pooled_height_ + 1, pooled_width_ + 1);
}
template <typename Dtype>
// ... 275 lines not shown
```

Baseline: 228.6.

## Add column-form inner product via plane-GEMM with ragged last column block

```diff
diff --git a/include/mscnn_hip.h b/include/mscnn_hip.h
--- a/include/mscnn_hip.h
+++ b/include/mscnn_hip.h
@@ -86,6 +86,18 @@
 MSCNN_API int mscnn_inner_product_wg_pack(const float* w, float* wt, int N, int K, void* stream);
 MSCNN_API int mscnn_inner_product_wg_fwd(const float* x, const float* wt, const float* bias, float* y, int M, int N, int K, int relu,
                                          void* workspace, size_t workspace_bytes, void* stream);
+MSCNN_API int mscnn_inner_product_cols_supported(int M, int N, int K);
+MSCNN_API int mscnn_inner_product_cols_row_stride(int M, int N, int K);
+MSCNN_API int mscnn_inner_product_cols_preferred(int M, int N, int K);
+MSCNN_API size_t mscnn_inner_product_cols_packed_bytes(int N, int K);
+MSCNN_API size_t mscnn_inner_product_cols_workspace_bytes(int M, int N, int K);
+MSCNN_API int mscnn_inner_product_cols_pack(const float* w, float* up, int N, int K, void* stream);
+MSCNN_API int mscnn_inner_product_cols_fwd(const float* xt, const float* up, float* yt, int M, int N, int K, void* workspace,
+                                           size_t workspace_bytes, void* stream);
+MSCNN_API int mscnn_inner_product_cols_transpose_in(const float* x, float* xt, int M, int K, int T_pad, void* stream);
+MSCNN_API int mscnn_inner_product_cols_finish(const float* yt, const float* bias, float* y, int M, int N, int T_pad, int relu, void* stream);
+MSCNN_API void mscnn_debug_inner_product_cols_variant(int variant);
+MSCNN_API long mscnn_debug_inner_product_cols_schedule(int M, int N, int K, int variant, int whole_tiles, int* rows, long max_rows, int info[9]);
 MSCNN_API unsigned long long mscnn_wgemm_handoff_event(void);
 MSCNN_API void mscnn_wgemm_force_whole_tiles(int on);
 MSCNN_API int mscnn_wgemm_whole_tiles_forced(void);
diff --git a/mscnn_amd/csrc/gemm.hip b/mscnn_amd/csrc/gemm.hip
--- a/mscnn_amd/csrc/gemm.hip
+++ b/mscnn_amd/csrc/gemm.hip
@@ -554,3 +554,123 @@
   MSCNN_POST_LAUNCH();
   return mscnn::wgemm_launch(pl, up, wt, y, pl.ws_bytes ? slabs : nullptr, st, 0, nullptr, bias, relu, (size_t)M * N * sizeof(float));
 }
+
+
+namespace {
+
+int g_ip_cols_variant = 0;
+
+bool ip_cols_plan(int M, int N, int K, mscnn::WgemmPlan* pl) {
+  if (M < 192 || N < 256 || N % 32 != 0 || K % 32 != 0) return false;
+  return mscnn::wgemm_plan_cols(N, K, M, g_ip_cols_variant, pl);
+}
+
+__global__ __launch_bounds__(256) void ip_transpose_in_kernel(const float* __restrict__ x, float* __restrict__ xt, int M, int K, int T_pad) {
+  __shared__ float t[32][33];
+  const int k0 = blockIdx.x * 32, r0 = blockIdx.y * 32, tx = threadIdx.x & 31, ty = threadIdx.x >> 5;
+#pragma unroll
+  for (int i = 0; i < 4; ++i) {
+    const int r = r0 + ty + 8 * i, k = k0 + tx;
+    t[ty + 8 * i][tx] = (r < M && k < K) ? x[(size_t)r * K + k] : 0.f;
+  }
+  __syncthreads();
+#pragma unroll
+  for (int i = 0; i < 4; ++i) {
+    const int k = k0 + ty + 8 * i, r = r0 + tx;
+    if (k < K && r < T_pad) xt[(size_t)k * T_pad + r] = t[tx][ty + 8 * i];
+  }
+}
+
+__global__ __launch_bounds__(256) void ip_cols_finish_kernel(const float* __restrict__ yt, const float* __restrict__ bias, float* __restrict__ y,
+                                                             int M, int N, int T_pad, int relu) {
+  __shared__ float t[32][33];
+  const int r0 = blockIdx.x * 32, n0 = blockIdx.y * 32, tx = threadIdx.x & 31, ty = threadIdx.x >> 5;
+#pragma unroll
+  for (int i = 0; i < 4; ++i) {
+    const int n = n0 + ty + 8 * i, r = r0 + tx;
+    t[ty + 8 * i][tx] = (n < N && r < M) ? yt[(size_t)n * T_pad + r] : 0.f;
+  }
+  __syncthreads();
+#pragma unroll
+  for (int i = 0; i < 4; ++i) {
+    const int r = r0 + ty + 8 * i, n = n0 + tx;
+    if (r < M && n < N) {
+      float v = t[tx][ty + 8 * i];
+      if (bias) v += bias[n];
+      if (relu) v = v < 0.f ? 0.f : v;
+      y[(size_t)r * N + n] = v;
+    }
+  }
+}
+
+}
+
+extern "C" void mscnn_debug_inner_product_cols_variant(int variant) { g_ip_cols_variant = variant == 4 || variant == 5 ? variant : 0; }
+extern "C" int mscnn_inner_product_cols_supported(int M, int N, int K) {
+  mscnn::WgemmPlan pl;
+  return ip_cols_plan(M, N, K, &pl) ? 1 : 0;
+}
+extern "C" int mscnn_inner_product_cols_preferred(int M, int N, int K) {
+  mscnn::WgemmPlan pl;
+  if (!ip_cols_plan(M, N, K, &pl)) return 0;
+  const long executed = (long)(pl.NT - 1) * pl.BN + 32L * pl.nb_last, padded_rows = (long)(M + 255) / 256 * 256;
+  return executed * 100 <= padded_rows * 94 ? 1 : 0;
+}
+extern "C" int mscnn_inner_product_cols_row_stride(int M, int N, int K) {
+  mscnn::WgemmPlan pl;
+  return ip_cols_plan(M, N, K, &pl) ? pl.T_pad : 0;
+}
+extern "C" size_t mscnn_inner_product_cols_packed_bytes(int N, int K) {
+  return N > 0 && K > 0 && K % 32 == 0 ? (size_t)((N + 255) / 256) * (size_t)(K / 32) * (32 * 256) * sizeof(float) : 0;
+}
+extern "C" size_t mscnn_inner_product_cols_workspace_bytes(int M, int N, int K) {
+  mscnn::WgemmPlan pl;
+  return ip_cols_plan(M, N, K, &pl) ? pl.ws_bytes : 0;
+}
+extern "C" int mscnn_inner_product_cols_pack(const float* w, float* up, int N, int K, void* stream) {
+  MSCNN_REQUIRE(w && up && N > 0 && K > 0 && K % 32 == 0, "inner_product cols pack: bad argument (N=%d K=%d)", N, K);
+  MSCNN_REQUIRE(reinterpret_cast<uintptr_t>(w) % 16 == 0, "inner_product cols pack: unaligned weights");
+  ip_pack_rows_kernel<<<dim3(K / 32, (N + 255) / 256), 256, 0, as_stream(stream)>>>(w, up, N, K, K / 32);
+  MSCNN_POST_LAUNCH();
+  return MSCNN_OK;
+}
+extern "C" int mscnn_inner_product_cols_fwd(const float* xt, const float* up, float* yt, int M, int N, int K, void* workspace,
+                                            size_t workspace_bytes, void* stream) {
+  MSCNN_REQUIRE(M >= 0 && N > 0 && K > 0, "inner_product: bad shape M=%d N=%d K=%d", M, N, K);
+  if (M == 0) return MSCNN_OK;
+  mscnn::WgemmPlan pl;
+  MSCNN_REQUIRE(ip_cols_plan(M, N, K, &pl), "inner_product cols: shape M=%d N=%d K=%d is not one the column form takes", M, N, K);
+  MSCNN_REQUIRE(xt && up && yt, "inner_product cols: null pointer");
+  MSCNN_REQUIRE_ALIGNED(xt, 16, "inner_product cols: xt");
+  MSCNN_REQUIRE_ALIGNED(up, 16, "inner_product cols: up");
+  if (pl.ws_bytes) {
+    MSCNN_REQUIRE_ALIGNED(workspace, 16, "inner_product cols: workspace");
+    if (!workspace || workspace_bytes < pl.ws_bytes) {
+      set_error("inner_product cols: workspace %zu < %zu", workspace_bytes, pl.ws_bytes);
+      return MSCNN_ERR_WORKSPACE;
+    }
+  }
+  return mscnn::wgemm_launch(pl, up, xt, yt, pl.ws_bytes ? static_cast<float*>(workspace) : nullptr, as_stream(stream), 0, nullptr, nullptr, 0,
+                             (size_t)N * pl.T_pad * sizeof(float));
+}
+extern "C" int mscnn_inner_product_cols_transpose_in(const float* x, float* xt, int M, int K, int T_pad, void* stream) {
+  MSCNN_REQUIRE(x && xt && M > 0 && K > 0 && T_pad >= M, "inner_product cols transpose: bad argument");
+  ip_transpose_in_kernel<<<dim3(cdiv(K, 32), cdiv(T_pad, 32)), 256, 0, as_stream(stream)>>>(x, xt, M, K, T_pad);
+  MSCNN_POST_LAUNCH();
+  return MSCNN_OK;
+}
+extern "C" int mscnn_inner_product_cols_finish(const float* yt, const float* bias, float* y, int M, int N, int T_pad, int relu, void* stream) {
+  MSCNN_REQUIRE(yt && y && M > 0 && N > 0 && T_pad >= M, "inner_product cols finish: bad argument");
+  ip_cols_finish_kernel<<<dim3(cdiv(M, 32), cdiv(N, 32)), 256, 0, as_stream(stream)>>>(yt, bias, y, M, N, T_pad, relu);
+  MSCNN_POST_LAUNCH();
+  return MSCNN_OK;
+}
+extern "C" long mscnn_debug_inner_product_cols_schedule(int M, int N, int K, int variant, int whole_tiles, int* rows, long max_rows, int info[9]) {
+  mscnn::WgemmPlan pl;
+  if (!mscnn::wgemm_plan_cols(N, K, M, variant, &pl)) return -1;
+  if (info) {
+    const int v[9] = {pl.tiles, pl.MT, pl.NT, pl.KI, pl.G, pl.full_q, pl.BN, pl.nb_last, pl.nb_split};
+    for (int i = 0; i < 9; ++i) info[i] = v[i];
+  }
+  return mscnn::wgemm_debug_schedule(pl, whole_tiles, rows, max_rows);
+}
diff --git a/mscnn_amd/csrc/wgemm.h b/mscnn_amd/csrc/wgemm.h
--- a/mscnn_amd/csrc/wgemm.h
+++ b/mscnn_amd/csrc/wgemm.h
@@ -24,6 +24,20 @@
   nt = q - nt_off[pp];
 }
 
+__host__ __device__ __forceinline__ void wgemm_unit_range(int RT, int KI, int MT, int NI, int nb_last, int G, int g, int& b, int& e) {
+  const unsigned U = (unsigned)RT * (unsigned)KI;
+  if (nb_last >= NI) {
+    b = (int)(U * (unsigned)g / (unsigned)G);
+    e = (int)(U * (unsigned)(g + 1) / (unsigned)G);
+    return;
+  }
+  const unsigned U2 = (unsigned)(RT < MT ? RT : MT) * (unsigned)KI, U1 = U - U2;
+  const unsigned C1 = U1 * (unsigned)NI, total = C1 + U2 * (unsigned)nb_last;
+  const unsigned cb = total * (unsigned)g / (unsigned)G, ce = total * (unsigned)(g + 1) / (unsigned)G;
+  b = (int)(cb <= C1 ? cb / (unsigned)NI : U1 + (cb - C1) / (unsigned)nb_last);
+  e = (int)(ce <= C1 ? ce / (unsigned)NI : U1 + (ce - C1) / (unsigned)nb_last);
+}
+
 struct WgemmPlan {
   int P, Cout, Cin, T, T_pad;
   int BM, BN, CK, MT, NT, KI;
@@ -39,7 +53,11 @@
   const char* name;
   size_t packed_bytes;
   size_t ws_bytes;
+  int nb_last;
+  int nb_split;
 };
+
+bool wgemm_plan_cols(int Cout, int Cin, int T, int variant, WgemmPlan* out);
 
 bool wgemm_plan(int P, int Cout, int Cin, int T, int variant, WgemmPlan* out, const int* plane_cols = nullptr);
 
diff --git a/mscnn_amd/csrc/wgemm.hip b/mscnn_amd/csrc/wgemm.hip
--- a/mscnn_amd/csrc/wgemm.hip
+++ b/mscnn_amd/csrc/wgemm.hip
@@ -21,6 +21,8 @@
   unsigned spin_limit;
   int drop_publish;
   int nt_off[mscnn::kWgemmMaxPlanes + 1];
+  int nb_last;
+  int nb_split;
 };
 
 template <int BM_, int BN_, int WGM_, int WGN_, int CK_, int ST_, int DPG_ = 1, int SK_ = 0>
@@ -78,21 +80,15 @@
 __device__ __forceinline__ void lds_wait() { asm volatile("s_waitcnt lgkmcnt(%0)" ::"n"(N) : "memory"); }
 __device__ __forceinline__ void lds_pin(float& v) { asm volatile("" : "+v"(v)); }
 
-__device__ __host__ __forceinline__ void wg_range(int total, int G, int g, int& b, int& e) {
-  b = (int)((unsigned)total * (unsigned)g / (unsigned)G);
-  e = (int)((unsigned)total * (unsigned)(g + 1) / (unsigned)G);
-}
-
 struct SegCursor {
   int slot, G, KI, full_q, rem_tile0, r;
   int it, re;
   int nparts;
-  __device__ __forceinline__ void init(const WgemmArgs& a, int slot_) { init(a.tiles, a.G, a.KI, a.full_q, slot_); }
-  __device__ __host__ __forceinline__ void init(int tiles, int G_, int KI_, int a_full_q, int slot_) {
+  __device__ __host__ __forceinline__ void init(int tiles, int G_, int KI_, int a_full_q, int slot_, int NI, int nb_last, int MT) {
     slot = slot_; G = G_; KI = KI_; rem_tile0 = a_full_q * G_; r = 0; nparts = 0;
     const int rounds = slot_ < tiles ? (tiles - slot_ + G_ - 1) / G_ : 0;
     full_q = a_full_q < rounds ? a_full_q : rounds;
-    if (tiles > rem_tile0) wg_range((tiles - rem_tile0) * KI_, G_, slot_, it, re);
+    if (tiles > rem_tile0) mscnn::wgemm_unit_range(tiles - rem_tile0, KI_, MT, NI, nb_last, G_, slot_, it, re);
     else it = re = 0;
   }
   __device__ __forceinline__ int units() const { return full_q * KI + (re - it); }
@@ -109,8 +105,10 @@
   }
 };
 
-template <class C, int ABL, int EPI = 0, bool RAG = false>
+template <class C, int ABL, int EPI = 0, bool RAG = false, bool COLS = false>
 __global__ __launch_bounds__(C::THREADS, C::NW / 4) void wgemm_kernel(WgemmArgs a) {
+  static_assert(!COLS || (C::WGN == 1 && !RAG), "the column form: every wave owns all NI column blocks; one plane");
+  constexpr bool ALT = COLS && C::NI <= 3;
   __shared__ __attribute__((aligned(1024))) float lds[C::LDS_FLOATS];
   __shared__ unsigned s_handoff_timeout;
   static_assert(C::ST == 3, "the ring protocol below is written for three stages");
@@ -123,7 +121,9 @@
   const int xcd = (int)(blockIdx.x % 8), gq = a.G / 8, gr = a.G % 8;
   const int slot = xcd * gq + min(xcd, gr) + (int)(blockIdx.x / 8);
   SegCursor pcur, ccur;
-  pcur.init(a, slot); ccur.init(a, slot);
+  const int nb_last = COLS ? a.nb_last : C::NI, nb_split = COLS ? a.nb_split : C::NI;
+  pcur.init(a.tiles, a.G, a.KI, a.full_q, slot, C::NI, nb_split, a.MT);
+  ccur = pcur;
   const int nunits = pcur.units();
   if (nunits == 0) return;
   unsigned long long dbg_c = 0, dbg_r = 0;
@@ -213,11 +213,15 @@
     for (int ni = 0; ni < C::NI; ++ni) old_voff[mi][ni] = 0x80000000u;
 
   float av[2][C::MI], bv[2][C::NI];
-#define WG_READ(buf, stage_addr, s)                                                                                         \
+  if constexpr (COLS) {
+#pragma unroll
+    for (int ni = 0; ni < C::NI; ++ni) bv[0][ni] = bv[1][ni] = 0.f;
+  }
+#define WG_READ(buf, stage_addr, s, nbr)                                                                                    \
   {                                                                                                                         \
     _Pragma("unroll") for (int mi = 0; mi < C::MI; ++mi) av[buf][mi] = 0.f;                                                  \
     static_for<0, C::MI>([&](auto m_) { av[buf][decltype(m_)::value] = lds_rd<(s) * 2 * C::BM * 4 + decltype(m_)::value * 128>((stage_addr) + a_lane); }); \
-    static_for<0, C::NI>([&](auto n_) { bv[buf][decltype(n_)::value] = lds_rd<(s) * 2 * C::BN * 4 + decltype(n_)::value * 128>((stage_addr) + b_lane); }); \
+    static_for<0, (nbr)>([&](auto n_) { bv[buf][decltype(n_)::value] = lds_rd<(s) * 2 * C::BN * 4 + decltype(n_)::value * 128>((stage_addr) + b_lane); }); \
   }
   constexpr int NR = C::MI + C::NI;
   constexpr int NMF = C::MI * C::NI;
@@ -244,7 +248,7 @@
   unsigned old_rowb = row_bytes;
   bool old_pub = false;
   unsigned c_addr = lds0;
-  WG_READ(0, c_addr, 0);
+  WG_READ(0, c_addr, 0, C::NI);
 
   auto store_one = [&](auto qc, auto ec) {
     constexpr int Q = decltype(qc)::value, e = decltype(ec)::value;
@@ -260,16 +264,17 @@
     }
   };
 
-  auto chunk = [&](auto par_c, auto flush_c, unsigned next_addr) {
+  auto chunk = [&](auto par_c, auto flush_c, auto nb_c, unsigned next_addr) {
     constexpr int PAR = decltype(par_c)::value;
     constexpr bool FLUSH = decltype(flush_c)::value;
+    constexpr int NB = decltype(nb_c)::value;
     p_begin();
     static_for<0, C::STEPS>([&](auto sc) {
       constexpr int s = decltype(sc)::value, cur = s & 1, nxt = cur ^ 1;
       if constexpr (!(ABL & 8)) {
-        if constexpr (s + 1 < C::STEPS) WG_READ(nxt, c_addr, s + 1)
-        else WG_READ(nxt, next_addr, 0)
-        lds_wait<NR>();
+        if constexpr (s + 1 < C::STEPS) WG_READ(nxt, c_addr, s + 1, NB)
+        else WG_READ(nxt, next_addr, 0, C::NI)
+        lds_wait<(s + 1 < C::STEPS ? C::MI + NB : NR)>();
       }
 #pragma unroll
       for (int mi = 0; mi < C::MI; ++mi) lds_pin(av[cur][mi]);
@@ -278,7 +283,8 @@
       __builtin_amdgcn_sched_barrier(0);
       static_for<0, NMF>([&](auto jc) {
         constexpr int j = decltype(jc)::value, mi = j / C::NI, ni = j % C::NI;
-        if constexpr (!(ABL & 4)) acc[PAR][mi][ni] = __builtin_amdgcn_mfma_f32_32x32x2f32(av[cur][mi], bv[cur][ni], acc[PAR][mi][ni], 0, 0, 0);
+        constexpr int SET = ALT && !FLUSH && (s & 1) ? PAR ^ 1 : PAR;
+        if constexpr (!(ABL & 4) && ni < NB) acc[SET][mi][ni] = __builtin_amdgcn_mfma_f32_32x32x2f32(av[cur][mi], bv[cur][ni], acc[SET][mi][ni], 0, 0, 0);
         __builtin_amdgcn_sched_barrier(0);
         if constexpr (FLUSH && s >= C::SK) {
           if constexpr (!(ABL & 2))
@@ -307,7 +313,7 @@
     return lds0 + (unsigned)c_stage * C::STAGE_BYTES;
   };
   int t, k0, k1, part;
-  int fin_tile = -1;
+  int fin_tile = -1, fin_nb = C::NI;
   typedef __attribute__((address_space(1))) unsigned long long gu64;
   gu64* flags = (gu64*)(a.ws + (size_t)a.G * (C::BM * C::BN));
   const unsigned long long want_flag = ((unsigned long long)a.epoch << 32) | (unsigned)~a.epoch;
@@ -317,13 +323,39 @@
   };
   auto segment = [&](auto par_c) {
     constexpr int PAR = decltype(par_c)::value;
-    chunk(par_c, std::true_type{}, next_stage_addr());
-    if (old_pub) { publish_flag(); old_pub = false; }
-    for (int kc = k0 + 1; kc < k1; ++kc) chunk(par_c, std::false_type{}, next_stage_addr());
     int mt, nt, p;
     mscnn::wgemm_tile_decode(t, a.MT, a.NT, a.P, RAG ? a.nt_off : nullptr, p, nt, mt);
+    const int nb = COLS ? __builtin_amdgcn_readfirstlane(nt == a.NT - 1 ? nb_last : C::NI) : C::NI;
+    auto chunks = [&](auto nb_c) {
+      chunk(par_c, std::true_type{}, nb_c, next_stage_addr());
+      if (old_pub) { publish_flag(); old_pub = false; }
+      if constexpr (ALT) {
+#pragma unroll
+        for (int mi = 0; mi < C::MI; ++mi)
+#pragma unroll
+          for (int ni = 0; ni < C::NI; ++ni)
+#pragma unroll
+            for (int r = 0; r < 16; ++r) acc[PAR ^ 1][mi][ni][r] = 0.f;
+        for (int kc = k0 + 1; kc < k1; ++kc) chunk(par_c, std::false_type{}, nb_c, next_stage_addr());
+#pragma unroll
+        for (int mi = 0; mi < C::MI; ++mi)
+#pragma unroll
+          for (int ni = 0; ni < C::NI; ++ni)
+#pragma unroll
+            for (int r = 0; r < 16; ++r) acc[PAR][mi][ni][r] += acc[PAR ^ 1][mi][ni][r];
+      } else {
+        for (int kc = k0 + 1; kc < k1; ++kc) chunk(par_c, std::false_type{}, nb_c, next_stage_addr());
+      }
+    };
+    if constexpr (COLS) {
+      static_for<1, C::NI + 1>([&](auto nb_c) {
+        if (nb == decltype(nb_c)::value) chunks(nb_c);
+      });
+    } else {
+      chunks(std::integral_constant<int, C::NI>{});
+    }
     const bool pub = part >= 0 && k0 > 0;
-    if (part >= 0 && k0 == 0) fin_tile = t;
+    if (part >= 0 && k0 == 0) { fin_tile = t; fin_nb = nb; }
     old_pub = pub;
     if (pub) { old_rsrc = rW; old_rowb = (unsigned)C::BN * 4u; }
     else { old_rsrc = rM; old_rowb = row_bytes; }
@@ -341,8 +373,8 @@
       for (int ni = 0; ni < C::NI; ++ni) {
         const int row = wm * C::WM + mi * 32, col = wn * C::WN + ni * 32 + l31;
         const int co0 = mt * C::BM + row;
-        const unsigned to_m = co0 + 32 <= a.Cout ? ((unsigned)(p * a.Cout + co0 + 4 * khalf) * (unsigned)a.T_pad + (unsigned)(nt * C::BN + col)) * 4u : 0x80000000u;
-        const unsigned to_ws = slab + (unsigned)((row + 4 * khalf) * C::BN + col) * 4u;
+        const unsigned to_m = COLS && ni >= nb ? 0x80000000u : co0 + 32 <= a.Cout ?((unsigned)(p * a.Cout + co0 + 4 * khalf) * (unsigned)a.T_pad + (unsigned)(nt * C::BN + col)) * 4u : 0x80000000u;
+        const unsigned to_ws = COLS && ni >= nb ? 0x80000000u : slab + (unsigned)((row + 4 * khalf) * C::BN + col) * 4u;
         old_voff[mi][ni] = pub ? to_ws : to_m;
 #pragma unroll
         for (int r = 0; r < 16; ++r) acc[PAR ^ 1][mi][ni][r] = 0.f;
@@ -360,11 +392,11 @@
   auto finish = [&](auto qc) {
     constexpr int Q = decltype(qc)::value;
     if (fin_tile >= 0) {
-      const int rem_tile0 = a.full_q * a.G, RU = (a.tiles - rem_tile0) * a.KI;
+      const int rem_tile0 = a.full_q * a.G;
       const int tile_end = (fin_tile - rem_tile0 + 1) * a.KI;
       for (int s2 = slot + 1; s2 < a.G; ++s2) {
         int b, e;
-        wg_range(RU, a.G, s2, b, e);
+        mscnn::wgemm_unit_range(a.tiles - rem_tile0, a.KI, a.MT, C::NI, nb_split, a.G, s2, b, e);
         if (b >= tile_end) break;
         if (e <= b) continue;
         if (tid == 0) {
@@ -385,7 +417,8 @@
         for (int mi = 0; mi < C::MI; ++mi)
 #pragma unroll
           for (int ni = 0; ni < C::NI; ++ni) {
-            const unsigned vo = sl2 + (unsigned)((wm * C::WM + mi * 32 + 4 * khalf) * C::BN + wn * C::WN + ni * 32 + l31) * 4u;
+            if (COLS && ni >= fin_nb) continue;
+            const unsigned vo = sl2 +(unsigned)((wm * C::WM + mi * 32 + 4 * khalf) * C::BN + wn * C::WN + ni * 32 + l31) * 4u;
 #pragma unroll
             for (int r = 0; r < 16; ++r)
               acc[Q][mi][ni][r] += __builtin_bit_cast(float, __builtin_amdgcn_raw_buffer_load_b32(rW, vo, (unsigned)((r & 3) + 8 * (r >> 2)) * (unsigned)(C::BN * 4), 0));
@@ -415,6 +448,7 @@
 #define WG_ENTRY(name, v, abl, BM, BN, WGM, WGN, CK) {name, v, abl, BM, BN, CK, WGM * WGN * 64, wgemm_kernel<WCfg<BM, BN, WGM, WGN, CK, 3>, abl>}
 #define WG_ENTRY_R(name, v, BM, BN, WGM, WGN, CK) {name, v, 0, BM, BN, CK, WGM * WGN * 64, wgemm_kernel<WCfg<BM, BN, WGM, WGN, CK, 3>, 0>, wgemm_kernel<WCfg<BM, BN, WGM, WGN, CK, 3>, 0, 0, true>}
 #define WG_ENTRY_EPI(name, v, BM, BN, WGM, WGN, CK) {name, v + 64, 0, BM, BN, CK, WGM * WGN * 64, wgemm_kernel<WCfg<BM, BN, WGM, WGN, CK, 3>, 0, 1>}
+#define WG_ENTRY_COLS(name, v, BM, BN, WGM, WGN, CK) {name, v + 128, 0, BM, BN, CK, WGM * WGN * 64, wgemm_kernel<WCfg<BM, BN, WGM, WGN, CK, 3>, 0, 0, false, true>}
 #define WG_ENTRY_S(name, v, BM, BN, WGM, WGN, CK, DPG, SK) {name, v, 0, BM, BN, CK, WGM * WGN * 64, wgemm_kernel<WCfg<BM, BN, WGM, WGN, CK, 3, DPG, SK>, 0>}
 const WEntry kW[] = {
     WG_ENTRY_R("wgemm_256x128_ck32", 1, 256, 128, 4, 2, 32),
@@ -423,6 +457,8 @@
     WG_ENTRY_R("wgemm_256x96_ck32", 4, 256, 96, 8, 1, 32),
     WG_ENTRY_R("wgemm_256x160_ck32", 5, 256, 160, 8, 1, 32),
     WG_ENTRY_EPI("wgemm_256x128_ck32_epi", 1, 256, 128, 4, 2, 32),
+    WG_ENTRY_COLS("wgemm_256x96_ck32_cols", 4, 256, 96, 8, 1, 32),
+    WG_ENTRY_COLS("wgemm_256x160_ck32_cols", 5, 256, 160, 8, 1, 32),
 #ifdef MSCNN_WGEMM_DEV
     WG_ENTRY_S("wgemm_256x128_ck32_d2", 25, 256, 128, 4, 2, 32, 2, 0),
     WG_ENTRY_S("wgemm_256x128_ck32_d2_s3", 26, 256, 128, 4, 2, 32, 2, 3),
@@ -543,12 +579,58 @@
   if (variant_flags & 1) o->full_q = (int)(tiles / o->G);
   if (variant_flags & 2) o->full_q = (int)((tiles + o->G - 1) / o->G);
   o->variant = variant; o->name = e->name;
+  o->nb_last = o->nb_split = e->BN / 32;
   o->packed_bytes = (size_t)P * o->MT * o->KI * e->CK * e->BM * 4;
   o->ws_bytes = tiles > (long)o->full_q * o->G ? (size_t)o->G * e->BM * e->BN * 4 + ((size_t)o->G + 1) * 8 : 0;
   const double lim = 2147483648.0 - 65536.0;
   if ((double)tiles * o->KI * o->G >= 2.0e9 || o->KI < 1) return false;
   if ((double)P * Cin * o->T_pad * 4 >= lim || (double)P * Cout * o->T_pad * 4 >= lim || (double)o->packed_bytes >= lim ||
       (double)o->ws_bytes >= lim) return false;
+  return true;
+}
+
+bool wgemm_plan_cols(int Cout, int Cin, int T, int variant, WgemmPlan* o) {
+  if (variant == 0) {
+    WgemmPlan p4, p5;
+    const bool h4 = wgemm_plan_cols(Cout, Cin, T, 4, &p4), h5 = wgemm_plan_cols(Cout, Cin, T, 5, &p5);
+    if (!h4 && !h5) return false;
+    auto executed = [](const WgemmPlan& p) { return (p.NT - 1) * p.BN + 32 * p.nb_last; };
+    *o = h4 && (!h5 || executed(p4) < executed(p5)) ? p4 : p5;
+    return true;
+  }
+  if ((variant != 4 && variant != 5) || T < 1 || !wgemm_plan(1, Cout, Cin, T, variant + 128, o)) return false;
+  const int NI = o->BN / 32, G = o->G, MT = o->MT, KI = o->KI;
+  const long tiles = o->tiles, rem = tiles % G;
+  const double chunk_us = (double)o->BM * o->BN * o->CK / 128.0 / 2214.0, block_us = chunk_us / NI;
+  const double handoff_us = 18.0 * (double)(o->BM * o->BN) / (256.0 * 128.0);
+  auto model = [&](int nb) {
+    const double blocks = ((double)(tiles - MT) * NI + (double)MT * nb) * KI;
+    const double whole = (double)((tiles + G - 1) / G) * (KI * chunk_us + 6.0);
+    const double split = blocks / G * block_us + (double)tiles / G * 6.0 + handoff_us;
+    const bool use_split = rem > 0 && split < 0.97 * whole;
+    o->full_q = (int)(tiles / G) + (rem > 0 && !use_split ? 1 : 0);
+    o->model_us = use_split ? split : whole;
+    o->nb_split = nb;
+  };
+  const int nb = (T - (o->NT - 1) * o->BN + 31) / 32;
+  o->nb_last = nb;
+  model(nb);
+  const int RT = (int)(tiles - (long)o->full_q * G);
+  if (nb < NI && RT > 0) {
+    const unsigned U2 = (unsigned)(RT < MT ? RT : MT) * KI, U1 = (unsigned)RT * KI - U2;
+    bool ok = ((double)U1 * NI + (double)U2 * nb) * G < 4.0e9;
+    long lo = 0, hi = 0;
+    for (int g = 0; ok && g < G; ++g) {
+      int b, e;
+      wgemm_unit_range(RT, KI, MT, NI, nb, G, g, b, e);
+      auto cum = [&](unsigned u) { return u <= U1 ? (long)u * NI : (long)U1 * NI + (long)(u - U1) * nb; };
+      const long c = cum((unsigned)e) - cum((unsigned)b);
+      if (g == 0 || c < lo) lo = c;
+      if (g == 0 || c > hi) hi = c;
+    }
+    if (!ok || hi - lo > NI) model(NI);
+  }
+  o->ws_bytes = tiles > (long)o->full_q * G ? (size_t)G * o->BM * o->BN * 4 + ((size_t)G + 1) * 8 : 0;
   return true;
 }
 
@@ -569,6 +651,8 @@
   a.tiles = p.tiles; a.G = p.G;
   a.abl = abl; a.dbg = dbg;
   for (int i = 0; i <= kWgemmMaxPlanes; ++i) a.nt_off[i] = p.nt_off[i];
+  a.nb_last = p.nb_last >= 1 && p.nb_last <= p.BN / 32 ? p.nb_last : p.BN / 32;
+  a.nb_split = p.nb_split >= 1 && p.nb_split <= p.BN / 32 ? p.nb_split : p.BN / 32;
   a.full_q = p.full_q; a.ws_bytes = (unsigned)p.ws_bytes;
   if (g_whole_tiles.load(std::memory_order_relaxed)) a.full_q = (a.tiles + p.G - 1) / p.G;
   const int rem = a.tiles - a.full_q * p.G;
@@ -593,7 +677,7 @@
   long n = 0;
   for (int slot = 0; slot < p.G; ++slot) {
     SegCursor c;
-    c.init(p.tiles, p.G, p.KI, full_q, slot);
+    c.init(p.tiles, p.G, p.KI, full_q, slot, p.BN / 32, p.nb_split, p.MT);
     int t, k0, k1, part;
     while (c.next(t, k0, k1, part)) {
       if (out) {
diff --git a/mscnn_amd/hipapi.py b/mscnn_amd/hipapi.py
--- a/mscnn_amd/hipapi.py
+++ b/mscnn_amd/hipapi.py
@@ -102,6 +102,20 @@
         L.mscnn_inner_product_wg_workspace_bytes.argtypes = [C.c_int] * 3
         L.mscnn_inner_product_wg_pack.argtypes = [C.c_void_p, C.c_void_p, C.c_int, C.c_int, C.c_void_p]
         L.mscnn_inner_product_wg_fwd.argtypes = [C.c_void_p] * 4 + [C.c_int] * 4 + [C.c_void_p, C.c_size_t, C.c_void_p]
+        L.mscnn_inner_product_cols_supported.argtypes = [C.c_int] * 3
+        L.mscnn_inner_product_cols_row_stride.argtypes = [C.c_int] * 3
+        L.mscnn_inner_product_cols_packed_bytes.restype = C.c_size_t
+        L.mscnn_inner_product_cols_packed_bytes.argtypes = [C.c_int, C.c_int]
+        L.mscnn_inner_product_cols_workspace_bytes.restype = C.c_size_t
+        L.mscnn_inner_product_cols_workspace_bytes.argtypes = [C.c_int] * 3
+        L.mscnn_inner_product_cols_pack.argtypes = [C.c_void_p, C.c_void_p, C.c_int, C.c_int, C.c_void_p]
+        L.mscnn_inner_product_cols_fwd.argtypes = [C.c_void_p] * 3 + [C.c_int] * 3 + [C.c_void_p, C.c_size_t, C.c_void_p]
+        L.mscnn_inner_product_cols_transpose_in.argtypes = [C.c_void_p, C.c_void_p, C.c_int, C.c_int, C.c_int, C.c_void_p]
+        L.mscnn_inner_product_cols_finish.argtypes = [C.c_void_p] * 3 + [C.c_int] * 4 + [C.c_void_p]
+        L.mscnn_debug_inner_product_cols_variant.restype = None
+        L.mscnn_debug_inner_product_cols_variant.argtypes = [C.c_int]
+        L.mscnn_debug_inner_product_cols_schedule.restype = C.c_long
+        L.mscnn_debug_inner_product_cols_schedule.argtypes = [C.c_int] * 5 + [C.c_void_p, C.c_long, C.c_void_p]
         L.mscnn_max_rel_diff_f32.argtypes = [C.c_void_p, C.c_void_p, C.c_size_t, C.c_float, C.c_void_p, C.c_void_p]
         L.mscnn_sum_squares_f32.argtypes = [C.c_void_p, C.c_size_t, C.c_void_p, C.c_void_p]
         L.mscnn_max_rel_diff_strided_f32.argtypes = [C.c_void_p, C.c_size_t, C.c_void_p, C.c_size_t, C.c_size_t, C.c_size_t, C.c_void_p, C.c_double,
@@ -462,6 +476,79 @@
     return y, wt
 
 
+def inner_product_cols_supported(M, N, K):
+    return bool(lib().mscnn_inner_product_cols_supported(M, N, K))
+
+
+def debug_inner_product_cols_variant(variant):
+    lib().mscnn_debug_inner_product_cols_variant(int(variant))
+
+
+def inner_product_cols_row_stride(M, N, K):
+    return lib().mscnn_inner_product_cols_row_stride(M, N, K)
+
+
+def inner_product_cols_pack(w):
+    Nn, K = w.shape[0], w.numel() // w.shape[0]
+    up = torch.empty(lib().mscnn_inner_product_cols_packed_bytes(Nn, K) // 4, dtype=torch.float32, device=w.device)
+    _check(lib().mscnn_inner_product_cols_pack(_dev(w), _dev(up), Nn, K, _stream()))
+    return up
+
+
+def inner_product_cols_transpose_in(x, T_pad, out=None):
+    M = x.shape[0]
+    K = x.numel() // M
+    xt = out if out is not None else torch.empty((K, T_pad), dtype=torch.float32, device=x.device)
+    _check(lib().mscnn_inner_product_cols_transpose_in(_dev(x), _dev(xt), M, K, T_pad, _stream()))
+    return xt
+
+
+def inner_product_cols_fwd(xt, up, M, N, yt=None, ws=None):
+    K, T_pad = xt.shape
+    wb = lib().mscnn_inner_product_cols_workspace_bytes(M, N, K)
+    if ws is None:
+        ws = torch.empty(max((wb + 3) // 4, 1), dtype=torch.float32, device=xt.device)
+    if yt is None:
+        yt = torch.empty((N, T_pad), dtype=torch.float32, device=xt.device)
+    _check(lib().mscnn_inner_product_cols_fwd(_dev(xt), _dev(up), _dev(yt), M, N, K, _dev(ws) if wb else None, wb, _stream()))
+    return yt, ws
+
+
+def inner_product_cols_finish(yt, M, bias=None, relu=False, out=None):
+    Nn, T_pad = yt.shape
+    y = out if out is not None else torch.empty((M, Nn), dtype=torch.float32, device=yt.device)
+    _check(lib().mscnn_inner_product_cols_finish(_dev(yt), _dev(bias), _dev(y), M, Nn, T_pad, int(relu), _stream()))
+    return y
+
+
+def inner_product_cols(x, w, bias=None, relu=False, up=None):
+    M = x.shape[0]
+    K = x.numel() // M
+    Nn = w.shape[0]
+    T_pad = inner_product_cols_row_stride(M, Nn, K)
+    if not T_pad:
+        raise MscnnError("inner_product cols: shape M=%d N=%d K=%d is not one the column form takes" % (M, Nn, K))
+    if up is None:
+        up = inner_product_cols_pack(w)
+    yt, _ = inner_product_cols_fwd(inner_product_cols_transpose_in(x, T_pad), up, M, Nn)
+    y = inner_product_cols_finish(yt, M, bias, relu)
+    torch.cuda.current_stream().synchronize()
+    return y, up
+
+
+def inner_product_cols_schedule(M, N, K, variant=0, whole_tiles=False):
+    import numpy as np
+    info = (C.c_int * 9)()
+    n = lib().mscnn_debug_inner_product_cols_schedule(M, N, K, variant, int(whole_tiles), None, 0, info)
+    if n < 0:
+        return None
+    rows = np.zeros((n, 7), dtype=np.int32)
+    got = lib().mscnn_debug_inner_product_cols_schedule(M, N, K, variant, int(whole_tiles), rows.ctypes.data_as(C.POINTER(C.c_int)), n, info)
+    assert got == n
+    keys = ("tiles", "MT", "NT", "KI", "G", "full_q", "BN", "nb_last", "nb_split")
+    return dict(zip(keys, info)), rows
+
+
 def inner_product(x, w, bias=None, relu=False):
     M = x.shape[0]
     K = x.numel() // max(M, 1) if M else w.shape[1]
diff --git a/mscnn_amd/host/include/caffe/layers/mscnn_layers.hpp b/mscnn_amd/host/include/caffe/layers/mscnn_layers.hpp
--- a/mscnn_amd/host/include/caffe/layers/mscnn_layers.hpp
+++ b/mscnn_amd/host/include/caffe/layers/mscnn_layers.hpp
@@ -225,8 +225,10 @@
   void set_amax_trusted(bool on) { amax_trusted_ = on; }
   const char* dtype() const { return used_x3_ ? "f16x3" : used_f16_ ? "f16" : "f32"; }
   void set_algo(int algo) { algo_ = algo; }
-  const char* kernel_name() const { return used_x3_ ? "x3_gemm" : used_f16_ ? "gemm16_tn" : used_wg_ ? "wgemm_256x128_ck32_epi" : "gemm_tn"; }
-  virtual void OnWeightsChanged() { w16_dirty_ = true; wt_dirty_ = true; }
+  const char* kernel_name() const {
+    return used_x3_ ? "x3_gemm" : used_f16_ ? "gemm16_tn" : used_cols_ ? "wgemm_cols" : used_wg_ ? "wgemm_256x128_ck32_epi" : "gemm_tn";
+  }
+  virtual void OnWeightsChanged() { w16_dirty_ = true; wt_dirty_ = true; up_dirty_ = true; }
   virtual void LayerSetUp(const vector<Blob<Dtype>*>& bottom, const vector<Blob<Dtype>*>& top);
   virtual void Reshape(const vector<Blob<Dtype>*>& bottom, const vector<Blob<Dtype>*>& top);
   virtual inline const char* type() const { return "InnerProduct"; }
@@ -247,6 +249,8 @@
   int algo_ = 0;
   bool wt_dirty_ = true, used_wg_ = false;
   DeviceBuffer wt_, wg_ws_;
+  bool up_dirty_ = true, used_cols_ = false;
+  DeviceBuffer up_, cols_xt_, cols_yt_, cols_ws_;
 };
 
 template <typename Dtype>
diff --git a/mscnn_amd/host/src/capi.cpp b/mscnn_amd/host/src/capi.cpp
--- a/mscnn_amd/host/src/capi.cpp
+++ b/mscnn_amd/host/src/capi.cpp
@@ -150,7 +150,7 @@
 int mscnn_net_set_inner_product_algo(mscnn_net* n, int layer, int algo) {
   return guarded([&] {
     CHECK_LT(layer, (int)n->net->layers().size());
-    CHECK(algo == 0 || algo == 1) << "inner product algo: 0 auto, 1 gemm.hip's stream-K kernel";
+    CHECK(algo == 0 || algo == 1 || algo == 2) << "inner product algo: 0 auto, 1 gemm.hip's stream-K kernel, 2 the plane-GEMM kernel's row form";
     for (int l = (layer < 0 ? 0 : layer); l < (layer < 0 ? (int)n->net->layers().size() : layer + 1); ++l)
       if (auto* ip = dynamic_cast<caffe::InnerProductLayer<float>*>(n->net->layers()[l].get())) ip->set_algo(algo);
       else CHECK_LT(layer, 0) << "layer " << n->net->layer_names()[l] << " is not an InnerProduct";
diff --git a/mscnn_amd/host/src/layers.cpp b/mscnn_amd/host/src/layers.cpp
--- a/mscnn_amd/host/src/layers.cpp
+++ b/mscnn_amd/host/src/layers.cpp
@@ -611,7 +611,7 @@
 }
 template <typename Dtype>
 void InnerProductLayer<Dtype>::Forward_gpu(const vector<Blob<Dtype>*>& bottom, const vector<Blob<Dtype>*>& top) {
-  used_wg_ = false;
+  used_wg_ = used_cols_ = false;
   used_x3_ = x3_ && mscnn_inner_product_x3_supported(N_, K_);
   if (used_x3_) {
     void* pk = w16_.Reserve(mscnn_inner_product_x3_packed_bytes(N_, K_));
@@ -638,7 +638,24 @@
                                             top[0]->mutable_gpu_data(), M_, N_, K_, relu_ ? 1 : 0, S()));
     return;
   }
-  used_wg_ = algo_ == 0 && !mscnn_wgemm_whole_tiles_forced() && mscnn_inner_product_wg_supported(M_, N_, K_);
+  used_cols_ = algo_ == 0 && !mscnn_wgemm_whole_tiles_forced() && mscnn_inner_product_cols_preferred(M_, N_, K_);
+  if (used_cols_) {
+    float* up = static_cast<float*>(up_.Reserve(mscnn_inner_product_cols_packed_bytes(N_, K_)));
+    if (up_dirty_) {
+      MSCNN_CHECK(mscnn_inner_product_cols_pack(this->blobs_[0]->gpu_data(), up, N_, K_, S()));
+      up_dirty_ = false;
+    }
+    const int T = mscnn_inner_product_cols_row_stride(M_, N_, K_);
+    float* xt = static_cast<float*>(cols_xt_.Reserve(sizeof(float) * (size_t)K_ * T));
+    float* yt = static_cast<float*>(cols_yt_.Reserve(sizeof(float) * (size_t)N_ * T));
+    const size_t wb = mscnn_inner_product_cols_workspace_bytes(M_, N_, K_);
+    MSCNN_CHECK(mscnn_inner_product_cols_transpose_in(bottom[0]->gpu_data(), xt, M_, K_, T, S()));
+    MSCNN_CHECK(mscnn_inner_product_cols_fwd(xt, up, yt, M_, N_, K_, wb ? cols_ws_.Reserve(wb) : nullptr, wb, S()));
+    MSCNN_CHECK(mscnn_inner_product_cols_finish(yt, bias_term_ ? this->blobs_[1]->gpu_data() : nullptr, top[0]->mutable_gpu_data(), M_, N_, T,
+                                                relu_ ? 1 : 0, S()));
+    return;
+  }
+  used_wg_ = (algo_ == 0 || algo_ == 2) && !mscnn_wgemm_whole_tiles_forced() && mscnn_inner_product_wg_supported(M_, N_, K_);
   if (used_wg_) {
     float* wt = static_cast<float*>(wt_.Reserve(mscnn_inner_product_wg_packed_bytes(N_, K_)));
     if (wt_dirty_) {
```

New measurement: 229.9, median of 6. About the same (+0.6%).
